# tcantenot/bmfr

Measured on AMD Instinct MI355X. Metric: ms/frame @1080p & 4K, 1/2/4/8 GPU; PSNR vs 4096spp reference, lower is better.
Workload: dtype f32+f16 tmp_data

## Files before the change

### bmfr_amd/_build.py

```python
from __future__ import annotations

import concurrent.futures as cf
import hashlib
import os
import subprocess

HERE = os.path.dirname(os.path.abspath(__file__))
CSRC = os.path.join(HERE, "csrc")
LIB = os.path.join(HERE, "libbmfr.so")
DIAG_LIB = os.path.join(HERE, "libbmfr_diag.so")
HIPCC = os.environ.get("HIPCC", "/opt/rocm/bin/hipcc")
SOURCES = ["bmfr_kernels.hip", "bmfr_fused.hip", "bmfr_fused_cols.hip", "bmfr_fused_cols_f32.hip", "bmfr_capi.hip",
           "bmfr_fused_plane.hip", "bmfr_fused_cols_plane.hip", "bmfr_fused_cols_f32_plane.hip",
           "bmfr_exchange.hip", "bmfr_prepare.hip", "bmfr_resolve.hip", "bmfr_firefly.hip",
           "bmfr_upsample.hip", "bmfr_display_taa.hip", "bmfr_synth.hip",
           "bmfr_generic_ns1.hip", "bmfr_generic_ns2.hip", "bmfr_generic_ns3.hip", "bmfr_generic_ns4.hip",
           "bmfr_generic_aux_ns1.hip", "bmfr_generic_aux_ns2.hip", "bmfr_generic_aux_ns3.hip",
           "bmfr_generic_aux_ns4.hip"]
FLAGS = ["--offload-arch=gfx950", "-O3", "-std=c++17", "-fPIC", "-ffp-contract=off", "-fno-slp-vectorize",
         "-Wall", "-Wno-unused-function"]
LINK_FLAGS = ["--offload-arch=gfx950", "-shared", "-fPIC"]
LINK_LIBS = ["-ldl"]


INCLUDE = os.path.join(HERE, "..", "include")
ID_MARK = b"bmfr-build-id:"


def source_files() -> list:
    files = [os.path.join(CSRC, f) for f in sorted(os.listdir(CSRC)) if f.endswith((".hip", ".h"))]
    files += [os.path.join(INCLUDE, f) for f in sorted(os.listdir(INCLUDE)) if f.endswith(".h")]
    return files


def source_hash() -> str:
    h = hashlib.sha256()
    h.update(" ".join(FLAGS).encode() + b"\0" + " ".join(LINK_FLAGS + LINK_LIBS).encode() + b"\0")
    for f in source_files():
        h.update(os.path.basename(f).encode() + b"\0")
        with open(f, "rb") as fh:
            h.update(fh.read())
        h.update(b"\0")
    return h.hexdigest()


def build_id(diag: bool = False, extra_flags=()) -> str:
    flags = (["-DBMFR_STAMPS"] if diag else []) + [f for f in extra_flags if f]
    return source_hash() + ("+" + ",".join(flags) if flags else "")


def embedded_id(lib: str) -> str | None:
    if not os.path.exists(lib):
        return None
    with open(lib, "rb") as f:
        data = f.read()
    i = data.find(ID_MARK)
    if i < 0:
        return None
    j = data.index(b"\0", i)
    return data[i + len(ID_MARK):j].decode()


class _BuildLock:

    def __enter__(self):
        import fcntl
        self.f = open(os.path.join(HERE, ".build.lock"), "w")
        fcntl.flock(self.f, fcntl.LOCK_EX)
        return self

    def __exit__(self, *exc):
        import fcntl
        fcntl.flock(self.f, fcntl.LOCK_UN)
        self.f.close()


def _on_gpu_box() -> bool:
    return bool(os.environ.get("GRAFT_REPO_ROOT"))


def build(force: bool = False, verbose: bool = False, diag: bool = False, variant: str = "",
          extra_flags=()) -> str:
    lib = DIAG_LIB if diag else (os.path.join(HERE, f"libbmfr_{variant}.so") if variant else LIB)
    if _on_gpu_box() and os.path.exists(lib) and not force:
        return lib
    with _BuildLock():
        return _build(force, verbose, diag, variant, extra_flags)


def _build(force, verbose, diag, variant, extra_flags) -> str:
    lib = DIAG_LIB if diag else (os.path.join(HERE, f"libbmfr_{variant}.so") if variant else LIB)
    want = build_id(diag, extra_flags)
    if not force and embedded_id(lib) == want:
        return lib
    objdir = os.path.join(HERE, "_obj_diag" if diag else (f"_obj_{variant}" if variant else "_obj"))
    os.makedirs(objdir, exist_ok=True)
# ... 79 lines not shown
```

### bmfr_amd/_lib.py

```python
from __future__ import annotations

import ctypes as C
import os

import torch

HERE = os.path.dirname(os.path.abspath(__file__))
_variant = os.environ.get("BMFR_LIB", "")
LIB_PATH = os.path.join(HERE, f"libbmfr_{_variant}.so" if _variant else "libbmfr.so")

MAX_FEATURES = 16
MAX_AUX_FEATURES = 4

FEATURE_ONE, NORMAL_X, NORMAL_Y, NORMAL_Z = 0, 1, 2, 3
POSITION_X, POSITION_Y, POSITION_Z = 4, 5, 6
POSITION_X2, POSITION_Y2, POSITION_Z2 = 7, 8, 9
POSITION_X3, POSITION_Y3, POSITION_Z3 = 10, 11, 12
FEATURE_AUX0, FEATURE_AUX1, FEATURE_AUX2, FEATURE_AUX3 = 13, 14, 15, 16

STATUS = {0: "ok", 1: "invalid argument", 2: "unsupported configuration",
          3: "out of device memory", 4: "HIP runtime error", 5: "no HIP device",
          6: "reprojection reached past the tile halo",
          7: "a kernel's bounded wait for another work-group gave up"}
HALO_EXCEEDED = 6
# ... 74 lines not shown

class Surface(C.Structure):
    _fields_ = [
        ("data", C.c_void_p), ("format", C.c_int), ("pitch", C.c_size_t),
        ("width", C.c_int), ("height", C.c_int), ("origin_x", C.c_int), ("origin_y", C.c_int),
        ("flip_y", C.c_int), ("bgr", C.c_int), ("alpha", C.c_float),
    ]


UPSAMPLE_HDR, UPSAMPLE_TONEMAPPED = 0, 1


class UpsampleGuides(C.Structure):
    _fields_ = [
        ("width", C.c_int), ("height", C.c_int),
        ("albedo", C.c_void_p), ("albedo_format", C.c_int),
        ("normals", C.c_void_p), ("normal_format", C.c_int),
        ("positions", C.c_void_p), ("depth", C.c_void_p),
        ("inv_view_proj", C.c_float * 16), ("pixel_offset", C.c_float * 2),
        ("plane_limit_squared", C.c_float), ("normal_limit_squared", C.c_float),
    ]


class Plane(C.Structure):
    _fields_ = [("data", C.c_void_p), ("format", C.c_int), ("pitch", C.c_size_t)]


class DisplayTaaArgs(C.Structure):
    _fields_ = [
        ("width", C.c_int), ("height", C.c_int),
        ("current", Plane), ("history", Plane), ("result", Plane),
        ("prev_pixel", C.c_void_p),
        ("motion", C.c_void_p), ("motion_format", C.c_int),
        ("motion_scale", C.c_float * 2), ("motion_at_pixel_centre", C.c_int), ("pixel_offset", C.c_float * 2),
        ("blend_alpha", C.c_float), ("reset", C.c_int),
    ]


class FireflyParams(C.Structure):
    _fields_ = [("threshold", C.c_float), ("radius", C.c_int), ("floor", C.c_float), ("replace_nonfinite", C.c_int)]


class StateView(C.Structure):
    _fields_ = [(n, C.c_void_p) for n in
                ("noisy_accumulated", "spp", "filtered_accumulated", "tone_mapped",
                 "prev_frame_pixel", "accept", "result")]


class FrameProfile(C.Structure):
    _fields_ = [("frame_number", C.c_int), ("fused_block_ms", C.c_float), ("taa_ms", C.c_float),
                ("total_ms", C.c_float)]


_P, _I, _F16, _F2 = C.c_void_p, C.c_int, C.POINTER(C.c_float), C.POINTER(C.c_float)
SIGNATURES = {
    "bmfr_config_default": (None, [C.POINTER(Config), _I, _I]),
    "bmfr_config_sizes": (_I, [C.POINTER(Config), C.POINTER(Sizes)]),
    "bmfr_status_string": (C.c_char_p, [_I]),
    "bmfr_last_hip_error": (_I, []),
    "bmfr_build_id": (C.c_char_p, []),
    "bmfr_create": (_I, [C.POINTER(Config), _I, C.POINTER(_P)]),
    "bmfr_destroy": (_I, [_P]),
    "bmfr_get_sizes": (_I, [_P, C.POINTER(Sizes)]),
    "bmfr_accumulate_noisy_data": (_I, [_P, _P, _P, _P, _P, _P, _P, _P, _P, _P, _P, _P, _P,
                                        _F16, _F2, _I]),
    "bmfr_fitter": (_I, [_P, _P, _P, _P, _P, _I]),
    "bmfr_weighted_sum": (_I, [_P, _P, _P, _P, _P, _P, _P, _P, _I]),
    "bmfr_accumulate_filtered_data": (_I, [_P, _P, _P, _P, _P, _P, _P, _P, _P, _P, _I]),
    "bmfr_taa": (_I, [_P, _P, _P, _P, _P, _P, _I]),
    "bmfr_process_frame": (_I, [_P, _P, C.POINTER(FrameInputs), _F16, _F2, _I]),
    "bmfr_process_frame_interior": (_I, [_P, _P, C.POINTER(FrameInputs), _F16, _F2, _I]),
    "bmfr_gbuffer_default": (None, [C.POINTER(GBuffer)]),
    "bmfr_prepare_frame": (_I, [_P, _P, C.POINTER(GBuffer), C.POINTER(Prepared), _F2]),
    "bmfr_surface_default": (None, [C.POINTER(Surface)]),
    "bmfr_resolve_output": (_I, [_P, _P, _I, _P, C.POINTER(Surface)]),
    "bmfr_upsample_guides_default": (None, [C.POINTER(UpsampleGuides), C.POINTER(Config)]),
    "bmfr_upsample_output": (_I, [_P, _P, _I, _P, _P, C.POINTER(UpsampleGuides), C.POINTER(Surface), _P]),
    "bmfr_display_taa_default": (None, [C.POINTER(DisplayTaaArgs), C.POINTER(Config)]),
    "bmfr_display_taa": (_I, [_P, _P, C.POINTER(DisplayTaaArgs), C.POINTER(Surface)]),
    "bmfr_firefly_default": (None, [C.POINTER(FireflyParams)]),
    "bmfr_suppress_fireflies": (_I, [_P, _P, _P, _P, C.POINTER(FireflyParams), _P]),
    "bmfr_halo_copy": (_I, [_P, _P, C.POINTER(C.c_int), _I, _P, _I, C.POINTER(C.c_size_t)]),
    "bmfr_halo_need": (_I, [C.POINTER(Config), _I, C.POINTER(C.c_int), C.POINTER(C.c_int)]),
    "bmfr_process_sequence": (_I, [_P, _P, _I, C.POINTER(FrameInputs), _F16, _F2, _I, C.POINTER(_P)]),
    "bmfr_process_frame_border": (_I, [_P, _P, C.POINTER(FrameInputs), _F16, _F2, _I]),
    "bmfr_process_frame_aux": (_I, [_P, _P, C.POINTER(FrameInputs), C.POINTER(AuxInputs), _F16, _F2, _I]),
    "bmfr_process_frame_interior_aux": (_I, [_P, _P, C.POINTER(FrameInputs), C.POINTER(AuxInputs), _F16, _F2, _I]),
    "bmfr_process_frame_border_aux": (_I, [_P, _P, C.POINTER(FrameInputs), C.POINTER(AuxInputs), _F16, _F2, _I]),
    "bmfr_process_sequence_aux": (_I, [_P, _P, _I, C.POINTER(FrameInputs), C.POINTER(AuxInputs), _F16, _F2, _I,
                                       C.POINTER(_P)]),
    "bmfr_output": (_P, [_P]),
    "bmfr_halo_status": (_I, [_P, C.POINTER(C.c_uint)]),
    "bmfr_frame_status": (_I, [_P]),
    "bmfr_state": (_I, [_P, _I, C.POINTER(StateView)]),
    "bmfr_set_profiling": (_I, [_P, _I, _I]),
    "bmfr_set_profiling_stride": (_I, [_P, _I]),
    "bmfr_get_profile": (_I, [_P, C.POINTER(FrameProfile), _I, C.POINTER(_I)]),
    "bmfr_halo_plan": (_I, [C.POINTER(Config), C.POINTER(_I), _I, _I, _I, C.POINTER(_I), C.POINTER(_I),
                            C.POINTER(_I), C.POINTER(_I), _I, C.POINTER(_I)]),
    "bmfr_comm_unique_id": (_I, [C.c_char_p]),
    "bmfr_comm_create": (_I, [C.c_char_p, _I, _I, _I, C.POINTER(_P)]),
    "bmfr_comm_create_all": (_I, [_I, C.POINTER(_I), C.POINTER(_P)]),
    "bmfr_comm_destroy": (_I, [_P]),
    "bmfr_exchange_create": (_I, [_P, C.POINTER(Config), C.POINTER(_I), _I, _I, _P, C.POINTER(_P)]),
    "bmfr_exchange_run": (_I, [_P, _P, _I]),
    "bmfr_exchange_run_all": (_I, [C.POINTER(_P), _I, C.POINTER(_P), _I]),
    "bmfr_exchange_bytes": (_I, [_P, _I, C.POINTER(C.c_size_t), C.POINTER(C.c_size_t)]),
    "bmfr_exchange_destroy": (_I, [_P]),
    "bmfr_synth_camera": (None, [_I, _I, _I, _F16, _F2]),
    "bmfr_debug_stamps": (_I, [_P, _P, C.c_size_t]),
    "bmfr_debug_sync": (_I, [_P, _I, _I]),
    "bmfr_debug_frame_launches": (_I, [_P, _I]),
    "bmfr_debug_suppress_fireflies": (_I, [_P, _P, _P, _I, _I, _I, C.POINTER(FireflyParams), _P]),
    "bmfr_synth_frame_host": (_I, [_I, _I, _I, C.c_uint32, _P, _P, _P, _P, _P]),
    "bmfr_synth_frame_device": (_I, [_I, _I, _I, C.c_uint32, _P, _P, _P, _P, _P, _P]),
    "bmfr_synth_region_device": (_I, [_I, _I, _I, _I, _I, _I, _I, C.c_uint32, _P, _P, _P, _P, _P, _P]),
}

_lib = None


class StaleLibraryError(ImportError):
    """The library on disk was not built from the sources in this tree."""


def check_build_id(lib: C.CDLL, path: str) -> str:
    from . import _build
    if not hasattr(lib, "bmfr_build_id"):
        raise StaleLibraryError(f"{path} predates bmfr_build_id(): rebuild it (__graft_entry__.build())")
    lib.bmfr_build_id.restype = C.c_char_p
    got = lib.bmfr_build_id().decode()
    want = _build.source_hash()
    if got.split("+")[0] != want and os.environ.get("BMFR_ALLOW_FOREIGN_BUILD") != "1":
        raise StaleLibraryError(f"{path} was built from other sources (build id {got[:16]}..., tree "
                                f"{want[:16]}...): rebuild it (__graft_entry__.build())")
    if "BMFR_PROBE" in got and os.environ.get("BMFR_ALLOW_PROBE") != "1":
        raise StaleLibraryError(f"{path} is a probe build ({got.split('+', 1)[1]}): its results are not "
                                f"guaranteed; set BMFR_ALLOW_PROBE=1 to time it anyway")
    return got


def build_id() -> str:
    return load().bmfr_build_id().decode()


def load() -> C.CDLL:
    global _lib
    if _lib is None:
        if not os.path.exists(LIB_PATH):
            raise ImportError(f"{LIB_PATH} missing: run `python -c 'import __graft_entry__ as g; g.build()'`")
        lib = C.CDLL(LIB_PATH)
        check_build_id(lib, LIB_PATH)
        for name, (res, args) in SIGNATURES.items():
            if _variant and not hasattr(lib, name):
                continue
            fn = getattr(lib, name)
            fn.restype = res
            fn.argtypes = args
        _lib = lib
    return _lib


def check(status: int, what: str) -> None:
    if status != 0:
        raise BmfrError(status, what)

# ... 5 lines not shown
```

### bmfr_amd/csrc/bmfr_capi.hip

```cpp
#include <algorithm>
#include <cmath>
#include <cstdio>
#include <cstdlib>
#include <cstring>
#include <initializer_list>

#include "../../include/bmfr.h"
#include "../../include/bmfr_debug.h"
#include "bmfr_firefly.h"
#include "bmfr_launch.h"
#include "bmfr_prepare.h"
#include "bmfr_resolve.h"
#include "bmfr_upsample.h"
#include "bmfr_display_taa.h"

using bmfr::Params;

struct bmfr_ctx {
    bmfr_config cfg;
    bmfr_sizes sizes;
    Params P;
    int device;
    float* noisy_acc[2] = {nullptr, nullptr};
    uint8_t* spp[2] = {nullptr, nullptr};
// ... 60 lines not shown
bmfr_status validate(const bmfr_config* c) {
    if (!c) return BMFR_ERROR_INVALID_ARGUMENT;
    for (int d = 0; d < 2; ++d) {
        const int n = d ? c->image_height : c->image_width;
        const int E = BMFR_BLOCK_EDGE_LENGTH;
        const int workset = E * ((n + E - 1) / E);
        if (n < E || workset + 30 > 2 * n) return BMFR_ERROR_INVALID_ARGUMENT;
    }
    if ((unsigned long long)c->image_width * c->image_height * 12ull > 0xffffffffull)
        return BMFR_ERROR_INVALID_ARGUMENT;
    if (c->features_not_scaled < 0 || c->features_scaled < 0 ||
        c->features_not_scaled + c->features_scaled > BMFR_MAX_FEATURES ||
        c->features_not_scaled + c->features_scaled < 1)
        return BMFR_ERROR_INVALID_ARGUMENT;
    for (int i = 0; i < c->features_not_scaled + c->features_scaled; ++i)
        if (c->feature_buffers[i] < 0 || c->feature_buffers[i] >= BMFR_FEATURE_COUNT_)
            return BMFR_ERROR_INVALID_ARGUMENT;
    if (c->tile_x || c->tile_y || c->tile_width || c->tile_height || c->tile_halo) {
        if (c->tile_x < 0 || c->tile_y < 0 || c->tile_width <= 0 || c->tile_height <= 0 ||
            c->tile_x + c->tile_width > c->image_width || c->tile_y + c->tile_height > c->image_height ||
            c->tile_halo < kMinTileHalo)
            return BMFR_ERROR_INVALID_ARGUMENT;
    }
    return BMFR_OK;
}

bool is_tiled(const bmfr_config* c) { return c->tile_width > 0; }
size_t done_bytes(const bmfr_ctx* c) { return (size_t)c->P.blocks_x * c->P.blocks_y * sizeof(unsigned); }
bool stage_api_ok(const bmfr_config* c) { return !is_tiled(c) && !c->input_half; }
bool names_aux(const bmfr_ctx* c) { return bmfr::aux_mask(c->P) != 0; }
bool aux_planes_ok(const bmfr_ctx* c, const bmfr_aux_inputs* aux) {
    const int mask = bmfr::aux_mask(c->P);
    for (int k = 0; k < BMFR_MAX_AUX_FEATURES; ++k)
        if ((mask & (1 << k)) && (!aux || !aux->aux[k])) return false;
    return true;
}

Params make_params(const bmfr_config* c, const bmfr_sizes* s) {
    Params P{};
    P.width = c->image_width;
    P.height = c->image_height;
    P.workset_w = s->workset_width;
    P.workset_h = s->workset_height;
    P.margins_w = s->workset_with_margins_width;
    P.margins_h = s->workset_with_margins_height;
    P.blocks_x = P.margins_w / BMFR_BLOCK_EDGE_LENGTH;
    P.blocks_y = P.margins_h / BMFR_BLOCK_EDGE_LENGTH;
    P.buffers = s->buffer_count;
    P.not_scaled = c->features_not_scaled;
    P.scaled = c->features_scaled;
    for (int i = 0; i < bmfr::kMaxFeatures; ++i) P.codes[i] = c->feature_buffers[i];
    P.noise2 = c->noise_amount * (double)2.f;
    P.blend_alpha = c->blend_alpha;
    P.second_blend_alpha = c->second_blend_alpha;
    P.taa_blend_alpha = c->taa_blend_alpha;
    P.position_limit_sq = as_kernel_literal(c->position_limit_squared);
    P.normal_limit_sq = as_kernel_literal(c->normal_limit_squared);
    P.half_tmp = c->use_half_precision_in_tmp_data ? 1 : 0;
    P.input_half = c->input_half ? 1 : 0;
    P.library_powr = c->library_powr ? 1 : 0;
    P.fast_fit = c->fast_fit ? 1 : 0;
    P.ox = s->region_x;
    P.oy = s->region_y;
    P.stride = s->region_width;
    P.rows = s->region_height;
    P.bx0 = P.by0 = 0;
    P.nbx = P.blocks_x;
    P.nby = P.blocks_y;
    P.tx0 = P.ty0 = 0;
    P.tx1 = P.width;
    P.ty1 = P.height;
    P.check_reach = c->tile_width > 0 ? 1 : 0;
    P.vx0 = P.ox;
    P.vy0 = P.oy;
    P.vx1 = P.ox + P.stride;
    P.vy1 = P.oy + P.rows;
    P.wx0 = P.vx0, P.wy0 = P.vy0, P.wx1 = P.vx1, P.wy1 = P.vy1;
    P.max_polls = bmfr::kDefaultMaxPolls;
    P.debug_delay = 0;
    P.frame_launches = 0;
    return P;
}

Params frame_params_cfg(const bmfr_config& g, Params P, int frame) {
    const int E = BMFR_BLOCK_EDGE_LENGTH;
    const int ox = bmfr::kBlockOffsetTable[frame & 15][0], oy = bmfr::kBlockOffsetTable[frame & 15][1];
    auto range = [&](int lo, int hi, int off, int nblocks, int& b0, int& nb) {
        b0 = -1;
        nb = 0;
        for (int b = 0; b < nblocks; ++b) {
            const int p0 = E * b - E / 2 + off, p1 = p0 + E;
            if (p0 < hi && p1 > lo) {
                if (b0 < 0) b0 = b;
                nb = b - b0 + 1;
            }
        }
    };
    range(std::max(0, g.tile_x - 1), std::min(g.image_width, g.tile_x + g.tile_width + 1), ox, P.blocks_x, P.bx0,
          P.nbx);
    range(std::max(0, g.tile_y - 1), std::min(g.image_height, g.tile_y + g.tile_height + 1), oy, P.blocks_y,
          P.by0, P.nby);
    P.tx0 = g.tile_x;
    P.ty0 = g.tile_y;
    P.tx1 = g.tile_x + g.tile_width;
    P.ty1 = g.tile_y + g.tile_height;
    const int reach = g.tile_halo - 33;
    auto need = [&](int b0, int nb, int off, int size, int r0, int r1, int& v0, int& v1) {
        int lo = size, hi = -1;
        for (int p = E * b0 - E / 2 + off; p < E * (b0 + nb) - E / 2 + off; ++p) {
            const int m = p < 0 ? -p - 1 : (p >= size ? 2 * size - p - 1 : p);
            lo = std::min(lo, m);
            hi = std::max(hi, m);
        }
        v0 = std::max(lo - reach, r0);
        v1 = std::min(hi + 1 + reach, r1);
    };
    need(P.bx0, P.nbx, ox, g.image_width, P.ox, P.ox + P.stride, P.vx0, P.vx1);
    need(P.by0, P.nby, oy, g.image_height, P.oy, P.oy + P.rows, P.vy0, P.vy1);
    P.wx0 = std::max(P.tx0 - reach, P.ox), P.wx1 = std::min(P.tx1 + reach, P.ox + P.stride);
    P.wy0 = std::max(P.ty0 - reach, P.oy), P.wy1 = std::min(P.ty1 + reach, P.oy + P.rows);
    return P;
}

Params frame_params(const bmfr_ctx* c, int frame) {
    return is_tiled(&c->cfg) ? frame_params_cfg(c->cfg, c->P, frame) : c->P;
}

hipStream_t as_stream(void* s) { return reinterpret_cast<hipStream_t>(s); }

bmfr::Camera make_camera(const float m[16], const float off[2]) {
    bmfr::Camera cam;
    for (int i = 0; i < 16; ++i) cam.m[i] = m[i];
    cam.jx = off[0];
    cam.jy = off[1];
    return cam;
}

}

extern "C" {

void bmfr_config_default(bmfr_config* c, int w, int h) {
    std::memset(c, 0, sizeof *c);
    c->image_width = w;
    c->image_height = h;
    const int f[] = {BMFR_FEATURE_ONE,        BMFR_FEATURE_NORMAL_X,   BMFR_FEATURE_NORMAL_Y,
                     BMFR_FEATURE_NORMAL_Z,   BMFR_FEATURE_POSITION_X, BMFR_FEATURE_POSITION_Y,
                     BMFR_FEATURE_POSITION_Z, BMFR_FEATURE_POSITION_X2, BMFR_FEATURE_POSITION_Y2,
                     BMFR_FEATURE_POSITION_Z2};
    c->features_not_scaled = 4;
    c->features_scaled = 6;
    for (int i = 0; i < 10; ++i) c->feature_buffers[i] = f[i];
    c->noise_amount = 1e-2;
    c->blend_alpha = 0.2f;
    c->second_blend_alpha = 0.1f;
    c->taa_blend_alpha = 0.2f;
    c->position_limit_squared = 0.01;
    c->normal_limit_squared = 0.1;
    c->use_half_precision_in_tmp_data = 1;
}

bmfr_status bmfr_config_sizes(const bmfr_config* c, bmfr_sizes* s) {
    const bmfr_status v = validate(c);
    if (v != BMFR_OK) return v;
    if (!s) return BMFR_ERROR_INVALID_ARGUMENT;
    const int E = BMFR_BLOCK_EDGE_LENGTH;
    s->buffer_count = c->features_not_scaled + c->features_scaled + 3;
    s->r_edge = s->buffer_count - 2;
    s->workset_width = E * ((c->image_width + E - 1) / E);
    s->workset_height = E * ((c->image_height + E - 1) / E);
    s->workset_with_margins_width = s->workset_width + E;
    s->workset_with_margins_height = s->workset_height + E;
    s->blocks = (s->workset_with_margins_width / E) * (s->workset_with_margins_height / E);
    const size_t elem = c->use_half_precision_in_tmp_data ? 2 : 4;
    s->tmp_data_bytes = (size_t)s->workset_with_margins_width * s->workset_with_margins_height *
                        s->buffer_count * elem;
    s->weights_bytes = (size_t)s->blocks * (s->buffer_count - 3) * 3 * sizeof(float);
    s->mins_maxs_bytes = (size_t)s->blocks * c->features_scaled * 2 * sizeof(float);
    s->image_bytes = (size_t)c->image_width * c->image_height * 3 * sizeof(float);
    if (is_tiled(c)) {
        s->region_x = std::max(0, c->tile_x - c->tile_halo);
        s->region_y = std::max(0, c->tile_y - c->tile_halo);
        s->region_width = std::min(c->image_width, c->tile_x + c->tile_width + c->tile_halo) - s->region_x;
        s->region_height = std::min(c->image_height, c->tile_y + c->tile_height + c->tile_halo) - s->region_y;
    } else {
        s->region_x = s->region_y = 0;
        s->region_width = c->image_width;
        s->region_height = c->image_height;
    }
    s->region_bytes = (size_t)s->region_width * s->region_height * 3 * sizeof(float);
    s->frame_launches = s->blocks >= bmfr::kTwoLaunchBlocks ? 2 : 1;
    return BMFR_OK;
}

const char* bmfr_status_string(bmfr_status s) {
    switch (s) {
        case BMFR_OK: return "ok";
        case BMFR_ERROR_INVALID_ARGUMENT: return "invalid argument";
        case BMFR_ERROR_UNSUPPORTED: return "unsupported configuration";
        case BMFR_ERROR_OUT_OF_MEMORY: return "out of device memory";
        case BMFR_ERROR_HIP: return "HIP runtime error";
        case BMFR_ERROR_NO_DEVICE: return "no HIP device";
        case BMFR_ERROR_HALO_EXCEEDED: return "reprojection reached past the tile halo";
        case BMFR_ERROR_SYNC_TIMEOUT: return "a kernel's bounded wait for another work-group gave up";
    }
    return "unknown status";
}

// ... 918 lines not shown
    if (!std::isfinite(p->threshold) || !(p->threshold > 0.0f) || (p->radius != 1 && p->radius != 2) ||
        !std::isfinite(p->floor) || p->floor < 0.0f)
        return BMFR_ERROR_INVALID_ARGUMENT;
    bmfr::FireflyArgs a{};
    a.noisy = noisy;
    a.out = out;
    a.stats = stats;
    a.threshold = p->threshold;
    a.floor = p->floor;
    a.replace_nonfinite = p->replace_nonfinite != 0;
    a.rw = width;
    a.rh = height;
    return hip_status(bmfr::launch_firefly(a, half, p->radius, as_stream(stream)));
}

}

bmfr_status bmfr_suppress_fireflies(bmfr_ctx* c, void* stream, const void* noisy, void* out,
                                    const bmfr_firefly_params* p, uint32_t* stats) {
    if (!c) return BMFR_ERROR_INVALID_ARGUMENT;
    DeviceGuard guard(c->device);
    return suppress_fireflies(stream, noisy, out, c->sizes.region_width, c->sizes.region_height,
                              c->cfg.input_half != 0, p, stats);
}

bmfr_status bmfr_debug_suppress_fireflies(void* stream, const void* noisy, void* out, int width, int height,
                                          int half, const bmfr_firefly_params* p, uint32_t* stats) {
    if (width <= 0 || height <= 0 || (unsigned long long)width * height * 12ull > 0xffffffffull)
        return BMFR_ERROR_INVALID_ARGUMENT;
    return suppress_fireflies(stream, noisy, out, width, height, half != 0, p, stats);
}

bmfr_status bmfr_halo_copy(bmfr_ctx* c, void* stream, const int* rects, int n, void* buffer, int unpack,
                           size_t* bytes) {
    if (!c || n < 0 || (n > 0 && !rects)) return BMFR_ERROR_INVALID_ARGUMENT;
    if (!is_tiled(&c->cfg)) return BMFR_ERROR_UNSUPPORTED;
    DeviceGuard guard(c->device);
    const int i = c->cur;
    struct {
        uint8_t* base;
        int bpp;
    } planes[4] = {{reinterpret_cast<uint8_t*>(c->noisy_acc[i]), 12}, {c->spp[i], 1},
                   {reinterpret_cast<uint8_t*>(c->acc[i]), 12}, {reinterpret_cast<uint8_t*>(c->result[i]), 12}};
    const bmfr_sizes& s = c->sizes;
    bmfr::HaloArgs a{};
    long long off = 0;
    for (int r = 0; r < n; ++r) {
        const int* q = rects + 5 * r;
        const int x = q[0], y = q[1], w = q[2], h = q[3], mask = q[4];
        if (w <= 0 || h <= 0 || x < s.region_x || y < s.region_y || x + w > s.region_x + s.region_width ||
            y + h > s.region_y + s.region_height || mask <= 0 || mask > BMFR_HALO_ALL)
            return BMFR_ERROR_INVALID_ARGUMENT;
        for (int k = 0; k < 4; ++k) {
            if (!(mask & (1 << k))) continue;
            if (a.nseg == bmfr::kMaxHaloSegs) return BMFR_ERROR_INVALID_ARGUMENT;
            const auto& p = planes[k];
            bmfr::HaloSeg& g = a.seg[a.nseg++];
            const size_t first = ((size_t)(y - s.region_y) * s.region_width + (x - s.region_x)) * p.bpp;
            g.plane = reinterpret_cast<unsigned long long>(p.base + first);
            g.buf_off = off;
            g.row_bytes = w * p.bpp;
            g.rows = h;
            g.pitch = s.region_width * p.bpp;
            off += ((long long)g.row_bytes * h + 15) & ~15LL;
        }
    }
    if (bytes) *bytes = (size_t)off;
    if (!buffer) return BMFR_OK;
    return hip_status(bmfr::launch_halo_copy(a, as_stream(stream), buffer, unpack));
}

bmfr_status bmfr_halo_need(const bmfr_config* cfg, int frame_number, int state_rect[4], int result_rect[4]) {
    if (!cfg || frame_number < 0 || !state_rect || !result_rect) return BMFR_ERROR_INVALID_ARGUMENT;
    bmfr_sizes sz;
    const bmfr_status st = bmfr_config_sizes(cfg, &sz);
    if (st != BMFR_OK) return st;
    if (!is_tiled(cfg)) return BMFR_ERROR_UNSUPPORTED;
    const Params P = frame_params_cfg(*cfg, make_params(cfg, &sz), frame_number);
    const int v[4] = {P.vx0, P.vy0, P.vx1 - P.vx0, P.vy1 - P.vy0}, w[4] = {P.wx0, P.wy0, P.wx1 - P.wx0, P.wy1 - P.wy0};
    for (int k = 0; k < 4; ++k) state_rect[k] = v[k], result_rect[k] = w[k];
    return BMFR_OK;
}

bmfr_status bmfr_set_profiling_stride(bmfr_ctx* c, int stride) {
    if (!c || stride <= 0 || c->pending_frame >= 0) return BMFR_ERROR_INVALID_ARGUMENT;
    c->prof_stride = stride;
    return BMFR_OK;
}

bmfr_status bmfr_set_profiling(bmfr_ctx* c, int enable, int capacity) {
    if (!c || (enable && capacity <= 0) || c->pending_frame >= 0) return BMFR_ERROR_INVALID_ARGUMENT;
    DeviceGuard guard(c->device);
    if (c->prof_events) {
        (void)hipDeviceSynchronize();
        for (int i = 0; i < 3 * c->prof_capacity; ++i) (void)hipEventDestroy(c->prof_events[i]);
        delete[] c->prof_events;
        delete[] c->prof_frames;
        c->prof_events = nullptr;
        c->prof_frames = nullptr;
    }
    c->prof_capacity = 0;
    c->prof_count = 0;
    if (!enable) return BMFR_OK;
    c->prof_events = new hipEvent_t[3 * capacity]();
    c->prof_frames = new int[capacity]();
    for (int i = 0; i < 3 * capacity; ++i) {
        const bmfr_status st = hip_status(hipEventCreate(&c->prof_events[i]));
        if (st != BMFR_OK) return st;
    }
    c->prof_capacity = capacity;
    return BMFR_OK;
}

bmfr_status bmfr_get_profile(bmfr_ctx* c, bmfr_frame_profile* out, int max_frames, int* count) {
    if (!c || !count || (max_frames > 0 && !out)) return BMFR_ERROR_INVALID_ARGUMENT;
    DeviceGuard guard(c->device);
    const long have = c->prof_count < c->prof_capacity ? c->prof_count : c->prof_capacity;
    const long first = c->prof_count - have;
    int n = 0;
    for (long k = first; k < c->prof_count && n < max_frames; ++k, ++n) {
        const int slot = (int)(k % c->prof_capacity);
        hipEvent_t* ev = c->prof_events + 3 * slot;
        bmfr_status st = hip_status(hipEventSynchronize(ev[2]));
        if (st != BMFR_OK) return st;
        float a = 0, b = 0, t = 0;
        if ((st = hip_status(hipEventElapsedTime(&a, ev[0], ev[1]))) != BMFR_OK) return st;
        if ((st = hip_status(hipEventElapsedTime(&b, ev[1], ev[2]))) != BMFR_OK) return st;
        if ((st = hip_status(hipEventElapsedTime(&t, ev[0], ev[2]))) != BMFR_OK) return st;
        out[n].frame_number = c->prof_frames[slot];
        out[n].fused_block_ms = a;
        out[n].taa_ms = b;
        out[n].total_ms = t;
    }
    *count = n;
    return BMFR_OK;
}

bmfr_status bmfr_halo_status(bmfr_ctx* c, unsigned* overshoot) {
    if (!c) return BMFR_ERROR_INVALID_ARGUMENT;
    if (overshoot) *overshoot = 0;
    DeviceGuard guard(c->device);
    const bmfr_status st = wait_frames(c);
    if (st != BMFR_OK) return st;
    if (c->reach_host && overshoot) *overshoot = c->reach_host[0];
    return reported(c);
}

bmfr_status bmfr_frame_status(bmfr_ctx* c) {
    if (!c) return BMFR_ERROR_INVALID_ARGUMENT;
    return bmfr_halo_status(c, nullptr);
}

bmfr_status bmfr_debug_sync(bmfr_ctx* c, int max_polls, int k1_delay) {
    if (!c || k1_delay < 0 || c->pending_frame >= 0) return BMFR_ERROR_INVALID_ARGUMENT;
    c->P.max_polls = max_polls < 0 ? bmfr::kDefaultMaxPolls : max_polls;
    c->P.debug_delay = k1_delay;
    return BMFR_OK;
}

bmfr_status bmfr_debug_frame_launches(bmfr_ctx* c, int launches) {
    if (!c || launches < 0 || launches > 2 || c->pending_frame >= 0) return BMFR_ERROR_INVALID_ARGUMENT;
    c->P.frame_launches = launches;
    return BMFR_OK;
}

bmfr_status bmfr_debug_stamps(const bmfr_ctx* c, unsigned long long* host, size_t count) {
// ... 28 lines not shown
```

### bmfr_amd/csrc/bmfr_fused.hip

```cpp
#include <utility>

#include "bmfr_launch.h"
#include "bmfr_taa_tile.h"
#include "bmfr_wave.h"

namespace bmfr {

constexpr int kThreads = 256;
constexpr int kS64Stride = 72;

template <int B, int N>
struct FloatRows {
    float v[B][N];
    __device__ __forceinline__ float get(int f, int j) const { return v[f][j]; }
    __device__ __forceinline__ void set(int f, int j, float x) { v[f][j] = x; }
    __device__ __forceinline__ void fence(int f) {
#pragma unroll
        for (int i = 0; i < N; ++i) asm volatile("" : "+v"(v[f][i]));
    }
};

template <int B>
struct K1Lds {
    static constexpr int KMAX = (B - 1) > 2 * (B - 7) ? (B - 1) : 2 * (B - 7);
// ... 143 lines not shown
        const float ucl = L.bc;
        const float vlen = sqrtf(sumsq + ucl * ucl);
        const float ucl2 = ucl - vlen;
        const float ulen2 = sumsq + ucl2 * ucl2;
        const float recip = 1.f / ulen2;
        if (t < col) {
#pragma unroll
            for (int ch = 0; ch < 3; ++ch) L.R[(col * RE + t) * 3 + ch] = A.get(col, 0);
        }
        if (t == col) {
#pragma unroll
            for (int ch = 0; ch < 3; ++ch) L.R[(col * RE + col) * 3 + ch] = vlen;
        }
        float u[kSubs];
#pragma unroll
        for (int s = 0; s < kSubs; ++s) u[s] = A.get(col, s);
        if (t == cl) u[0] = ucl2;

        constexpr int K = B - 1 - cl;
        float dot[K];
#pragma unroll
        for (int k = 0; k < K; ++k) {
            const int fb = cl + 1 + k;
            float sum = 0.f;
#pragma unroll
            for (int s = 0; s < kSubs; ++s)
                if (s > 0 || t >= cl) sum = sum + A.get(fb, s) * u[s];
            dot[k] = sum;
        }
#pragma unroll
        for (int fb = cl + 1; fb < B; ++fb) A.fence(fb);
        block_reduce<K>(dot, L, t);
#pragma unroll
        for (int k = 0; k < K; ++k) {
            const int fb = cl + 1 + k;
            const float c2 = 2.f * dot[k];
            if constexpr (FAST) {
                const float sc = c2 * recip;
#pragma unroll
                for (int s = 0; s < kSubs; ++s)
                    if (s > 0 || t >= cl) A.set(fb, s, __builtin_fmaf(-u[s], sc, A.get(fb, s)));
            } else {
#pragma unroll
                for (int s = 0; s < kSubs; ++s)
                    if (s > 0 || t >= cl) A.set(fb, s, A.get(fb, s) - div_by_recip(u[s] * c2, ulen2, recip));
            }
        }
    }
}

template <int B, bool FAST, class M, int... C>
__device__ __forceinline__ void qr_columns(M& A, K1Lds<B>& L, int t, const float* __restrict__ noise,
                                           double noise2, std::integer_sequence<int, C...>) {
    (qr_column<C, B, FAST>(A, L, t, noise, noise2), ...);
}

template <int B>
__device__ __forceinline__ void back_substitute(K1Lds<B>& L, int t) {
    constexpr int RE = B - 2;
    if (t >= 64) return;
    const int ch = t % 3, x = t / 3;
    float* R = L.R;
    for (int i = RE - 2; i >= 0; --i) {
        const float div = R[(i * RE + i) * 3 + ch];
        __builtin_amdgcn_wave_barrier();
        if (x < RE && x >= i) R[(x * RE + i) * 3 + ch] = R[(x * RE + i) * 3 + ch] / div;
        __builtin_amdgcn_fence(__ATOMIC_RELEASE, "wavefront");
        __builtin_amdgcn_wave_barrier();
        if (x == 0) {
            float rhs = R[((RE - 1) * RE + i) * 3 + ch];
            for (int j = i + 1; j < RE - 1; ++j) rhs = rhs - R[(j * RE + i) * 3 + ch];
            R[((RE - 1) * RE + i) * 3 + ch] = rhs;
        }
        __builtin_amdgcn_fence(__ATOMIC_RELEASE, "wavefront");
        __builtin_amdgcn_wave_barrier();
        const float xi = R[((RE - 1) * RE + i) * 3 + ch];
        if (x <= i && x < RE) R[(i * RE + x) * 3 + ch] = R[(i * RE + x) * 3 + ch] * xi;
        __builtin_amdgcn_fence(__ATOMIC_RELEASE, "wavefront");
        __builtin_amdgcn_wave_barrier();
    }
    if (x < B - 3) L.weights[x * 3 + ch] = R[((RE - 1) * RE + x) * 3 + ch];
}

template <int NS, int FS, class IN, bool COH = false, bool FAST = false, bool PLANE = false>
__device__ __forceinline__ void k1_rows_body(const Params& P, const K1Args& A, K1Lds<NS + FS + 3>& L, int g) {
    constexpr int B = NS + FS + 3;
    const int t = threadIdx.x;
    const int frame = A.frame;
    const NoisyInputs& in = A.in;
#ifdef BMFR_STAMPS
#define BMFR_STAMP(k) \
    if (t == 0 && A.stamps) A.stamps[(size_t)g * 8 + (k)] = __builtin_amdgcn_s_memtime()
#else
#define BMFR_STAMP(k) (void)0
#endif
    BMFR_STAMP(0);
    int bx, by;
    k1_block(P, g, bx, by);
    if constexpr (COH) {
        if (t == 0) {
            L.flag = (by - P.by0) * P.nbx + (bx - P.bx0);
            L.delay = P.debug_delay;
        }
    }

    FloatRows<B, kSubs> M;
    int over = 0;
    uint32_t state = 0;
    uint32_t state_hi = 0;
    NoisyCur<IN, PLANE> cur[kSubs];
#pragma unroll
    for (int s = 0; s < kSubs; ++s)
        cur[s] = noisy_load_current<IN, true, PLANE>(P, in, bx * kEdge + (t & (kEdge - 1)), by * kEdge + (t >> 5) + 8 * s,
                                                     frame, A.prev_pixel_in);
#pragma unroll
    for (int s = 0; s < kSubs; ++s) {
        const NoisyItem it = noisy_item_spec<true, IN, PLANE>(P, in, A.cam, cur[s], frame, A.acc_prev);
        L.keep[(s * 3 + 0) * kThreads + t] = it.prev_f.x;
        L.keep[(s * 3 + 1) * kThreads + t] = it.prev_f.y;
        L.keep[(s * 3 + 2) * kThreads + t] = it.prev_f.z;
        over = max(over, it.over);
#pragma unroll
        for (int f = 0; f < B; ++f) {
            float v;
            if (f < B - 3) v = feature_value(f, it.n, it.p);
            else v = f == B - 3 ? it.color.x : (f == B - 2 ? it.color.y : it.color.z);
            if (__builtin_isnan(v)) v = 0.0f;
            M.set(f, s, v);
        }
        const uint32_t bits = (uint32_t)it.owner | ((uint32_t)it.accept << 1) | ((uint32_t)it.prev_f_divided << 5) |
                              ((uint32_t)it.spp << 8);
        if (s < 2) state |= bits << (16 * s);
        else state_hi |= bits << (16 * (s - 2));
        st3_drop(drop_plane(A.noisy_out), it.lin, it.owner, it.color);
        st1_drop(drop_plane(A.spp_out), it.lin, it.owner, it.spp);
        st2_drop<COH ? kSc1 : 0>(drop_plane(A.prev_pixel_out), it.lin, it.owner, make_float2(it.pfx, it.pfy));
    }
    report_reach(P, A.reach, over);

    BMFR_STAMP(1);
    if constexpr (FS > 0) {
        float mm[2 * FS];
#pragma unroll
        for (int f = 0; f < FS; ++f) {
            float hi = -INFINITY, lo = INFINITY;
#pragma unroll
            for (int s = 0; s < kSubs; ++s) {
                hi = fmaxf(M.get(NS + f, s), hi);
                lo = fminf(M.get(NS + f, s), lo);
            }
            mm[f] = hi;
            mm[FS + f] = lo;
        }
        block_reduce<2 * FS, 1, FS>(mm, L, t);
#pragma unroll
        for (int f = 0; f < FS; ++f) {
            const float bmax = mm[f], bmin = mm[FS + f];
            const float d = bmax - bmin;
            const bool divide = fabsf(d) > 1.0f;
            const float rcp = 1.f / d;
            if (t == 0) {
                L.mm[3 * f] = bmin;
                L.mm[3 * f + 1] = bmax;
                L.mm[3 * f + 2] = rcp;
            }
#pragma unroll
            for (int s = 0; s < kSubs; ++s) {
                const float v = M.get(NS + f, s) - bmin;
                M.set(NS + f, s, divide ? div_by_recip(v, d, rcp) : v);
            }
        }
    }

    BMFR_STAMP(2);
    qr_columns<B, FAST>(M, L, t, A.noise, P.noise2, std::make_integer_sequence<int, B - 3>{});
    if (t < B - 3) {
#pragma unroll
        for (int ch = 0; ch < 3; ++ch) L.R[((B - 3) * (B - 2) + t) * 3 + ch] = M.get(B - 3 + ch, 0);
    }
    __syncthreads();
    BMFR_STAMP(3);
    back_substitute<B>(L, t);
    __syncthreads();
    BMFR_STAMP(4);

    int t3 = t;
    asm volatile("" : "+v"(t3));
    const int2 off = kBlockOffsets[frame & 15];
    f3 n[kSubs], pos[kSubs];
    uint32_t lin[kSubs];
    uint32_t bits[kSubs];
#pragma unroll
    for (int s = 0; s < kSubs; ++s) {
        bits[s] = (s < 2 ? state >> (16 * s) : state_hi >> (16 * (s - 2))) & 0xffffu;
        const int px = bx * kEdge + (t3 & (kEdge - 1)) - kEdge / 2 + off.x;
        const int py = by * kEdge + (t3 >> 5) + 8 * s - kEdge / 2 + off.y;
        lin[s] = pix(P, (bits[s] & 1u) ? px : P.ox, (bits[s] & 1u) ? py : P.oy);
        n[s] = ld3in<IN>(in.n_cur, lin[s]);
        pos[s] = ld3in<IN>(in.p_cur, lin[s]);
    }
#pragma unroll
    for (int s = 0; s < kSubs; ++s) {
        if (bits[s] & 1u) {
            f3 c{0.f, 0.f, 0.f};
#pragma unroll
            for (int f = 0; f < B - 3; ++f) {
                float v = feature_value(f, n[s], pos[s]);
                if (f >= NS) {
                    const float bmin = L.mm[3 * (f - NS)], bmax = L.mm[3 * (f - NS) + 1];
                    const float d = bmax - bmin;
                    v = v - bmin;
                    if (fabsf(d) > 1.0f) v = div_by_recip(v, d, L.mm[3 * (f - NS) + 2]);
                }
                c.x = c.x + L.weights[3 * f] * v;
                c.y = c.y + L.weights[3 * f + 1] * v;
                c.z = c.z + L.weights[3 * f + 2] * v;
            }
            c.x = c.x < 0.f ? 0.f : c.x;
            c.y = c.y < 0.f ? 0.f : c.y;
            c.z = c.z < 0.f ? 0.f : c.z;
            const float alpha = (bits[s] & 32u) ? fmaxf(rcp_nr((float)(bits[s] >> 8)), P.second_blend_alpha) : 1.f;
            const float beta = 1.f - alpha;
            const f3 prev{L.keep[(s * 3) * kThreads + t3], L.keep[(s * 3 + 1) * kThreads + t3],
                          L.keep[(s * 3 + 2) * kThreads + t3]};
            const f3 acc{alpha * c.x + beta * prev.x, alpha * c.y + beta * prev.y, alpha * c.z + beta * prev.z};
            if constexpr (COH) st3_coh(coh_plane(A.acc_out), lin[s], acc);
            else st3(A.acc_out, lin[s], acc);
        }
    }
#ifdef BMFR_STAMPS
    __syncthreads();
#endif
    BMFR_STAMP(5);
#undef BMFR_STAMP
    if constexpr (COH) {
        const int delay = L.delay;
        if (delay > 0 && g % kDelayStride == kDelayPhase)
            for (int k = 0; k < delay; ++k) __builtin_amdgcn_s_sleep(127);
        __builtin_amdgcn_s_waitcnt(0x0f70);
        __syncthreads();
        if (t == 0) __hip_atomic_store(&A.done[L.flag], A.epoch, __ATOMIC_RELAXED, __HIP_MEMORY_SCOPE_AGENT);
    }
}

constexpr int kRowsMinWaves = 4;
template <int NS, int FS, class IN, bool FAST = false, bool PLANE = false>
__global__ __launch_bounds__(kThreads, FS == 6 ? kRowsMinWaves : 3) void k_fused(Params P, K1Args A) {
    __shared__ K1Lds<NS + FS + 3> L;
    k1_rows_body<NS, FS, IN, false, FAST, PLANE>(P, A, L, xcd_swizzle(blockIdx.x, gridDim.x));
}

static_assert(kThreads == kTileThreads, "the TAA tiles run on this kernel's work-groups");
template <int NS, int FS, class IN, bool FAST = false, bool PLANE = false>
__global__ __launch_bounds__(kThreads, FS == 6 ? kRowsMinWaves : 3) void k_fused_rows_taa(Params P, K1Args A, TaaArgs T, int nk1, int nk1p) {
    __shared__ union {
        K1Lds<NS + FS + 3> k1;
        FrameTaaLds k2;
    } U;
    const int b = blockIdx.x;
    if (b < nk1) k1_rows_body<NS, FS, IN, true, FAST, PLANE>(P, A, U.k1, xcd_swizzle(b, nk1));
    else if (b >= nk1p) frame_taa_part<IN, true>(P, T, b, nk1p, U.k2);
}

#ifndef BMFR_ROWS_PLANE
#define BMFR_ROWS_PLANE 0
#endif
constexpr bool kRowsPlane = BMFR_ROWS_PLANE;
hipError_t launch_fused_rows_frame_one_plane(const Params& P, hipStream_t st, const FusedArgs& A);
hipError_t launch_fused_k1_plane(const Params& P, hipStream_t st, const FusedArgs& A);

#if !BMFR_ROWS_PLANE
bool fused_supported(const Params& P) {
    if (P.not_scaled != 4 || (P.scaled != 6 && P.scaled != 9)) return false;
    for (int f = 0; f < P.buffers - 3; ++f)
        if (P.codes[f] != f) return false;
    return true;
}
#endif

namespace {

template <template <int, class, bool> class L, class... Args>
static void dispatch_rows(const Params& Q, Args&&... args) {
    if (Q.scaled == 6) {
        if (Q.input_half) Q.fast_fit ? L<6, _Float16, true>::go(args...) : L<6, _Float16, false>::go(args...);
        else Q.fast_fit ? L<6, float, true>::go(args...) : L<6, float, false>::go(args...);
    } else {
        if (Q.input_half) Q.fast_fit ? L<9, _Float16, true>::go(args...) : L<9, _Float16, false>::go(args...);
        else Q.fast_fit ? L<9, float, true>::go(args...) : L<9, float, false>::go(args...);
    }
}

template <int FS, class IN, bool FAST>
struct LaunchK1 {
    static void go(const Params& P, hipStream_t st, const FusedArgs& A) {
        hipLaunchKernelGGL((k_fused<4, FS, IN, FAST, kRowsPlane>), dim3(k1_blocks(P)), dim3(kThreads), 0, st, P, k1_args(A));
    }
};

template <int FS, class IN, bool FAST>
struct LaunchRowsFrame {
    static void go(const Params& P, hipStream_t st, const FusedArgs& A) {
        const int nk1 = P.ring < 0 || P.nbx <= 0 || P.nby <= 0 ? 0 : k1_blocks(P), nk1p = (nk1 + 7) & ~7;
        hipLaunchKernelGGL((k_fused_rows_taa<4, FS, IN, FAST, kRowsPlane>), dim3(nk1p + frame_taa_tiles(P)),
                           dim3(kThreads), 0, st, P, k1_args(A), taa_args(A), nk1, nk1p);
    }
};

}

#if BMFR_ROWS_PLANE
hipError_t launch_fused_rows_frame_one_plane(const Params& P, hipStream_t st, const FusedArgs& A) {
    dispatch_rows<LaunchRowsFrame>(P, P, st, A);
    return hipGetLastError();
}

hipError_t launch_fused_k1_plane(const Params& P, hipStream_t st, const FusedArgs& A) {
    dispatch_rows<LaunchK1>(P, P, st, A);
    return hipGetLastError();
}
#else
hipError_t launch_fused_rows_frame_one(const Params& P, hipStream_t st, const FusedArgs& A) {
    if (A.prev_pixel_in) return launch_fused_rows_frame_one_plane(P, st, A);
    dispatch_rows<LaunchRowsFrame>(P, P, st, A);
    return hipGetLastError();
}

hipError_t launch_fused_k1(const Params& P, hipStream_t st, const FusedArgs& A) {
    if (A.prev_pixel_in) return launch_fused_k1_plane(P, st, A);
    dispatch_rows<LaunchK1>(P, P, st, A);
    return hipGetLastError();
}
#endif

}
```

### bmfr_amd/csrc/bmfr_fused_cols.hip

```cpp
#include <type_traits>
#include <utility>

#include "bmfr_launch.h"
#include "bmfr_taa_tile.h"
#include "bmfr_wave.h"

namespace bmfr {
namespace cols {

constexpr int kNW = 4;
constexpr int kK1Threads = 64 * kNW;
static_assert(kK1Threads == kTileThreads, "the frame kernels' TAA tiles run on K1's work-groups");
constexpr int kItems = 16 / kNW;
constexpr int kSlots = 16;
constexpr int kUStride = 20;
constexpr int kPre = 2;

constexpr int kUBufs = 3;
constexpr int kKeep = 16 * 3 * 64;
template <bool F32>
constexpr int m_slots() { return F32 ? kSlots - 4 : kSlots; }
constexpr bool keep_in_m(int B, bool F32 = false) {
    return (B - 1) * 64 * (F32 ? 4 * m_slots<true>() : 2 * kSlots) >= (kUBufs * 64 * kUStride + kKeep) * 4;
}
// ... 546 lines not shown
                        for (int i = 0; i < 8; ++i)
                            a[k][i] = __builtin_convertvector(
                                (f2v{fma_h<0>(a[k][i], fs, fo), fma_h<1>(a[k][i], fs, fo)}), h2);
                    } else {
#pragma unroll
                        for (int i = 0; i < 8; ++i) a[k][i] = __builtin_elementwise_fma(a[k][i], f2v{fs, fs}, f2v{fo, fo});
                    }
                } else {
#pragma unroll
                    for (int j = 0; j < kSlots; ++j) {
                        const float v = hget(a[k], j) - bmin;
                        hset(a[k], j, divide ? div_by_recip(v, d, rcp) : v);
                    }
                }
            }
        });
        if (W == 0 && l < 3) L.fo().R[l] = 32.f;

        steps(a, L, W, l, noise, pre, noise2, std::make_integer_sequence<int, NF>{});

        sfor<NSL>([&](auto K) {
            constexpr int k = decltype(K)::value;
            const int c = 1 + W + kNW * k;
            if (owns(W, c) && c >= NF) {
                if (l < NF) L.fo().R[((B - 3) * (B - 2) + l) * 3 + (c - NF)] = hget(a[k], 0);
            }
        });
    }
};

template <int K>
__device__ __forceinline__ float row_shl(float v) {
    if constexpr (K == 0) return v;
    else return __int_as_float(__builtin_amdgcn_update_dpp(0, __float_as_int(v), 0x100 + K, 0xf, 0xf, true));
}
template <int N>
__device__ __forceinline__ float row_bcast(float v) {
    return __int_as_float(__builtin_amdgcn_update_dpp(0, __float_as_int(v), 0x150 + N, 0xf, 0xf, false));
}
template <int B, bool FAST, class LDS>
__device__ __forceinline__ void back_substitute_regs(LDS& L, int t) {
    constexpr int RE = B - 2;
    static_assert(RE <= 16, "one DPP row per channel");
    if (t >= 64) return;
    const int ch = t >> 4, x = t & 15;
    const bool live = ch < 3 && x < RE;
    float col[RE - 1];
#pragma unroll
    for (int y = 0; y < RE - 1; ++y) col[y] = live ? L.fo().R[(x * RE + y) * 3 + ch] : 0.f;
    sfor<RE - 1>([&](auto I) {
        constexpr int i = RE - 2 - decltype(I)::value;
        const float div = row_bcast<i>(col[i]);
        if constexpr (FAST) {
            const float r = __builtin_amdgcn_rcpf(div);
            if (live && x >= i) col[i] = col[i] * r;
        } else {
            if (live && x >= i) col[i] = col[i] / div;
        }
        const float v = col[i];
        constexpr int src = i == RE - 2 ? RE - 1 : RE - 2;
        float acc = v;
        if constexpr (i < RE - 2) {
            acc = row_shl<RE - 2 - i>(v) - v;
#pragma unroll
            for (int j = i + 2; j <= RE - 2; ++j) acc = dpp_shr1(acc) - v;
        }
        if constexpr (i < RE - 2) {
            const float at_rhs = dpp_shr1(acc);
            if (x == RE - 1) col[i] = at_rhs;
        }
        const float xi = row_shl<src - i>(acc);
        if (x == i) {
#pragma unroll
            for (int y = 0; y <= i; ++y) col[y] = col[y] * xi;
        }
    });
    if (ch < 3 && x == RE - 1) {
#pragma unroll
        for (int y = 0; y < B - 3; ++y) L.fo().weights[y * 3 + ch] = col[y];
    }
}


template <int NS, int FS, class IN, bool COH = false, bool FAST = false, bool F32 = false, bool PLANE = false>
__device__ __forceinline__ void k1_cols_body(const Params& P, const K1Args& A, Lds<NS + FS + 3, F32>& L, int g) {
    constexpr int B = NS + FS + 3;
    constexpr bool FASTR = FAST && !F32;
    using P2 = Pair<F32>;
    using Fit = WaveFit<NS, FS, FAST, F32>;
    constexpr int NT = kK1Threads, NI = kItems;
    const int t = threadIdx.x;
    const int w = __builtin_amdgcn_readfirstlane(t >> 6);
    const int l = t & 63;
    const int frame = A.frame;
#ifdef BMFR_STAMPS
#define BMFR_STAMP(k) \
    if (t == 0 && A.stamps) A.stamps[(size_t)g * 8 + (k)] = __builtin_amdgcn_s_memtime()
#else
#define BMFR_STAMP(k) (void)0
#endif
    BMFR_STAMP(0);
#ifdef BMFR_STAMPS
    if (t == 0 && A.stamps) A.stamps[(size_t)g * 8 + 6] = __builtin_amdgcn_s_memrealtime();
#endif
    int bx, by;
    k1_block(P, g, bx, by);
    if constexpr (COH)
        if (t == 0) L.flag = (by - P.by0) * P.nbx + (bx - P.bx0);
    constexpr bool kInterleave = FASTR;
    auto item_slot = [&](int i) {
        return kInterleave ? kNW * i + w : NI * w + i;
    };
    const int lx = l & (kEdge - 1);
    auto item_row = [&](int lane, int i) { return (lane >> 5) + 2 * item_slot(i); };

    P2 pk[B];
    f2v own[Fit::NSL][2];
    uint32_t spps = 0;
    uint32_t ibits = 0;
    int over = 0;
    float kp[NI][3];
    constexpr bool kKeepNP = FAST && !F32 && B < 16;
    KeptNP<IN> keep_np[NI];
    NoisyCur<IN, PLANE> cur = noisy_load_current<IN, true, PLANE>(P, A.in, bx * kEdge + lx, by * kEdge + item_row(l, 0), frame,
                                                           A.prev_pixel_in);
#pragma unroll
    for (int i = 0; i < NI; ++i) {
        const NoisyTaps<IN> tp = noisy_taps_issue<true, IN, PLANE>(P, A.in, A.cam, cur, frame, A.acc_prev);
        NoisyCur<IN, PLANE> nxt;
        if (i < NI - 1)
            nxt = noisy_load_current<IN, true, PLANE>(P, A.in, bx * kEdge + lx, by * kEdge + item_row(l, i + 1), frame,
                                                      A.prev_pixel_in);
        __builtin_amdgcn_sched_barrier(0);
        const NoisyItem it = noisy_taps_finish<true, IN, PLANE>(P, cur, tp, frame);
        if constexpr (kKeepNP) keep_np[i].set(cur.nrm, cur.wp);
        {
#pragma unroll
            for (int f = 1; f < B; ++f) {
                float v;
                if (f < B - 3) v = feature_value(f, it.n, it.p);
                else v = f == B - 3 ? it.color.x : (f == B - 2 ? it.color.y : it.color.z);
                if constexpr (F32) v = __builtin_isnan(v) ? 0.0f : v;
                else v = __builtin_isnan(v) ? 0.0f : __builtin_amdgcn_fmed3f(v, -65504.f, 65504.f);
                if constexpr (kInterleave) {
                    const int j = item_slot(i);
                    L.M[f - 1][l * kSlots + 2 * ((j >> 1) ^ ((l >> 2) & 7)) + (j & 1)] = (_Float16)v;
                } else {
                    if constexpr (F32) pk[f][i & 1] = v;
                    else pk[f][i & 1] = (_Float16)v;
                }
            }
            spps |= (uint32_t)it.spp << (8 * i);
            ibits |= ((uint32_t)it.owner << i) | ((uint32_t)it.prev_f_divided << (4 + i));
            over = max(over, it.over);
            if constexpr (keep_in_m(B, F32)) {
                kp[i][0] = it.prev_f.x;
                kp[i][1] = it.prev_f.y;
                kp[i][2] = it.prev_f.z;
            } else {
                L.keep_s[(i * 3 + 0) * NT + t] = it.prev_f.x;
                L.keep_s[(i * 3 + 1) * NT + t] = it.prev_f.y;
                L.keep_s[(i * 3 + 2) * NT + t] = it.prev_f.z;
            }
            st3_drop(drop_plane(A.noisy_out), it.lin, it.owner, it.color);
            st1_drop(drop_plane(A.spp_out), it.lin, it.owner, it.spp);
            st2_drop<COH ? kSc1 : 0>(drop_plane(A.prev_pixel_out), it.lin, it.owner, make_float2(it.pfx, it.pfy));
            if (!kInterleave && (i & 1)) {
                if constexpr (F32) {
                    static_assert(!kInterleave, "f32 tmp_data: wave w computes row quad w");
#pragma unroll
                    for (int f = 1; f < B; ++f) {
                        const int ow = Fit::owner(f);
                        if (w == ow) own[Fit::slot(f)][i >> 1] = pk[f];
                        else
                            *reinterpret_cast<f2v*>(&L.M[f - 1][l * m_slots<true>() + 4 * (w - (w > ow)) + (i - 1)]) =
                                pk[f];
                    }
                } else {
                    const int pair = (item_slot(i) / 2) ^ ((l >> 2) & 7);
#pragma unroll
                    for (int f = 1; f < B; ++f)
                        *reinterpret_cast<uint32_t*>(&L.M[f - 1][l * kSlots + 2 * pair]) =
                            __builtin_bit_cast(uint32_t, pk[f]);
                }
            }
        }
        if (i < NI - 1) cur = nxt;
    }
    report_reach(P, A.reach, over);
    float pre[kPre][kSlots];
    Fit::prefetch_noise(w, l, A.noise, pre);
    k1_barrier();
    BMFR_STAMP(1);
    BMFR_STAMP(2);

    if (t == 0) L.delay = P.debug_delay;
    Fit::run(L, w, l, A.noise, pre, P.noise2, P.max_polls, kp, own);
    int l3 = l;
    asm volatile("" : "+v"(l3));
    const int2 off = kBlockOffsets[frame & 15];
    uint32_t lin[NI];
    In3<IN> nrm_r[NI], wp_r[NI];
#pragma unroll
    for (int i = 0; i < NI; ++i) {
        const int px = bx * kEdge + (l3 & (kEdge - 1)) - kEdge / 2 + off.x;
        const int py = by * kEdge + item_row(l3, i) - kEdge / 2 + off.y;
        lin[i] = pix(P, (ibits & (1u << i)) ? px : P.ox, (ibits & (1u << i)) ? py : P.oy);
        if constexpr (kKeepNP) {
            keep_np[i].get(nrm_r[i], wp_r[i]);
        } else {
            nrm_r[i] = ld3raw<IN>(A.in.n_cur, lin[i]);
            wp_r[i] = ld3raw<IN>(A.in.p_cur, lin[i]);
        }
    }
    k1_barrier();
    BMFR_STAMP(3);
    back_substitute_regs<B, FAST>(L, t);
    k1_barrier();
    if constexpr (!COH)
        if (t == 0 && L.timeout) report_sync_timeout(A.sync_err, kSyncPivot, frame);
    BMFR_STAMP(4);
    f3 nrm[NI], wp[NI];
#pragma unroll
    for (int i = 0; i < NI; ++i) {
        nrm[i] = widen(nrm_r[i]);
        wp[i] = widen(wp_r[i]);
    }

    constexpr int NPR = NI / 2;
    f2v cp[NPR][3];
#pragma unroll
    for (int h = 0; h < NPR; ++h)
        for (int ch = 0; ch < 3; ++ch) cp[h][ch] = f2v{0.f, 0.f};
    constexpr bool kPairs = B >= 16;
    constexpr int NH = kPairs ? NPR : 1;
#pragma unroll
    for (int hh = 0; hh < NH; ++hh) {
#pragma unroll
        for (int f = 0; f < B - 3; ++f) {
            const f2v wv[3] = {f2v{L.fo().weights[3 * f], L.fo().weights[3 * f]},
                               f2v{L.fo().weights[3 * f + 1], L.fo().weights[3 * f + 1]},
                               f2v{L.fo().weights[3 * f + 2], L.fo().weights[3 * f + 2]}};
            float bmin = 0.f, d = 0.f, rcp = 0.f;
            if (f >= NS) {
                bmin = L.fo().mm[3 * (f - NS)];
                d = L.fo().mm[3 * (f - NS) + 1] - bmin;
                rcp = L.fo().mm[3 * (f - NS) + 2];
            }
#pragma unroll
            for (int h = kPairs ? hh : 0; h < (kPairs ? hh + 1 : NPR); ++h) {
                f2v v = {feature_value(f, nrm[2 * h], wp[2 * h]), feature_value(f, nrm[2 * h + 1], wp[2 * h + 1])};
                if (f >= NS && FAST) {
                    const bool divide = fabsf(d) > 1.0f;
                    const float fs = divide ? rcp : 1.f, fo = divide ? -bmin * rcp : -bmin;
                    v = __builtin_elementwise_fma(v, f2v{fs, fs}, f2v{fo, fo});
                } else if (f >= NS) {
                    v = v - f2v{bmin, bmin};
                    if (fabsf(d) > 1.0f) {
                        const f2v q0 = v * f2v{rcp, rcp};
                        const f2v r = __builtin_elementwise_fma(-q0, f2v{d, d}, v);
                        v = __builtin_elementwise_fma(r, f2v{rcp, rcp}, q0);
                    }
                }
#pragma unroll
                for (int ch = 0; ch < 3; ++ch) cp[h][ch] = cp[h][ch] + wv[ch] * v;
            }
            __builtin_amdgcn_sched_barrier(0);
        }
    }
#pragma unroll
    for (int i = 0; i < NI; ++i) {
        if (ibits & (1u << i)) {
            f3 ci{cp[i >> 1][0][i & 1], cp[i >> 1][1][i & 1], cp[i >> 1][2][i & 1]};
            ci.x = ci.x < 0.f ? 0.f : ci.x;
            ci.y = ci.y < 0.f ? 0.f : ci.y;
            ci.z = ci.z < 0.f ? 0.f : ci.z;
            const float sp = (float)((spps >> (8 * i)) & 255u);
            const float alpha =
                (ibits & (1u << (4 + i))) ? fmaxf(COH ? 1.f / sp : rcp_nr(sp), P.second_blend_alpha) : 1.f;
            const float beta = 1.f - alpha;
            const int t3 = l3 + 64 * w;
            const float* kb = L.keep();
            const f3 prev{kb[(i * 3) * NT + t3], kb[(i * 3 + 1) * NT + t3], kb[(i * 3 + 2) * NT + t3]};
            const f3 acc{alpha * ci.x + beta * prev.x, alpha * ci.y + beta * prev.y, alpha * ci.z + beta * prev.z};
            if constexpr (COH) st3_coh(coh_plane(A.acc_out), lin[i], acc);
            else st3(A.acc_out, lin[i], acc);
        }
    }
#ifdef BMFR_STAMPS
    __syncthreads();
#endif
    BMFR_STAMP(5);
#ifdef BMFR_STAMPS
    if (t == 0 && A.stamps) A.stamps[(size_t)g * 8 + 7] = __builtin_amdgcn_s_memrealtime();
#endif
#undef BMFR_STAMP
    if constexpr (COH) {
        const int delay = L.delay;
        if (delay > 0 && g % kDelayStride == kDelayPhase)
            for (int k = 0; k < delay; ++k) __builtin_amdgcn_s_sleep(127);
        __builtin_amdgcn_s_waitcnt(0x0f70);
        lds_barrier();
        if (t == 0)
            __hip_atomic_store(&A.done[L.flag], A.epoch | (L.timeout ? kDoneTimeout : 0u), __ATOMIC_RELAXED,
                               __HIP_MEMORY_SCOPE_AGENT);
    }
}

template <int FS, bool F32>
constexpr int min_waves() {
    return F32 && FS == 9 ? 3 : 4;
}

template <int NS, int FS, class IN, bool FAST = false, bool F32 = false, bool PLANE = false>
__global__ __launch_bounds__(kK1Threads, (min_waves<FS, F32>())) void k_fused_cols(Params P, K1Args A) {
    __shared__ Lds<NS + FS + 3, F32> L;
    k1_cols_body<NS, FS, IN, false, FAST, F32, PLANE>(P, A, L, xcd_swizzle(blockIdx.x, gridDim.x));
}

template <int NS, int FS, class IN, bool SAME = false, bool FAST = false, bool F32 = false, bool PLANE = false>
__global__ __launch_bounds__(kK1Threads, (min_waves<FS, F32>())) void k_fused_cols_taa(Params P, K1Args A, Params P2,
                                                                                    TaaArgs T, int nk1, int nk1p) {
    __shared__ union {
        Lds<NS + FS + 3, F32> k1;
        FrameTaaLds k2;
    } U;
    const int b = blockIdx.x;
    if (b < nk1) k1_cols_body<NS, FS, IN, SAME, FAST, F32, PLANE>(P, A, U.k1, xcd_swizzle(b, nk1));
    else if (b >= nk1p) frame_taa_part<IN, SAME>(P2, T, b, nk1p, U.k2);
}

}

template <bool F32, bool PLANE>
hipError_t launch_cols_k1(const Params& P, hipStream_t st, const FusedArgs& A);
template <bool F32, bool PLANE>
hipError_t launch_cols_frame_one(const Params& P, hipStream_t st, const FusedArgs& A);
template <bool F32>
hipError_t launch_cols_k1_taa(const Params& P, hipStream_t st, const FusedArgs* A, const Params& P2,
                              const FusedArgs* A2);

#ifndef BMFR_COLS_F32
#define BMFR_COLS_F32 0
#endif
#ifndef BMFR_COLS_PLANE
#define BMFR_COLS_PLANE 0
#endif
constexpr bool kColsF32 = BMFR_COLS_F32;
constexpr bool kColsPlane = BMFR_COLS_PLANE;

namespace {


template <template <int, class, bool> class L, class... Args>
bool dispatch_cols(const Params& Q, Args&&... args) {
    if constexpr (!kColsF32) {
        if (Q.scaled == 6) {
            if (Q.input_half) Q.fast_fit ? L<6, _Float16, true>::go(args...) : L<6, _Float16, false>::go(args...);
            else Q.fast_fit ? L<6, float, true>::go(args...) : L<6, float, false>::go(args...);
        } else {
            if (Q.input_half) Q.fast_fit ? L<9, _Float16, true>::go(args...) : L<9, _Float16, false>::go(args...);
            else Q.fast_fit ? L<9, float, true>::go(args...) : L<9, float, false>::go(args...);
        }
    } else {
        if (!Q.fast_fit) return false;
        if (Q.scaled == 6) Q.input_half ? L<6, _Float16, true>::go(args...) : L<6, float, true>::go(args...);
        else Q.input_half ? L<9, _Float16, true>::go(args...) : L<9, float, true>::go(args...);
    }
    return true;
}

template <int FS, class IN, bool FAST>
struct LaunchCols {
    static void go(const Params& P, hipStream_t st, const FusedArgs& A) {
        hipLaunchKernelGGL((cols::k_fused_cols<4, FS, IN, FAST, kColsF32, kColsPlane>), dim3(k1_blocks(P)),
                           dim3(cols::kK1Threads), 0, st, P, k1_args(A));
    }
};

template <int FS, class IN, bool FAST>
struct LaunchFrameOne {
    static void go(const Params& P, hipStream_t st, const FusedArgs& A) {
        const int nk1 = P.ring < 0 || P.nbx <= 0 || P.nby <= 0 ? 0 : k1_blocks(P), nk1p = (nk1 + 7) & ~7;
        const int nk2 = frame_taa_tiles(P);
        hipLaunchKernelGGL((cols::k_fused_cols_taa<4, FS, IN, true, FAST, kColsF32, kColsPlane>), dim3(nk1p + nk2),
                           dim3(cols::kK1Threads), 0, st, P, k1_args(A), P, taa_args(A), nk1, nk1p);
    }
};

#if !BMFR_COLS_PLANE
template <int FS, class IN, bool FAST>
struct LaunchColsTaa {
    static void go(const Params& P, hipStream_t st, const FusedArgs* A, const Params& P2, const FusedArgs* A2) {
        const int nk1 = A ? k1_blocks(P) : 0, nk1p = (nk1 + 7) & ~7;
        const int nk2 = A2 ? frame_taa_tiles(P2) : 0;
        if (nk1 + nk2 == 0) return;
        const TaaArgs T = A2 ? taa_args(*A2) : TaaArgs{};
        hipLaunchKernelGGL((cols::k_fused_cols_taa<4, FS, IN, false, FAST, kColsF32>), dim3(nk2 ? nk1p + nk2 : nk1),
                           dim3(cols::kK1Threads), 0, st, A ? P : P2, k1_args(A ? *A : *A2), A2 ? P2 : P, T, nk1,
                           nk1p);
    }
};
#endif

}

template <>
hipError_t launch_cols_k1<kColsF32, kColsPlane>(const Params& P, hipStream_t st, const FusedArgs& A) {
    if (!dispatch_cols<LaunchCols>(P, P, st, A)) return hipErrorInvalidValue;
    return hipGetLastError();
}
template <>
hipError_t launch_cols_frame_one<kColsF32, kColsPlane>(const Params& P, hipStream_t st, const FusedArgs& A) {
    if (!dispatch_cols<LaunchFrameOne>(P, P, st, A)) return hipErrorInvalidValue;
    return hipGetLastError();
}
#if !BMFR_COLS_PLANE
template <>
hipError_t launch_cols_k1_taa<kColsF32>(const Params& P, hipStream_t st, const FusedArgs* A, const Params& P2,
                                        const FusedArgs* A2) {
    if (!dispatch_cols<LaunchColsTaa>(A ? P : P2, P, st, A, P2, A2)) return hipErrorInvalidValue;
    return hipGetLastError();
}
#endif

template <>
hipError_t launch_cols_k1<!kColsF32, kColsPlane>(const Params& P, hipStream_t st, const FusedArgs& A);
template <>
hipError_t launch_cols_k1<kColsF32, !kColsPlane>(const Params& P, hipStream_t st, const FusedArgs& A);
template <>
hipError_t launch_cols_k1<!kColsF32, !kColsPlane>(const Params& P, hipStream_t st, const FusedArgs& A);
template <>
hipError_t launch_cols_frame_one<!kColsF32, kColsPlane>(const Params& P, hipStream_t st, const FusedArgs& A);
template <>
hipError_t launch_cols_frame_one<kColsF32, !kColsPlane>(const Params& P, hipStream_t st, const FusedArgs& A);
template <>
hipError_t launch_cols_frame_one<!kColsF32, !kColsPlane>(const Params& P, hipStream_t st, const FusedArgs& A);

#if !BMFR_COLS_F32 && !BMFR_COLS_PLANE
bool fused_cols_supported(const Params& P) { return (P.half_tmp || P.fast_fit) && fused_supported(P); }

bool seq_fused_supported(const Params& P) { return fused_cols_supported(P) && P.ring == 0; }
bool frame_fused_supported(const Params& P) { return fused_supported(P); }

hipError_t launch_fused_frame_one(const Params& P, hipStream_t st, const FusedArgs& A) {
    if (!fused_cols_supported(P)) return launch_fused_rows_frame_one(P, st, A);
    if (A.prev_pixel_in)
        return P.half_tmp ? launch_cols_frame_one<false, true>(P, st, A) : launch_cols_frame_one<true, true>(P, st, A);
    return P.half_tmp ? launch_cols_frame_one<false, false>(P, st, A) : launch_cols_frame_one<true, false>(P, st, A);
}

hipError_t launch_fused_k1_taa(const Params& P, hipStream_t st, const FusedArgs* A, const Params& P2,
                               const FusedArgs* A2) {
    return (A ? P : P2).half_tmp ? launch_cols_k1_taa<false>(P, st, A, P2, A2)
                                 : launch_cols_k1_taa<true>(P, st, A, P2, A2);
}

hipError_t launch_fused_k1_cols(const Params& P, hipStream_t st, const FusedArgs& A) {
    if (A.prev_pixel_in) return P.half_tmp ? launch_cols_k1<false, true>(P, st, A) : launch_cols_k1<true, true>(P, st, A);
    return P.half_tmp ? launch_cols_k1<false, false>(P, st, A) : launch_cols_k1<true, false>(P, st, A);
}
#endif

}
```

### bmfr_amd/csrc/bmfr_kernels.h

```cpp
#pragma once

#include "bmfr_device.h"
#include "bmfr_powr.h"

namespace bmfr {

enum class RedOp { Sum, Max, Min };

template <RedOp OP>
__device__ __forceinline__ float red(float a, float b) {
    if constexpr (OP == RedOp::Sum) return a + b;
    else if constexpr (OP == RedOp::Max) return fmaxf(a, b);
    else return fminf(a, b);
}

template <RedOp OP>
__device__ __forceinline__ float bcast_lane(float v, int lane) {
    return __int_as_float(__builtin_amdgcn_readlane(__float_as_int(v), lane));
}

template <RedOp OP, int K>
__device__ __forceinline__ void block_reduce(const float (&v)[K], int n, float* __restrict__ part,
                                             float* __restrict__ res, int t) {
#pragma unroll
    for (int k = 0; k < K; ++k)
        if (k < n) part[k * kLocal + t] = v[k];
    __syncthreads();
    const int w = t >> 6, l = t & 63;
#pragma unroll
    for (int i = 0; i < (K + 3) / 4; ++i) {
        const int k = w + 4 * i;
        if (k < n) {
            const float* p = part + k * kLocal;
            float s;
            if constexpr (OP == RedOp::Sum) s = p[l] + ((p[l + 64] + p[l + 128]) + p[l + 192]);
            else s = red<OP>(red<OP>(red<OP>(p[l], p[l + 64]), p[l + 128]), p[l + 192]);
            float e;
            if constexpr (OP == RedOp::Sum) {
                float acc = __shfl(s, (l + 8) & 63);
#pragma unroll
                for (int j = 2; j < 8; ++j) acc = acc + __shfl(s, (l + 8 * j) & 63);
                e = s + acc;
            } else {
                e = s;
#pragma unroll
                for (int j = 1; j < 8; ++j) e = red<OP>(e, __shfl(s, (l + 8 * j) & 63));
            }
            float r = bcast_lane<OP>(e, 0);
#pragma unroll
            for (int j = 1; j < 8; ++j) r = red<OP>(r, bcast_lane<OP>(e, j));
            if (l == 0) res[k] = r;
        }
    }
    __syncthreads();
}

struct NoisyItem {
    f3 n, p;
    f3 color;
    float pfx, pfy;
    uint32_t lin;
    uint8_t accept;
    uint8_t spp;
    bool owner;
    f3 prev_f;
    bool prev_f_divided;
    int over;
};

struct NoisyInputs {
    const float* __restrict__ n_cur;
    const float* __restrict__ n_prev;
    const float* __restrict__ p_cur;
    const float* __restrict__ p_prev;
    const float* noisy_cur;
    const float* __restrict__ noisy_prev;
    const uint8_t* __restrict__ spp_prev;
};

struct Camera {
    float m[16];
    float jx, jy;
};

struct AuxPlanes {
    const float* p[kMaxAux];
};
struct AuxVals {
    float v[kMaxAux];
};
__device__ __forceinline__ float aux_value(int code, const AuxVals& x) {
    const int k = code - kFeatAux0;
    return k == 0 ? x.v[0] : (k == 1 ? x.v[1] : (k == 2 ? x.v[2] : x.v[3]));
}

__device__ __forceinline__ int xcd_swizzle(int g, int G) {
    constexpr int kXcds = 8;
    const int xcd = g % kXcds, k = g / kXcds;
    const int per = G / kXcds, rem = G % kXcds;
    return xcd < rem ? xcd * (per + 1) + k : rem * (per + 1) + (xcd - rem) * per + k;
}

__device__ __forceinline__ void k1_block(const Params& P, int g, int& bx, int& by) {
    if (P.ring == 0) {
        bx = P.bx0 + g % P.nbx;
        by = P.by0 + g / P.nbx;
        return;
    }
    const int W = P.nbx;
    const int top = (P.ry0 - P.by0) * W;
    if (g < top) {
        bx = P.bx0 + g % W;
        by = P.by0 + g / W;
        return;
    }
    g -= top;
    const int lw = P.rx0 - P.bx0, rw = P.bx0 + W - P.rx1, per_row = lw + rw, mid = (P.ry1 - P.ry0) * per_row;
    if (g < mid) {
        const int k = g % per_row;
        by = P.ry0 + g / per_row;
        bx = k < lw ? P.bx0 + k : P.rx1 + (k - lw);
        return;
    }
    g -= mid;
    bx = P.bx0 + g % W;
    by = P.ry1 + g / W;
}

__device__ __forceinline__ uint32_t pix(const Params& P, int x, int y) {
    return __umul24((uint32_t)(y - P.oy), (uint32_t)P.stride) + (uint32_t)(x - P.ox);
}
__device__ __forceinline__ int clamp_rx(const Params& P, int x) { return min(max(x, P.ox), P.ox + P.stride - 1); }
__device__ __forceinline__ int clamp_ry(const Params& P, int y) { return min(max(y, P.oy), P.oy + P.rows - 1); }

__device__ __forceinline__ NoisyItem noisy_item(const Params& P, const NoisyInputs& in,
                                                const Camera& cam, int gx, int gy, int frame,
                                                const float2* __restrict__ pf_plane = nullptr) {
    NoisyItem o;
    const int2 off = kBlockOffsets[frame & 15];
    const int ux = gx - kEdge / 2 + off.x, uy = gy - kEdge / 2 + off.y;
    const int px = mirror(ux, P.width), py = mirror(uy, P.height);
    o.owner = ux >= 0 && ux < P.width && uy >= 0 && uy < P.height;
    o.lin = (uint32_t)(py * P.width + px);

    const f3 wp = ld3(in.p_cur, o.lin);
    const f3 nrm = ld3(in.n_cur, o.lin);
    const f3 cur = ld3(in.noisy_cur, o.lin);
    o.n = nrm;
    o.p = wp;

    float pfx = (float)px, pfy = (float)py;
    uint8_t accept = 0;
    float alpha = 1.f;
    f3 prev{0.f, 0.f, 0.f};
    float sample_spp = 0.f;
    if (frame > 0) {
        if (pf_plane) {
            const float2 pf = ld_px(pf_plane, o.lin);
            pfx = pf.x;
            pfy = pf.y;
        } else {
            const float* M = cam.m;
            float u = dot4(M[0], M[4], M[8], M[12], wp.x, wp.y, wp.z, 1.f);
            float v = dot4(M[1], M[5], M[9], M[13], wp.x, wp.y, wp.z, 1.f);
            const float w = dot4(M[3], M[7], M[11], M[15], wp.x, wp.y, wp.z, 1.f);
            const float rw = 1.f / w;
            u = div_shared(u, w, rw);
            v = div_shared(v, w, rw);
            u = u + 1.f;
            v = v + 1.f;
            u = u / 2.f;
            v = v / 2.f;
            pfx = u * (float)P.width - cam.jx;
            pfy = v * (float)P.height - (1 - cam.jy);
        }
        const float flx = floorf(pfx), fly = floorf(pfy);
        const int ix = pf_plane ? (int)fminf(fmaxf(flx, -2.f), (float)P.width + 1.f) : (int)flx;
        const int iy = pf_plane ? (int)fminf(fmaxf(fly, -2.f), (float)P.height + 1.f) : (int)fly;
        const float fx = pfx - flx, fy = pfy - fly;
        const float omx = 1.f - fx, omy = 1.f - fy;
        const float wts[4] = {omx * omy, fx * omy, omx * fy, fx * fy};
        float total = 0.f;
#pragma unroll
        for (int i = 0; i < 4; ++i) {
            const int sx = ix + (i & 1), sy = iy + (i >> 1);
            if (sx >= 0 && sy >= 0 && sx < P.width && sy < P.height) {
                const uint32_t s = (uint32_t)(sy * P.width + sx);
                const f3 pp = ld3(in.p_prev, s);
                const f3 d{pp.x - wp.x, pp.y - wp.y, pp.z - wp.z};
                if (dot3(d, d) < P.position_limit_sq) {
                    const f3 pn = ld3(in.n_prev, s);
                    const f3 dn{pn.x - nrm.x, pn.y - nrm.y, pn.z - nrm.z};
                    if (dot3(dn, dn) < P.normal_limit_sq) {
                        accept |= (uint8_t)(1 << i);
                        sample_spp = sample_spp + wts[i] * (float)ld_px(in.spp_prev, s);
                        const f3 pc = ld3(in.noisy_prev, s);
                        prev.x = prev.x + wts[i] * pc.x;
                        prev.y = prev.y + wts[i] * pc.y;
                        prev.z = prev.z + wts[i] * pc.z;
                        total = total + wts[i];
                    }
                }
            }
        }
        if (total > 0.f) {
            const float rt = 1.f / total;
            prev.x = div_shared(prev.x, total, rt);
            prev.y = div_shared(prev.y, total, rt);
            prev.z = div_shared(prev.z, total, rt);
            sample_spp = div_shared(sample_spp, total, rt);
            alpha = 1.f / (sample_spp + 1.f);
            alpha = fmaxf(alpha, P.blend_alpha);
        }
    }
    uint8_t new_spp = 1;
    if (alpha < 1.f) new_spp = sample_spp > 254.f ? 255 : (uint8_t)((int)rintf(sample_spp) + 1);
    const float beta = 1.f - alpha;
    o.color = f3{alpha * cur.x + beta * prev.x, alpha * cur.y + beta * prev.y,
                 alpha * cur.z + beta * prev.z};
    o.pfx = pfx;
    o.pfy = pfy;
    o.accept = accept;
    o.spp = new_spp;
    return o;
}

template <bool PLANE>
struct NoisyCurPf {};
template <>
struct NoisyCurPf<true> {
    float2 pf;
};
template <class IN = float, bool PLANE = false>
struct NoisyCur : NoisyCurPf<PLANE> {
    In3<IN> wp, nrm, cur;
    int px, py;
    bool owner;
};
__device__ __forceinline__ void item_pixel(const Params& P, int gx, int gy, int frame, int& px, int& py, bool& owner) {
    const int2 off = kBlockOffsets[frame & 15];
    const int ux = gx - kEdge / 2 + off.x, uy = gy - kEdge / 2 + off.y;
    px = mirror(ux, P.width);
    py = mirror(uy, P.height);
    owner = ux >= 0 && ux < P.width && uy >= 0 && uy < P.height;
}

template <class IN = float, bool COLOUR = true, bool PLANE = false>
__device__ __forceinline__ NoisyCur<IN, PLANE> noisy_load_current(const Params& P, const NoisyInputs& in, int gx,
                                                                  int gy, int frame,
                                                                  const float2* __restrict__ pf_plane = nullptr) {
    NoisyCur<IN, PLANE> c;
    item_pixel(P, gx, gy, frame, c.px, c.py, c.owner);
    const uint32_t lin = pix(P, c.px, c.py);
    c.wp = ld3raw<IN>(in.p_cur, lin);
    c.nrm = ld3raw<IN>(in.n_cur, lin);
    if constexpr (COLOUR) c.cur = ld3raw<IN>(in.noisy_cur, lin);
    if constexpr (PLANE) c.pf = ld_px(pf_plane, lin);
    return c;
}

template <class IN>
constexpr bool kPairTaps = sizeof(IN) == 2;

template <class IN = float>
struct NoisyTaps {
    In3<IN> pp[4], pn[4];
    h3pair pq[2], nq[2];
    uint32_t fix;
    bool any_fix;
    f3 pc[4], pa[4];
    uint32_t spu[4];
    float wts[4];
    uint32_t inb;
    float pfx, pfy, flx, fly;
    int over;
};


__device__ __forceinline__ void bilinear_weights(float pfx, float pfy, float (&wts)[4]) {
    const float fx = pfx - floorf(pfx), fy = pfy - floorf(pfy);
    const float omx = 1.f - fx, omy = 1.f - fy;
    wts[0] = omx * omy;
    wts[1] = fx * omy;
    wts[2] = omx * fy;
    wts[3] = fx * fy;
}

struct Reproj {
    float pfx, pfy;
    int ix, iy;
    float wts[4];
    uint32_t inb;
    int over;
};
__device__ __forceinline__ void project_prev(const Params& P, const Camera& cam, const f3& wp, float& pfx, float& pfy) {
    const float* M = cam.m;
    float u = dot4(M[0], M[4], M[8], M[12], wp.x, wp.y, wp.z, 1.f);
    float v = dot4(M[1], M[5], M[9], M[13], wp.x, wp.y, wp.z, 1.f);
    const float w = dot4(M[3], M[7], M[11], M[15], wp.x, wp.y, wp.z, 1.f);
    const float rw = 1.f / w;
    u = div_shared(u, w, rw);
    v = div_shared(v, w, rw);
    u = u + 1.f;
    v = v + 1.f;
    u = u / 2.f;
    v = v / 2.f;
    pfx = u * (float)P.width - cam.jx;
    pfy = v * (float)P.height - (1 - cam.jy);
}
__device__ __forceinline__ Reproj reproject_taps(const Params& P, float pfx, float pfy, int px, int py) {
    Reproj r;
    r.pfx = pfx;
    r.pfy = pfy;
    const float flx = floorf(pfx), fly = floorf(pfy);
    const int ix = (int)fminf(fmaxf(flx, -2.f), (float)P.width + 1.f);
    const int iy = (int)fminf(fmaxf(fly, -2.f), (float)P.height + 1.f);
    r.ix = ix;
    r.iy = iy;
    bilinear_weights(pfx, pfy, r.wts);
    r.over = 0;
    if (P.check_reach) {
        const int x0 = max(ix, 0), x1 = min(ix + 1, P.width - 1);
        const int y0 = max(iy, 0), y1 = min(iy + 1, P.height - 1);
        const bool tpx = px >= P.tx0 && px < P.tx1 && py >= P.ty0 && py < P.ty1;
        const int vx0 = tpx ? P.wx0 : P.vx0, vx1 = tpx ? P.wx1 : P.vx1;
        const int vy0 = tpx ? P.wy0 : P.vy0, vy1 = tpx ? P.wy1 : P.vy1;
        if (x0 <= x1 && y0 <= y1)
            r.over = max(max(max(vx0 - x0, x1 - (vx1 - 1)), max(vy0 - y0, y1 - (vy1 - 1))), 0);
    }
    r.inb = 0;
#pragma unroll
    for (int i = 0; i < 4; ++i) {
        const int sx = ix + (i & 1), sy = iy + (i >> 1);
        r.inb |= (uint32_t)(sx >= 0 && sy >= 0 && sx < P.width && sy < P.height) << i;
    }
    return r;
}
__device__ __forceinline__ Reproj reproject(const Params& P, const Camera& cam, const f3& wp, int px, int py) {
    float pfx, pfy;
    project_prev(P, cam, wp, pfx, pfy);
    return reproject_taps(P, pfx, pfy, px, py);
}

template <bool FILT = false, class IN = float, bool PLANE = false>
__device__ __forceinline__ NoisyTaps<IN> noisy_taps_issue(const Params& P, const NoisyInputs& in, const Camera& cam,
                                                         const NoisyCur<IN, PLANE>& c, int frame,
                                                         const float* __restrict__ acc_prev = nullptr) {
    NoisyTaps<IN> tp;
    tp.pfx = (float)c.px;
    tp.pfy = (float)c.py;
    tp.over = 0;
    tp.inb = 0;
    if (frame > 0) {
        Reproj r;
        if constexpr (PLANE) r = reproject_taps(P, c.pf.x, c.pf.y, c.px, c.py);
        else r = reproject(P, cam, widen(c.wp), c.px, c.py);
        tp.pfx = r.pfx;
        tp.pfy = r.pfy;
        tp.over = r.over;
        tp.inb = r.inb;
        uint32_t sidx[4];
#pragma unroll
        for (int i = 0; i < 4; ++i) {
            tp.wts[i] = r.wts[i];
            sidx[i] = pix(P, clamp_rx(P, r.ix + (i & 1)), clamp_ry(P, r.iy + (i >> 1)));
        }
        if constexpr (kPairTaps<IN>) {
            const int n = P.stride * P.rows;
            const int xc = min(max(r.ix, P.ox - 1), P.ox + P.stride - 1) - P.ox;
            uint32_t spair[2];
            tp.fix = 0;
#pragma unroll
            for (int row = 0; row < 2; ++row) {
                const int sr = (int)__umul24((uint32_t)(clamp_ry(P, r.iy + row) - P.oy), (uint32_t)P.stride) + xc;
                spair[row] = (uint32_t)min(max(sr, 0), n - 2);
                tp.fix |= ((uint32_t)(sr < 0) << (2 * row)) | ((uint32_t)(sr > n - 2) << (2 * row + 1));
            }
            tp.any_fix = __builtin_amdgcn_ballot_w64(tp.fix != 0) != 0;
#pragma unroll
            for (int row = 0; row < 2; ++row) tp.pq[row] = ld3pair_h(in.p_prev, spair[row]);
#pragma unroll
            for (int row = 0; row < 2; ++row) tp.nq[row] = ld3pair_h(in.n_prev, spair[row]);
        } else {
#pragma unroll
            for (int i = 0; i < 4; ++i) tp.pp[i] = ld3raw<IN>(in.p_prev, sidx[i]);
#pragma unroll
            for (int i = 0; i < 4; ++i) tp.pn[i] = ld3raw<IN>(in.n_prev, sidx[i]);
        }
#pragma unroll
        for (int i = 0; i < 4; ++i) tp.pc[i] = ld3(in.noisy_prev, sidx[i]);
#pragma unroll
        for (int i = 0; i < 4; ++i) tp.spu[i] = ld_px(in.spp_prev, sidx[i]);
        if (FILT) {
#pragma unroll
            for (int i = 0; i < 4; ++i) tp.pa[i] = ld3(acc_prev, sidx[i]);
        }
    }
    return tp;
}

template <class IN = float>
__device__ __forceinline__ uint32_t taps_accept(const Params& P, const f3& wp, const f3& nrm, const In3<IN> (&pp)[4],
                                                const In3<IN> (&pn)[4], uint32_t inb) {
    uint32_t accept = 0;
#pragma unroll
    for (int i = 0; i < 4; ++i) {
        const f3 q = widen(pp[i]), m = widen(pn[i]);
        const f3 d{q.x - wp.x, q.y - wp.y, q.z - wp.z};
        const f3 dn{m.x - nrm.x, m.y - nrm.y, m.z - nrm.z};
        if ((inb & (1u << i)) && dot3(d, d) < P.position_limit_sq && dot3(dn, dn) < P.normal_limit_sq)
            accept |= 1u << i;
    }
    return accept;
}

template <bool FILT = false>
__device__ __forceinline__ NoisyItem taps_blend(const Params& P, const f3& cur, uint32_t accept, const float (&wts)[4],
                                                const f3 (&pc)[4], const uint32_t (&spu)[4], const f3 (&pa)[4],
                                                float pfx, float pfy, int over, uint32_t lin, bool owner, int frame) {
    NoisyItem o;
    o.owner = owner;
    o.lin = lin;
    float alpha = 1.f;
    f3 prev{0.f, 0.f, 0.f};
    float sample_spp = 0.f;
    o.prev_f = f3{0.f, 0.f, 0.f};
    o.prev_f_divided = false;
    o.over = over;
    if (frame > 0) {
        float total = 0.f;
#pragma unroll
        for (int i = 0; i < 4; ++i) {
            if (accept & (1u << i)) {
                sample_spp = sample_spp + wts[i] * (float)spu[i];
                prev.x = prev.x + wts[i] * pc[i].x;
                prev.y = prev.y + wts[i] * pc[i].y;
                prev.z = prev.z + wts[i] * pc[i].z;
                total = total + wts[i];
                if (FILT) {
                    o.prev_f.x = o.prev_f.x + wts[i] * pa[i].x;
                    o.prev_f.y = o.prev_f.y + wts[i] * pa[i].y;
                    o.prev_f.z = o.prev_f.z + wts[i] * pa[i].z;
                }
            }
        }
        if (total > 0.f) {
            const float rt = 1.f / total;
            prev.x = div_shared(prev.x, total, rt);
            prev.y = div_shared(prev.y, total, rt);
            prev.z = div_shared(prev.z, total, rt);
            sample_spp = div_shared(sample_spp, total, rt);
            alpha = rcp_nr(sample_spp + 1.f);
            alpha = fmaxf(alpha, P.blend_alpha);
            if (FILT) {
                o.prev_f_divided = true;
                o.prev_f.x = div_shared(o.prev_f.x, total, rt);
                o.prev_f.y = div_shared(o.prev_f.y, total, rt);
                o.prev_f.z = div_shared(o.prev_f.z, total, rt);
            }
        }
    }
    uint8_t new_spp = 1;
    if (alpha < 1.f) new_spp = sample_spp > 254.f ? 255 : (uint8_t)((int)rintf(sample_spp) + 1);
    const float beta = 1.f - alpha;
    o.color = f3{alpha * cur.x + beta * prev.x, alpha * cur.y + beta * prev.y, alpha * cur.z + beta * prev.z};
    o.pfx = pfx;
    o.pfy = pfy;
    o.accept = (uint8_t)accept;
    o.spp = new_spp;
    return o;
}

__device__ __forceinline__ void split_pairs(const h3pair (&q)[2], uint32_t fix, bool any_fix, In3<_Float16> (&t)[4]) {
#pragma unroll
    for (int r = 0; r < 2; ++r) {
        t[2 * r].v.xy = q[r].a;
        t[2 * r].v.z = (uint16_t)(q[r].b & 0xffffu);
        t[2 * r + 1].v.xy = __builtin_amdgcn_alignbit(q[r].c, q[r].b, 16);
        t[2 * r + 1].v.z = (uint16_t)(q[r].c >> 16);
    }
    if (any_fix) {
#pragma unroll
        for (int r = 0; r < 2; ++r) {
            if (fix & (1u << (2 * r))) t[2 * r + 1] = t[2 * r];
            if (fix & (2u << (2 * r))) t[2 * r] = t[2 * r + 1];
        }
    }
}

template <bool FILT = false, class IN = float, bool PLANE = false>
__device__ __forceinline__ NoisyItem noisy_taps_finish(const Params& P, const NoisyCur<IN, PLANE>& c,
                                                      const NoisyTaps<IN>& tp, int frame) {
    const f3 wp = widen(c.wp), nrm = widen(c.nrm), cur = widen(c.cur);
    uint32_t accept = 0u;
    if constexpr (kPairTaps<IN>) {
        if (frame > 0) {
            In3<IN> pp[4], pn[4];
            split_pairs(tp.pq, tp.fix, tp.any_fix, pp);
            split_pairs(tp.nq, tp.fix, tp.any_fix, pn);
            accept = taps_accept<IN>(P, wp, nrm, pp, pn, tp.inb);
        }
    } else {
        accept = frame > 0 ? taps_accept<IN>(P, wp, nrm, tp.pp, tp.pn, tp.inb) : 0u;
    }
    NoisyItem o = taps_blend<FILT>(P, cur, accept, tp.wts, tp.pc, tp.spu, tp.pa, tp.pfx, tp.pfy, tp.over,
                                   pix(P, c.px, c.py), c.owner, frame);
    o.n = nrm;
    o.p = wp;
    return o;
}

template <bool FILT = false, class IN = float, bool PLANE = false>
__device__ __forceinline__ NoisyItem noisy_item_spec(const Params& P, const NoisyInputs& in, const Camera& cam,
                                                     const NoisyCur<IN, PLANE>& c, int frame,
                                                     const float* __restrict__ acc_prev = nullptr) {
    return noisy_taps_finish<FILT, IN, PLANE>(P, c, noisy_taps_issue<FILT, IN, PLANE>(P, in, cam, c, frame, acc_prev), frame);
}

__device__ __forceinline__ void report_reach(const Params& P, unsigned* reach, int over) {
    if (P.check_reach && __builtin_amdgcn_ballot_w64(over > 0) != 0 && over > 0)
        atomicMax(reach, (unsigned)over);
}

template <bool AUX = false>
__device__ __forceinline__ float design_value(const Params& P, int f, const NoisyItem& it,
                                              const AuxVals* x = nullptr) {
    const int B = P.buffers;
    float v;
    if (f < B - 3) {
        if constexpr (AUX) v = P.codes[f] >= kFeatAux0 ? aux_value(P.codes[f], *x) : feature_value(P.codes[f], it.n, it.p);
        else v = feature_value(P.codes[f], it.n, it.p);
    } else v = f == B - 3 ? it.color.x : (f == B - 2 ? it.color.y : it.color.z);
    if (__builtin_isnan(v)) v = 0.0f;
    if (P.half_tmp) v = fmaxf(fminf(v, 65504.f), -65504.f);
    return v;
}

template <int B>
struct FitLds {
    float part[(B - 1) * kLocal];
    float res[B];
    float bc[2];
    float R[(B - 2) * (B - 2) * 3];
    float weights[(B - 3) * 3];
    float minmax[2 * (B - 3)];
};

template <int NS, int FS, bool HALF, bool FULL, bool FAST_DIV>
__device__ __forceinline__ void fit_block(float (&a)[NS + FS + 3][kSubs], FitLds<NS + FS + 3>& L,
                                          int t, int frame, double noise2) {
    constexpr int B = NS + FS + 3;
    constexpr int RE = B - 2;

    if constexpr (FS > 0) {
        float mx[FS], mn[FS];
#pragma unroll
        for (int f = 0; f < FS; ++f) {
            float hi = -INFINITY, lo = INFINITY;
#pragma unroll
            for (int s = 0; s < kSubs; ++s) {
                hi = fmaxf(a[NS + f][s], hi);
                lo = fminf(a[NS + f][s], lo);
            }
            mx[f] = hi;
            mn[f] = lo;
        }
        block_reduce<RedOp::Max, FS>(mx, FS, L.part, L.res, t);
        float bmax[FS];
#pragma unroll
        for (int f = 0; f < FS; ++f) bmax[f] = L.res[f];
        block_reduce<RedOp::Min, FS>(mn, FS, L.part, L.res, t);
#pragma unroll
        for (int f = 0; f < FS; ++f) {
            const float bmin = L.res[f];
            if (t == 0) {
                L.minmax[2 * f] = bmin;
                L.minmax[2 * f + 1] = bmax[f];
            }
#pragma unroll
            for (int s = 0; s < kSubs; ++s) {
                const float v = scale(a[NS + f][s], bmin, bmax[f]);
                a[NS + f][s] = HALF ? round_half(v) : v;
            }
        }
    }

    constexpr int COLS = FULL ? B : B - 3;
#pragma unroll
    for (int col = 0; col < COLS; ++col) {
        constexpr int dummy = 0;
        (void)dummy;
        const int cl = col < B - 3 ? col : B - 3;
        float sq = 0.f;
#pragma unroll
        for (int s = 0; s < kSubs; ++s) {
            const int i = t + s * kLocal;
            if (i >= cl + 1) sq = sq + a[col][s] * a[col][s];
        }
        if (t == cl) L.bc[0] = a[col][0];
        {
            float one[1] = {sq};
            block_reduce<RedOp::Sum, 1>(one, 1, L.part, L.res, t);
        }
// ... 66 lines not shown
                }
            }
        }
    }
    if constexpr (!FULL) {
        if (t < B - 3) {
#pragma unroll
            for (int ch = 0; ch < 3; ++ch) L.R[((RE - 1) * RE + t) * 3 + ch] = a[B - 3 + ch][0];
        }
    }
    __syncthreads();

    if (t < 3) {
        const int ch = t;
        float R[RE][RE];
#pragma unroll
        for (int x = 0; x < RE; ++x)
#pragma unroll
            for (int y = 0; y <= (x < RE - 1 ? x : RE - 2); ++y) R[x][y] = L.R[(x * RE + y) * 3 + ch];
#pragma unroll
        for (int i = RE - 2; i >= 0; --i) {
            const float div = R[i][i];
#pragma unroll
            for (int x = i; x < RE; ++x) R[x][i] = R[x][i] / div;
#pragma unroll
            for (int j = i + 1; j < RE - 1; ++j) R[RE - 1][i] = R[RE - 1][i] - R[j][i];
#pragma unroll
            for (int y = 0; y <= i; ++y) R[i][y] = R[i][y] * R[RE - 1][i];
        }
#pragma unroll
        for (int id = 0; id < B - 3; ++id) L.weights[id * 3 + ch] = R[RE - 1][id];
    }
    __syncthreads();
}

__device__ __forceinline__ f3 blend_filtered(const Params& P, f3 filtered, float pfx, float pfy,
                                             uint8_t acc_bits, uint8_t spp,
                                             const float* __restrict__ acc_prev, int frame) {
    f3 prev{0.f, 0.f, 0.f};
    float alpha = 1.f;
    if (frame > 0 && acc_bits > 0) {
        const float flx = floorf(pfx), fly = floorf(pfy);
        const int ix = (int)flx, iy = (int)fly;
        const float fx = pfx - flx, fy = pfy - fly;
        const float omx = 1.f - fx, omy = 1.f - fy;
        const float wts[4] = {omx * omy, fx * omy, omx * fy, fx * fy};
        float total = 0.f;
#pragma unroll
        for (int i = 0; i < 4; ++i) {
            if (acc_bits & (1 << i)) {
                total = total + wts[i];
                const f3 pc = ld3(acc_prev, pix(P, ix + (i & 1), iy + (i >> 1)));
                prev.x = prev.x + wts[i] * pc.x;
                prev.y = prev.y + wts[i] * pc.y;
                prev.z = prev.z + wts[i] * pc.z;
            }
        }
        if (total > 0.f) {
            alpha = 1.f / (float)spp;
            alpha = fmaxf(alpha, P.second_blend_alpha);
            const float rt = 1.f / total;
            prev.x = div_shared(prev.x, total, rt);
            prev.y = div_shared(prev.y, total, rt);
            prev.z = div_shared(prev.z, total, rt);
        }
    }
    const float beta = 1.f - alpha;
    return f3{alpha * filtered.x + beta * prev.x, alpha * filtered.y + beta * prev.y,
              alpha * filtered.z + beta * prev.z};
}

__device__ __forceinline__ f3 tone_map(const Params& P, f3 albedo, f3 a, const double* tE = kPowrE,
                                       const double2* tRP = kPowrRP) {
    const f3 p{albedo.x * a.x, albedo.y * a.y, albedo.z * a.z};
    if (P.library_powr) {
        const float g = 0.454545f;
        return f3{fminf(fmaxf(__ocml_powr_f32(fmaxf(0.f, p.x), g), 0.f), 1.f),
                  fminf(fmaxf(__ocml_powr_f32(fmaxf(0.f, p.y), g), 0.f), 1.f),
                  fminf(fmaxf(__ocml_powr_f32(fmaxf(0.f, p.z), g), 0.f), 1.f)};
    }
    return f3{gamma_clamped(p.x, tE, tRP), gamma_clamped(p.y, tE, tRP), gamma_clamped(p.z, tE, tRP)};
}

__device__ __forceinline__ void taa_load_taps(const Params& P, float2 pf, const float* __restrict__ prev_frame,
                                              f3 (&pc)[4]) {
    const int ix = (int)fminf(fmaxf(floorf(pf.x), -2.f), (float)P.width + 1.f);
    const int iy = (int)fminf(fmaxf(floorf(pf.y), -2.f), (float)P.height + 1.f);
#pragma unroll
    for (int i = 0; i < 4; ++i)
        pc[i] = ld3(prev_frame, pix(P, clamp_rx(P, ix + (i & 1)), clamp_ry(P, iy + (i >> 1))));
}

__device__ __forceinline__ f3 taa_history(const Params& P, float2 pf, const f3 (&pc)[4]) {
    const int W = P.width, H = P.height;
    const float flx = floorf(pf.x), fly = floorf(pf.y);
    const int ix = (int)fminf(fmaxf(flx, -2.f), (float)W + 1.f);
    const int iy = (int)fminf(fmaxf(fly, -2.f), (float)H + 1.f);
    f3 prev{0.f, 0.f, 0.f};
    float total = 0.f;
    const float fx = pf.x - flx, fy = pf.y - fly;
    const float omx = 1.f - fx, omy = 1.f - fy;
    const float tw[4] = {omx * omy, fx * omy, omx * fy, fx * fy};
#pragma unroll
    for (int i = 0; i < 4; ++i) {
        const bool okx = (i & 1) ? (ix < W - 1) : (ix >= 0);
        const bool oky = (i >> 1) ? (iy < H - 1) : (iy >= 0);
        if (okx && oky) {
            prev.x = prev.x + tw[i] * pc[i].x;
            prev.y = prev.y + tw[i] * pc[i].y;
            prev.z = prev.z + tw[i] * pc[i].z;
            total = total + tw[i];
        }
    }
    const float rt = 1.f / total;
    prev = f3{div_shared(prev.x, total, rt), div_shared(prev.y, total, rt), div_shared(prev.z, total, rt)};
    return rgb_to_ycocg(prev);
}

__device__ __forceinline__ f3 taa_clamp_tail(const Params& P, f3 me, f3 mnb, f3 mxb, f3 mnc, f3 mxc, f3 py);
__device__ __forceinline__ bool taa_offscreen(const Params& P, float2 pf, int frame) {
    const float flx = floorf(pf.x), fly = floorf(pf.y);
    return frame == 0 || flx < -1.f || fly < -1.f || flx >= (float)P.width || fly >= (float)P.height;
}
template <bool CHECK>
__device__ __forceinline__ f3 taa_clamp(const Params& P, int x, int y, f3 me, float2 pf, const f3 (&nb)[9], f3 py,
                                        int frame) {
    const int W = P.width, H = P.height;
    const float flx = floorf(pf.x), fly = floorf(pf.y);
    if (frame == 0 || flx < -1.f || fly < -1.f || flx >= (float)W || fly >= (float)H)
        return me;
    f3 nlo[9], nhi[9];
#pragma unroll
    for (int k = 0; k < 9; ++k) {
        nlo[k] = nb[k];
        nhi[k] = nb[k];
        if (CHECK) {
            const int sx = x + k % 3 - 1, sy = y + k / 3 - 1;
            const bool in = sx >= 0 && sy >= 0 && sx < W && sy < H;
            nlo[k] = in ? nlo[k] : f3{INFINITY, INFINITY, INFINITY};
            nhi[k] = in ? nhi[k] : f3{-INFINITY, -INFINITY, -INFINITY};
        }
    }
    auto box_cross = [&](auto get, float& mnb_, float& mxb_, float& mnc_, float& mxc_) {
        const float inf = INFINITY;
        float m = vmin3s(inf, get(nlo[0]), get(nlo[1]));
        m = vmin3(m, get(nlo[2]), get(nlo[3]));
        m = vmin3(m, get(nlo[4]), get(nlo[5]));
        m = vmin3(m, get(nlo[6]), get(nlo[7]));
        mnb_ = vmin(m, get(nlo[8]));
        float M = vmax3s(-inf, get(nhi[0]), get(nhi[1]));
        M = vmax3(M, get(nhi[2]), get(nhi[3]));
        M = vmax3(M, get(nhi[4]), get(nhi[5]));
        M = vmax3(M, get(nhi[6]), get(nhi[7]));
        mxb_ = vmax(M, get(nhi[8]));
        mnc_ = vmin(vmin3(vmin3s(inf, get(nlo[1]), get(nlo[3])), get(nlo[4]), get(nlo[5])), get(nlo[7]));
        mxc_ = vmax(vmax3(vmax3s(-inf, get(nhi[1]), get(nhi[3])), get(nhi[4]), get(nhi[5])), get(nhi[7]));
    };
    f3 mnb, mxb, mnc, mxc;
    box_cross([](const f3& v) { return v.x; }, mnb.x, mxb.x, mnc.x, mxc.x);
    box_cross([](const f3& v) { return v.y; }, mnb.y, mxb.y, mnc.y, mxc.y);
    box_cross([](const f3& v) { return v.z; }, mnb.z, mxb.z, mnc.z, mxc.z);
    return taa_clamp_tail(P, me, mnb, mxb, mnc, mxc, py);
}

__device__ __forceinline__ f3 taa_clamp_tail(const Params& P, f3 me, f3 mnb, f3 mxb, f3 mnc, f3 mxc, f3 py) {
    const f3 lo{(mnb.x + mnc.x) / 2.f, (mnb.y + mnc.y) / 2.f, (mnb.z + mnc.z) / 2.f};
    const f3 hi{(mxb.x + mxc.x) / 2.f, (mxb.y + mxc.y) / 2.f, (mxb.z + mxc.z) / 2.f};
// ... 14 lines not shown
```

### bmfr_amd/csrc/bmfr_kernels.hip

```cpp
#include "bmfr_kernels.h"
#include "bmfr_generic.h"
#include "bmfr_launch.h"

namespace bmfr {

__global__ __launch_bounds__(256) void k_accumulate_noisy(Params P, NoisyInputs in, Camera cam,
                                                          int frame, int pass, float2* prev_pixel,
                                                          uint8_t* accept, float* noisy_out,
                                                          uint8_t* spp_cur, void* tmp) {
    const int gx = blockIdx.x * blockDim.x + threadIdx.x;
    const int gy = blockIdx.y * blockDim.y + threadIdx.y;
    if (gx >= P.margins_w || gy >= P.margins_h) return;
    const int2 off = kBlockOffsets[frame & 15];
    const int ux = gx - kEdge / 2 + off.x, uy = gy - kEdge / 2 + off.y;
    const bool owner = ux >= 0 && ux < P.width && uy >= 0 && uy < P.height;
    if ((int)owner != pass) return;

    const NoisyItem it = noisy_item(P, in, cam, gx, gy, frame);
    spp_cur[it.lin] = it.spp;
    const int bx = gx / kEdge, by = gy / kEdge;
    const size_t base = ((size_t)by * P.blocks_x + bx) * (size_t)P.buffers * kBlockPixels +
                        (size_t)(gy % kEdge) * kEdge + (gx % kEdge);
    for (int f = 0; f < P.buffers; ++f) {
        const float v = design_value(P, f, it);
        if (P.half_tmp) ((_Float16*)tmp)[base + (size_t)f * kBlockPixels] = (_Float16)v;
        else ((float*)tmp)[base + (size_t)f * kBlockPixels] = v;
    }
    if (it.owner) {
        st3(noisy_out, it.lin, it.color);
        prev_pixel[it.lin] = make_float2(it.pfx, it.pfy);
        accept[it.lin] = it.accept;
    }
}

__device__ __forceinline__ int block_of_pixel(const Params& P, int x, int y, int frame) {
    const int2 off = kBlockOffsets[frame & 15];
    return (x + kEdge / 2 - off.x) / kEdge + ((y + kEdge / 2 - off.y) / kEdge) * P.blocks_x;
}

__global__ __launch_bounds__(256) void k_weighted_sum(Params P, const float* __restrict__ weights,
                                                      const float* __restrict__ mins_maxs,
                                                      float* __restrict__ out,
                                                      const float* __restrict__ normals,
                                                      const float* __restrict__ positions, int frame) {
    const int x = blockIdx.x * blockDim.x + threadIdx.x;
    const int y = blockIdx.y * blockDim.y + threadIdx.y;
    if (x >= P.width || y >= P.height) return;
    const uint32_t lin = (uint32_t)(y * P.width + x);
    const int g = block_of_pixel(P, x, y, frame);
    const f3 c = weighted_color(P, weights + (size_t)g * (P.buffers - 3) * 3,
                                mins_maxs + (size_t)g * P.scaled * 2, ld3(normals, lin),
                                ld3(positions, lin));
    st3(out, lin, c);
}

__global__ __launch_bounds__(256) void k_accumulate_filtered(
    Params P, const float* __restrict__ filtered, const float2* __restrict__ prev_pixel,
    const uint8_t* __restrict__ accept, const float* __restrict__ albedo,
    float* __restrict__ tone_mapped, const uint8_t* __restrict__ spp,
    const float* __restrict__ acc_prev, float* __restrict__ acc, int frame) {
    const int x = blockIdx.x * blockDim.x + threadIdx.x;
    const int y = blockIdx.y * blockDim.y + threadIdx.y;
    if (x >= P.width || y >= P.height) return;
    const uint32_t lin = (uint32_t)(y * P.width + x);
    const float2 pp = prev_pixel[lin];
    const f3 a = blend_filtered(P, ld3(filtered, lin), pp.x, pp.y, frame > 0 ? accept[lin] : 0, spp[lin],
                                acc_prev, frame);
    st3(acc, lin, a);
    st3(tone_mapped, lin, tone_map(P, ld3(albedo, lin), a));
}

__global__ __launch_bounds__(256) void k_taa(Params P, const float2* __restrict__ prev_pixel,
                                             const float* __restrict__ new_frame,
                                             float* __restrict__ result,
                                             const float* __restrict__ prev_frame, int frame) {
    const int x = blockIdx.x * blockDim.x + threadIdx.x;
    const int y = blockIdx.y * blockDim.y + threadIdx.y;
    if (x >= P.width || y >= P.height) return;
    const uint32_t lin = (uint32_t)(y * P.width + x);
    const f3 me = ld3(new_frame, lin);
    const float2 pf = prev_pixel[lin];
    f3 pc[4], nb[9];
    taa_load_taps(P, pf, prev_frame, pc);
#pragma unroll
    for (int k = 0; k < 9; ++k)
        nb[k] = rgb_to_ycocg(ld3(new_frame, pix(P, clamp_rx(P, x + k % 3 - 1), clamp_ry(P, y + k / 3 - 1))));
    st3(result, lin, taa_resolve<true>(P, x, y, me, pf, nb, pc, frame));
}

constexpr int kTaaW = 64, kTaaH = 12;
constexpr int kTaaNT = kTileThreads;
constexpr int kTaaMinWaves = 6;
template <class IN>
__global__ __launch_bounds__(kTaaNT, kTaaMinWaves) void k_fused_taa(Params P, TaaArgs T) {
    __shared__ float4 Y[(kTaaW + 2) * (kTaaH + 2)];
    __shared__ double sE[kPowrENum];
    __shared__ double2 sRP[kPowrRPNum];
    const int G = gridDim.x * gridDim.y;
    const int gi = G - 1 - xcd_swizzle(blockIdx.y * gridDim.x + blockIdx.x, G);
    const int bxi = gi % gridDim.x, byi = gi / gridDim.x;
    forward_reach(T, blockIdx.x == 0 && blockIdx.y == 0);
    taa_tile<IN, kTaaH, false>(P, T, P.tx0 + bxi * kTaaW, P.ty0 + byi * kTaaH, Y, sE, sRP);
}

__global__ __launch_bounds__(256) void k_halo_copy(HaloArgs a, uint8_t* __restrict__ buf, int unpack) {
    const HaloSeg& s = a.seg[blockIdx.y];
    uint8_t* plane = reinterpret_cast<uint8_t*>(s.plane);
    uint8_t* packed = buf + s.buf_off;
    const long total = (long)s.row_bytes * s.rows;
    const bool words = (s.row_bytes & 3) == 0 && (s.pitch & 3) == 0 && (s.plane & 3) == 0;
    const long stride = (long)gridDim.x * blockDim.x;
    if (words) {
        const int rw = s.row_bytes >> 2;
        for (long i = blockIdx.x * (long)blockDim.x + threadIdx.x; i < total / 4; i += stride) {
            const long row = i / rw, col = i % rw;
            uint32_t* p = reinterpret_cast<uint32_t*>(plane + row * s.pitch) + col;
            uint32_t* q = reinterpret_cast<uint32_t*>(packed) + i;
            if (unpack) *p = *q;
            else *q = *p;
        }
    } else {
        for (long i = blockIdx.x * (long)blockDim.x + threadIdx.x; i < total; i += stride) {
            const long row = i / s.row_bytes, col = i % s.row_bytes;
            uint8_t* p = plane + row * s.pitch + col;
            if (unpack) *p = packed[i];
            else packed[i] = *p;
        }
    }
}

hipError_t launch_halo_copy(const HaloArgs& a, hipStream_t st, void* buf, int unpack) {
    if (a.nseg <= 0) return hipSuccess;
    hipLaunchKernelGGL(k_halo_copy, dim3(64, a.nseg), dim3(256), 0, st, a, static_cast<uint8_t*>(buf), unpack);
    return hipGetLastError();
}

__global__ __launch_bounds__(256) void k_noise_table(int first, int frames, int buffers, float* __restrict__ table) {
    const int per_frame = (buffers - 4) * kBlockPixels;
    const int i = blockIdx.x * blockDim.x + threadIdx.x;
    if (i >= frames * per_frame) return;
    const int frame = first + i / per_frame, j = i % per_frame;
    const int fb = 1 + j / kBlockPixels, r = j % kBlockPixels;
    table[i] = hash_random((uint32_t)(r + fb * kBlockPixels + frame * buffers * kBlockPixels)) - 0.5f;
}

namespace {
dim3 grid2d(int w, int h, dim3 blk) { return dim3((w + blk.x - 1) / blk.x, (h + blk.y - 1) / blk.y); }
}

hipError_t launch_accumulate_noisy(const Params& P, hipStream_t st, float2* prev_pixel, uint8_t* accept,
                                   const NoisyInputs& in, float* noisy_out, uint8_t* spp_cur, void* tmp,
                                   const Camera& cam, int frame) {
    const dim3 blk(16, 16);
    const dim3 grd = grid2d(P.margins_w, P.margins_h, blk);
    for (int pass = 0; pass < 2; ++pass) {
        hipLaunchKernelGGL(k_accumulate_noisy, grd, blk, 0, st, P, in, cam, frame, pass, prev_pixel,
                           accept, noisy_out, spp_cur, tmp);
    }
    return hipGetLastError();
}

bool fitter_supported(int ns, int fs) { return ns >= 1 && ns <= 4 && fs >= 0 && fs <= 9; }

hipError_t launch_fitter(const Params& P, hipStream_t st, float* weights, float* mins_maxs, void* tmp,
                         int frame) {
    switch (P.not_scaled) {
        case 1: return launch_fitter_ns<1>(P, st, weights, mins_maxs, tmp, frame);
        case 2: return launch_fitter_ns<2>(P, st, weights, mins_maxs, tmp, frame);
        case 3: return launch_fitter_ns<3>(P, st, weights, mins_maxs, tmp, frame);
        case 4: return launch_fitter_ns<4>(P, st, weights, mins_maxs, tmp, frame);
        default: return hipErrorInvalidValue;
    }
}

hipError_t launch_fused_generic(const Params& P, hipStream_t st, const FusedArgs& A) {
    if (aux_mask(P) != 0) {
        switch (P.not_scaled) {
            case 1: return launch_fused_block_aux_ns<1>(P, st, A);
            case 2: return launch_fused_block_aux_ns<2>(P, st, A);
            case 3: return launch_fused_block_aux_ns<3>(P, st, A);
            case 4: return launch_fused_block_aux_ns<4>(P, st, A);
            default: return hipErrorInvalidValue;
        }
    }
    switch (P.not_scaled) {
        case 1: return launch_fused_block_ns<1>(P, st, A);
        case 2: return launch_fused_block_ns<2>(P, st, A);
        case 3: return launch_fused_block_ns<3>(P, st, A);
        case 4: return launch_fused_block_ns<4>(P, st, A);
        default: return hipErrorInvalidValue;
    }
}

hipError_t launch_weighted_sum(const Params& P, hipStream_t st, const float* weights,
                               const float* mins_maxs, float* out, const float* normals,
                               const float* positions, int frame) {
    const dim3 blk(64, 4);
    hipLaunchKernelGGL(k_weighted_sum, grid2d(P.width, P.height, blk), blk, 0, st, P, weights,
                       mins_maxs, out, normals, positions, frame);
    return hipGetLastError();
}

hipError_t launch_accumulate_filtered(const Params& P, hipStream_t st, const float* filtered,
                                      const float2* prev_pixel, const uint8_t* accept,
                                      const float* albedo, float* tone, const uint8_t* spp,
                                      const float* acc_prev, float* acc, int frame) {
    const dim3 blk(64, 4);
    hipLaunchKernelGGL(k_accumulate_filtered, grid2d(P.width, P.height, blk), blk, 0, st, P, filtered,
                       prev_pixel, accept, albedo, tone, spp, acc_prev, acc, frame);
    return hipGetLastError();
}

hipError_t launch_taa(const Params& P, hipStream_t st, const float2* prev_pixel, const float* new_frame,
                      float* result, const float* prev_frame, int frame) {
    const dim3 blk(64, 4);
    hipLaunchKernelGGL(k_taa, grid2d(P.width, P.height, blk), blk, 0, st, P, prev_pixel, new_frame,
                       result, prev_frame, frame);
    return hipGetLastError();
}

hipError_t launch_noise_tables(const Params& P, hipStream_t st, int first, int frames, float* table) {
    const int n = frames * (P.buffers - 4) * kBlockPixels;
    hipLaunchKernelGGL(k_noise_table, dim3((n + 255) / 256), dim3(256), 0, st, first, frames, P.buffers, table);
    return hipGetLastError();
}

hipError_t launch_noise_table(const Params& P, hipStream_t st, const FusedArgs& A) {
    return launch_noise_tables(P, st, A.frame, 1, A.noise_table);
}

hipError_t launch_fused_k1_blocks(const Params& P, hipStream_t st, const FusedArgs& A) {
    if (P.nbx <= 0 || P.nby <= 0 || P.ring < 0) return hipSuccess;
    return fused_cols_supported(P) ? launch_fused_k1_cols(P, st, A) : launch_fused_k1(P, st, A);
}

hipError_t launch_fused_k2(const Params& P, hipStream_t st, const FusedArgs& A) {
    const dim3 grd((P.tx1 - P.tx0 + kTaaW - 1) / kTaaW, (P.ty1 - P.ty0 + kTaaH - 1) / kTaaH);
    if (P.input_half) hipLaunchKernelGGL((k_fused_taa<_Float16>), grd, dim3(kTaaNT), 0, st, P, taa_args(A));
    else hipLaunchKernelGGL((k_fused_taa<float>), grd, dim3(kTaaNT), 0, st, P, taa_args(A));
    return hipGetLastError();
}

hipError_t launch_fused_frame(const Params& P, hipStream_t st, const FusedArgs& A, hipEvent_t mid) {
    hipError_t e;
    const bool one = P.frame_launches == 1 || (P.frame_launches == 0 && k1_blocks(P) < kTwoLaunchBlocks);
    if (!mid && A.done && frame_fused_supported(P) && one) return launch_fused_frame_one(P, st, A);
    if (fused_supported(P)) {
        if ((e = launch_fused_k1_blocks(P, st, A)) != hipSuccess) return e;
        if (mid) (void)hipEventRecord(mid, st);
        return launch_fused_k2(P, st, A);
    }
    e = launch_fused_generic(P, st, A);
    if (e != hipSuccess) return e;
    if (mid) (void)hipEventRecord(mid, st);
    return launch_taa(P, st, A.prev_pixel_out, A.tone_out, A.result_out, A.result_prev, A.frame);
}

}
```

### bmfr_amd/csrc/bmfr_launch.h

```cpp
#pragma once

#include <hip/hip_runtime.h>

#include "bmfr_kernels.h"
#include "bmfr_taa_tile.h"

namespace bmfr {

struct HaloSeg {
    unsigned long long plane;
    long long buf_off;
    int row_bytes, rows, pitch;
};
constexpr int kMaxHaloSegs = 64;
struct HaloArgs {
    HaloSeg seg[kMaxHaloSegs];
    int nseg;
};
hipError_t launch_halo_copy(const HaloArgs& a, hipStream_t st, void* buf, int unpack);

struct FusedArgs {
    NoisyInputs in;
    Camera cam;
    int frame;
    const float* albedo;
    const float* acc_prev;
    const float* result_prev;
    float* noisy_out;
    uint8_t* spp_out;
    float2* prev_pixel_out;
    float* acc_out;
    float* tone_out;
    float* result_out;
    float* noise_table;
    unsigned* reach;
    unsigned* reach_host;
    unsigned long long* stamps;
    unsigned* done;
    unsigned epoch;
    unsigned* sync_err;
    const float2* prev_pixel_in;
    AuxPlanes aux;
};

struct K1Args {
    NoisyInputs in;
    Camera cam;
    int frame;
    const float* acc_prev;
    float* noisy_out;
    uint8_t* spp_out;
    float2* prev_pixel_out;
    float* acc_out;
    const float* noise;
    unsigned* reach;
    unsigned long long* stamps;
    unsigned* done;
    unsigned epoch;
    unsigned* sync_err;
    const float2* prev_pixel_in;
};
inline K1Args k1_args(const FusedArgs& A) {
    return K1Args{A.in,      A.cam,         A.frame, A.acc_prev, A.noisy_out, A.spp_out,  A.prev_pixel_out, A.acc_out,
                  A.noise_table, A.reach,   A.stamps, A.done,    A.epoch,     A.sync_err, A.prev_pixel_in};
}
inline TaaArgs taa_args(const FusedArgs& A) {
    return TaaArgs{A.acc_out, A.albedo, A.prev_pixel_out, A.result_out, A.result_prev, A.frame, A.reach,
                   A.reach_host, A.done, A.epoch, A.sync_err};
}

bool fitter_supported(int not_scaled, int scaled);
inline int k1_blocks(const Params& P) { return P.ring > 0 ? P.ring : P.nbx * P.nby; }
constexpr int kTwoLaunchBlocks = 4096;
bool fused_supported(const Params& P);
hipError_t launch_fused_k1(const Params& P, hipStream_t st, const FusedArgs& A);
bool fused_cols_supported(const Params& P);
hipError_t launch_fused_k1_cols(const Params& P, hipStream_t st, const FusedArgs& A);

hipError_t launch_accumulate_noisy(const Params& P, hipStream_t st, float2* prev_pixel, uint8_t* accept,
                                   const NoisyInputs& in, float* noisy_out, uint8_t* spp_cur, void* tmp,
                                   const Camera& cam, int frame);
hipError_t launch_fitter(const Params& P, hipStream_t st, float* weights, float* mins_maxs, void* tmp,
                         int frame);
hipError_t launch_weighted_sum(const Params& P, hipStream_t st, const float* weights,
                               const float* mins_maxs, float* out, const float* normals,
                               const float* positions, int frame);
hipError_t launch_accumulate_filtered(const Params& P, hipStream_t st, const float* filtered,
                                      const float2* prev_pixel, const uint8_t* accept,
                                      const float* albedo, float* tone, const uint8_t* spp,
                                      const float* acc_prev, float* acc, int frame);
hipError_t launch_fused_frame(const Params& P, hipStream_t st, const FusedArgs& A, hipEvent_t mid = nullptr);
hipError_t launch_fused_generic(const Params& P, hipStream_t st, const FusedArgs& A);
hipError_t launch_noise_table(const Params& P, hipStream_t st, const FusedArgs& A);
constexpr int kNoiseFrames = 64;
hipError_t launch_noise_tables(const Params& P, hipStream_t st, int first, int frames, float* table);
hipError_t launch_fused_k1_blocks(const Params& P, hipStream_t st, const FusedArgs& A);
bool seq_fused_supported(const Params& P);
bool frame_fused_supported(const Params& P);
hipError_t launch_fused_frame_one(const Params& P, hipStream_t st, const FusedArgs& A);
hipError_t launch_fused_rows_frame_one(const Params& P, hipStream_t st, const FusedArgs& A);
hipError_t launch_fused_k1_taa(const Params& P, hipStream_t st, const FusedArgs* A, const Params& P2,
                               const FusedArgs* A2);
hipError_t launch_fused_k2(const Params& P, hipStream_t st, const FusedArgs& A);
hipError_t launch_taa(const Params& P, hipStream_t st, const float2* prev_pixel, const float* new_frame,
                      float* result, const float* prev_frame, int frame);

}
```

### bmfr_amd/csrc/bmfr_taa_tile.h

```cpp
#pragma once

#include "bmfr_kernels.h"

namespace bmfr {

struct TaaArgs {
    const float* src;
    const float* albedo;
    const float2* prev_pixel;
    float* result;
    const float* prev_frame;
    int frame;
    unsigned* reach_dev;
    unsigned* reach_host;
    const unsigned* done;
    unsigned epoch;
    unsigned* sync_err;
};

constexpr int kSyncPivot = 0, kSyncTile = 1;
constexpr unsigned kDoneTimeout = 0x80000000u;
__device__ __forceinline__ void report_sync_timeout(unsigned* err, int which, int frame) {
    if (err) {
        __hip_atomic_store(err + which, (unsigned)frame + 1u, __ATOMIC_RELAXED, __HIP_MEMORY_SCOPE_SYSTEM);
        __threadfence_system();
    }
}

__device__ __forceinline__ void wait_done(const Params& P, const TaaArgs& T, const unsigned* f) {
    const int limit = 4 * P.max_polls;
    for (int k = 0;; ++k) {
        const unsigned v = __hip_atomic_load(f, __ATOMIC_RELAXED, __HIP_MEMORY_SCOPE_AGENT);
        if ((v & ~kDoneTimeout) >= T.epoch) {
            if (v & kDoneTimeout) report_sync_timeout(T.sync_err, kSyncPivot, T.frame);
            return;
        }
        if (k >= limit) {
            report_sync_timeout(T.sync_err, kSyncTile, T.frame);
            return;
        }
        __builtin_amdgcn_s_sleep(2);
    }
}

__device__ __forceinline__ bool k1_in_launch(const Params& P, int bx, int by) {
    if (P.ring <= 0) return P.ring == 0;
    return bx < P.rx0 || bx >= P.rx1 || by < P.ry0 || by >= P.ry1;
}

__device__ __forceinline__ void wait_k1_blocks(const Params& P, const TaaArgs& T, int x0, int y0, int th) {
    const int2 off = kBlockOffsets[T.frame & 15];
    const int xa = max(x0 - 1, P.ox), xb = min(min(x0 + 64, P.tx1), P.ox + P.stride - 1);
    const int ya = max(y0 - 1, P.oy), yb = min(min(y0 + th, P.ty1), P.oy + P.rows - 1);
    const int bxa = (xa + kEdge / 2 - off.x) / kEdge, bxb = (xb + kEdge / 2 - off.x) / kEdge;
    const int bya = (ya + kEdge / 2 - off.y) / kEdge, byb = (yb + kEdge / 2 - off.y) / kEdge;
    const int nx = bxb - bxa + 1, n = nx * (byb - bya + 1);
    const int t = threadIdx.x;
    if (t < n) {
        const int bx = bxa + t % nx, by = bya + t / nx;
        if (k1_in_launch(P, bx, by)) wait_done(P, T, T.done + (by - P.by0) * P.nbx + (bx - P.bx0));
    }
    __syncthreads();
}

__device__ __forceinline__ void wait_all_k1_blocks(const Params& P, const TaaArgs& T) {
    for (int i = threadIdx.x; i < P.nbx * P.nby; i += blockDim.x) {
        const int bx = P.bx0 + i % P.nbx, by = P.by0 + i / P.nbx;
        if (k1_in_launch(P, bx, by)) wait_done(P, T, T.done + i);
    }
    __syncthreads();
}

__device__ __forceinline__ void forward_reach(const TaaArgs& T, bool here = true) {
    if (T.reach_dev && here && threadIdx.x == 0) {
        const unsigned v = atomicExch(T.reach_dev, 0u);
        volatile unsigned* h = T.reach_host;
        if (v > h[0]) h[0] = v;
        __threadfence_system();
        h[1] = (unsigned)T.frame + 1u;
        __threadfence_system();
    }
}

constexpr int kTileThreads = 256;

template <int TH>
struct TileShape {
    static constexpr int RP = kTileThreads / 64;
    static_assert(TH % RP == 0 && TH >= RP, "tile height");
    static constexpr int HW = 64 + 2, HH = TH + 2, N = HW * HH;
    static constexpr int RING = N - 64 * TH;
    static constexpr int KN = TH / RP;
    static_assert(RING <= kTileThreads, "one ring pixel per thread");
    static __device__ __forceinline__ int row(int ty, int k) { return ty * KN + k; }
};

template <class IN, int KN>
struct TileLoads {
    float2 pf[KN];
    f3 v[KN + 1];
    In3<IN> al[KN + 1];
};

template <int TH>
__device__ __forceinline__ void ring_pixel(int t, int& hx, int& hy) {
    using S = TileShape<TH>;
    if (t < 2 * S::HW) {
        hx = t % S::HW;
        hy = t < S::HW ? 0 : S::HH - 1;
    } else {
        hx = t < 2 * S::HW + TH ? 0 : S::HW - 1;
        hy = 1 + (t - 2 * S::HW) % TH;
    }
}

template <class IN, int TH, bool COH>
__device__ __forceinline__ void tile_issue(const Params& P, const TaaArgs& T, int x0, int y0, int hx, int hy,
                                           TileLoads<IN, TileShape<TH>::KN>& L) {
    using S = TileShape<TH>;
    const int t = threadIdx.x, tx = t & 63, ty = t >> 6;
    const CohPlane c_pp = coh_plane(T.prev_pixel), c_src = coh_plane(T.src);
#pragma unroll
    for (int k = 0; k < S::KN; ++k) {
        const uint32_t i = pix(P, min(x0 + tx, P.tx1 - 1), min(y0 + S::row(ty, k), P.ty1 - 1));
        if constexpr (COH) L.pf[k] = ld2_coh(c_pp, i);
        else L.pf[k] = ld_px(T.prev_pixel, i);
    }
#pragma unroll
    for (int k = 0; k <= S::KN; ++k) {
        const int lx = k < S::KN ? tx + 1 : hx, ly = k < S::KN ? S::row(ty, k) + 1 : hy;
        if (k == S::KN && t >= S::RING) break;
        const uint32_t lin = pix(P, clamp_rx(P, x0 - 1 + lx), clamp_ry(P, y0 - 1 + ly));
        if constexpr (COH) L.v[k] = ld3_coh(c_src, lin);
        else L.v[k] = ld3(T.src, lin);
        L.al[k] = ld3raw<IN>(T.albedo, lin);
    }
}

template <class IN, int TH>
__device__ __forceinline__ void tile_tone(const Params& P, const TileLoads<IN, TileShape<TH>::KN>& L, int hx,
                                          int hy, float4* __restrict__ Y, const double* __restrict__ sE,
                                          const double2* __restrict__ sRP, f3 (&me)[TileShape<TH>::KN]) {
    using S = TileShape<TH>;
    const int t = threadIdx.x, tx = t & 63, ty = t >> 6;
    uint32_t rare = 0;
    auto put = [&](int k, const f3& v) {
        const int lx = k < S::KN ? tx + 1 : hx, ly = k < S::KN ? S::row(ty, k) + 1 : hy;
        if (k < S::KN) me[k] = v;
        const f3 yc = rgb_to_ycocg(v);
        Y[ly * S::HW + lx] = make_float4(yc.x, yc.y, yc.z, 0.f);
    };
    if (P.library_powr) {
#pragma unroll
        for (int k = 0; k <= S::KN; ++k) {
            if (k == S::KN && t >= S::RING) break;
            put(k, tone_map(P, widen(L.al[k]), L.v[k], sE, sRP));
        }
    } else {
#pragma unroll
        for (int k = 0; k <= S::KN; ++k) {
            if (k == S::KN && t >= S::RING) break;
            const f3 a = widen(L.al[k]);
            const float p[3] = {a.x * L.v[k].x, a.y * L.v[k].y, a.z * L.v[k].z};
            float g[3];
            uint32_t r;
            gamma_table3(p, g, r, sE, sRP);
            rare |= (r != 0 ? 1u : 0u) << k;
            put(k, f3{g[0], g[1], g[2]});
        }
    }
    if (__builtin_expect(rare != 0, 0)) {
#pragma unroll
        for (int k = 0; k <= S::KN; ++k)
            if (rare & (1u << k)) put(k, tone_map(P, widen(L.al[k]), L.v[k], sE, sRP));
    }
}

template <int KN>
__device__ __forceinline__ void tile_taps(const Params& P, const TaaArgs& T, const float2 (&pf)[KN],
                                          f3 (&taps)[KN][4]) {
#pragma unroll
    for (int k = 0; k < KN; ++k) taa_load_taps(P, pf[k], T.prev_frame, taps[k]);
}

template <int TH, bool CHECK>
__device__ __forceinline__ void resolve_strip(const Params& P, const TaaArgs& T, int x0, int y0,
                                              const float4* __restrict__ Y, const f3 (&me)[TileShape<TH>::KN],
                                              const float2 (&pf)[TileShape<TH>::KN],
                                              const f3 (&hist)[TileShape<TH>::KN]) {
    using S = TileShape<TH>;
    const int t = threadIdx.x, tx = t & 63, ty = t >> 6;
    const int r0 = S::row(ty, 0);
    struct Row {
        f3 mn, mx;
        f3 clo, chi;
    };
    auto reduce_row = [&](int r) {
        f3 lo[3], hi[3];
#pragma unroll
        for (int dx = 0; dx < 3; ++dx) {
            const float4 q = Y[(r0 + r) * S::HW + tx + dx];
            lo[dx] = hi[dx] = f3{q.x, q.y, q.z};
            if constexpr (CHECK) {
                const int sx = x0 + tx + dx - 1, sy = y0 + r0 + r - 1;
                const bool in = sx >= 0 && sy >= 0 && sx < P.width && sy < P.height;
                lo[dx] = in ? lo[dx] : f3{INFINITY, INFINITY, INFINITY};
                hi[dx] = in ? hi[dx] : f3{-INFINITY, -INFINITY, -INFINITY};
            }
        }
        Row w;
        w.mn = f3{vmin3(lo[0].x, lo[1].x, lo[2].x), vmin3(lo[0].y, lo[1].y, lo[2].y), vmin3(lo[0].z, lo[1].z, lo[2].z)};
        w.mx = f3{vmax3(hi[0].x, hi[1].x, hi[2].x), vmax3(hi[0].y, hi[1].y, hi[2].y), vmax3(hi[0].z, hi[1].z, hi[2].z)};
        w.clo = lo[1];
        w.chi = hi[1];
        return w;
    };
    auto mn4 = [](float a, float b, float c) { return vmin(vmin3s(INFINITY, a, b), c); };
    auto mx4 = [](float a, float b, float c) { return vmax(vmax3s(-INFINITY, a, b), c); };
    Row w0 = reduce_row(0), w1 = reduce_row(1);
#pragma unroll
    for (int k = 0; k < S::KN; ++k) {
        const Row w2 = reduce_row(k + 2);
        const int x = x0 + tx, y = y0 + r0 + k;
        if (x < P.tx1 && y < P.ty1) {
            f3 r = me[k];
            if (!taa_offscreen(P, pf[k], T.frame)) {
                const f3 mnb{mn4(w0.mn.x, w1.mn.x, w2.mn.x), mn4(w0.mn.y, w1.mn.y, w2.mn.y),
                             mn4(w0.mn.z, w1.mn.z, w2.mn.z)};
                const f3 mxb{mx4(w0.mx.x, w1.mx.x, w2.mx.x), mx4(w0.mx.y, w1.mx.y, w2.mx.y),
                             mx4(w0.mx.z, w1.mx.z, w2.mx.z)};
                const f3 mnc{mn4(w0.clo.x, w1.mn.x, w2.clo.x), mn4(w0.clo.y, w1.mn.y, w2.clo.y),
                             mn4(w0.clo.z, w1.mn.z, w2.clo.z)};
                const f3 mxc{mx4(w0.chi.x, w1.mx.x, w2.chi.x), mx4(w0.chi.y, w1.mx.y, w2.chi.y),
                             mx4(w0.chi.z, w1.mx.z, w2.chi.z)};
                r = taa_clamp_tail(P, me[k], mnb, mxb, mnc, mxc, hist[k]);
            }
            st3(T.result, pix(P, x, y), r);
        }
        w0 = w1;
        w1 = w2;
    }
}

template <int TH>
__device__ __forceinline__ void tile_resolve(const Params& P, const TaaArgs& T, int x0, int y0,
                                             const float4* __restrict__ Y, const f3 (&me)[TileShape<TH>::KN],
                                             const float2 (&pf)[TileShape<TH>::KN],
                                             const f3 (&hist)[TileShape<TH>::KN]) {
    const bool edge = x0 == 0 || y0 == 0 || x0 + 64 >= P.width || y0 + TH >= P.height;
    if (edge) resolve_strip<TH, true>(P, T, x0, y0, Y, me, pf, hist);
    else resolve_strip<TH, false>(P, T, x0, y0, Y, me, pf, hist);
}

template <class IN, int TH, bool COH = false>
__device__ __forceinline__ void taa_tile(const Params& P, const TaaArgs& T, int x0, int y0, float4* __restrict__ Y,
                                         double* __restrict__ sE, double2* __restrict__ sRP) {
    using S = TileShape<TH>;
    constexpr int KN = S::KN;
    const int t = threadIdx.x;
    bmfr_powr_tables_to_lds<kTileThreads>(sE, sRP, t);
    if constexpr (COH) wait_k1_blocks(P, T, x0, y0, TH);
    int hx = 0, hy = 0;
    ring_pixel<TH>(t, hx, hy);
    TileLoads<IN, KN> L;
    tile_issue<IN, TH, COH>(P, T, x0, y0, hx, hy, L);
    __syncthreads();
    f3 me[KN];
    tile_tone<IN, TH>(P, L, hx, hy, Y, sE, sRP, me);
    f3 taps[KN][4];
    tile_taps<KN>(P, T, L.pf, taps);
    __syncthreads();
    f3 hist[KN];
#pragma unroll
    for (int k = 0; k < KN; ++k) hist[k] = taa_history(P, L.pf[k], taps[k]);
    tile_resolve<TH>(P, T, x0, y0, Y, me, L.pf, hist);
}

constexpr int kFrameTaaH = 16;
struct FrameTaaLds {
    float4 Y[(64 + 2) * (kFrameTaaH + 2)];
    double sE[kPowrENum];
    double2 sRP[kPowrRPNum];
};
template <class IN, bool COH>
__device__ __forceinline__ void frame_taa_part(const Params& P2, const TaaArgs& T, int b, int nk1p, FrameTaaLds& L) {
    constexpr int TH = kFrameTaaH;
    const int gx = (P2.tx1 - P2.tx0 + 63) / 64, n2 = (int)gridDim.x - nk1p;
    const int gi = xcd_swizzle(b - nk1p, n2);
    taa_tile<IN, TH, COH>(P2, T, P2.tx0 + (gi % gx) * 64, P2.ty0 + (gi / gx) * TH, L.Y, L.sE, L.sRP);
    if constexpr (COH) {
        if (T.reach_dev && b == (int)gridDim.x - 1) {
            wait_all_k1_blocks(P2, T);
            forward_reach(T);
        }
    }
}
inline int frame_taa_tiles(const Params& P) {
    constexpr int TH = kFrameTaaH;
    return ((P.tx1 - P.tx0 + 63) / 64) * ((P.ty1 - P.ty0 + TH - 1) / TH);
}

}
```

### bmfr_amd/pipeline.py

```python
from __future__ import annotations

import ctypes as C
import dataclasses

import torch

from . import _lib
from ._lib import check, floats

NOT_SCALED_DEFAULT = (_lib.FEATURE_ONE, _lib.NORMAL_X, _lib.NORMAL_Y, _lib.NORMAL_Z)
SCALED_DEFAULT = (_lib.POSITION_X, _lib.POSITION_Y, _lib.POSITION_Z,
                  _lib.POSITION_X2, _lib.POSITION_Y2, _lib.POSITION_Z2)
SCALED_THIRD_ORDER = SCALED_DEFAULT + (_lib.POSITION_X3, _lib.POSITION_Y3, _lib.POSITION_Z3)


@dataclasses.dataclass(frozen=True)
class BmfrConfig:
    image_width: int = 1280
    image_height: int = 720
    not_scaled: tuple = NOT_SCALED_DEFAULT
    scaled: tuple = SCALED_DEFAULT
    noise_amount: float = 1e-2
    blend_alpha: float = 0.2
    second_blend_alpha: float = 0.1
    taa_blend_alpha: float = 0.2
    position_limit_squared: float = 0.01
    normal_limit_squared: float = 0.1
    use_half_precision_in_tmp_data: int = 1
    tile: tuple | None = None
    tile_halo: int = 0
    input_half: int = 0
    library_powr: int = 0
    fast_fit: int = 0

    @property
    def buffer_count(self) -> int:
        return len(self.not_scaled) + len(self.scaled) + 3

    def to_c(self) -> _lib.Config:
        lib = _lib.load()
        c = _lib.Config()
        lib.bmfr_config_default(C.byref(c), self.image_width, self.image_height)
        feats = tuple(self.not_scaled) + tuple(self.scaled)
        c.features_not_scaled = len(self.not_scaled)
        c.features_scaled = len(self.scaled)
        for i in range(_lib.MAX_FEATURES):
            c.feature_buffers[i] = feats[i] if i < len(feats) else 0
        c.noise_amount = self.noise_amount
        c.blend_alpha = self.blend_alpha
        c.second_blend_alpha = self.second_blend_alpha
        c.taa_blend_alpha = self.taa_blend_alpha
        c.position_limit_squared = self.position_limit_squared
        c.normal_limit_squared = self.normal_limit_squared
        c.use_half_precision_in_tmp_data = self.use_half_precision_in_tmp_data
        if self.tile is not None:
            c.tile_x, c.tile_y, c.tile_width, c.tile_height = self.tile
            c.tile_halo = self.tile_halo
        c.input_half = self.input_half
        c.library_powr = self.library_powr
        c.fast_fit = self.fast_fit
        return c

    def sizes(self) -> _lib.Sizes:
        s = _lib.Sizes()
        check(_lib.load().bmfr_config_sizes(C.byref(self.to_c()), C.byref(s)), "bmfr_config_sizes")
        return s


def _ptr(t) -> int | None:
    return None if t is None else t.data_ptr()


def check_prev_pixel(plane, width: int, height: int, device: int = 0) -> None:
    if plane is None:
        return
    if not isinstance(plane, torch.Tensor):
        raise TypeError(f"prev_pixel must be a torch tensor or None, not {type(plane).__name__}")
    if plane.dtype != torch.float32:
        raise TypeError(f"prev_pixel must be float32 (also with input_half), not {plane.dtype}")
    if tuple(plane.shape) not in ((height, width, 2), (height * width * 2,)):
        raise ValueError(f"prev_pixel must have shape ({height}, {width}, 2) or ({height * width * 2},), "
                         f"not {tuple(plane.shape)}")
    if not plane.is_contiguous():
        raise ValueError("prev_pixel must be contiguous")
    if plane.device.type != "cuda" or (plane.device.index or 0) != device:
        raise ValueError(f"prev_pixel must live on cuda:{device}, not {plane.device}")


def aux_named(cfg: "BmfrConfig") -> tuple:
    feats = tuple(cfg.not_scaled) + tuple(cfg.scaled)
    return tuple(k for k in range(_lib.MAX_AUX_FEATURES) if _lib.FEATURE_AUX0 + k in feats)


def check_aux(aux, named, width: int, height: int, device: int = 0) -> tuple:
    if aux is None:
        aux = ()
    if isinstance(aux, torch.Tensor) or not hasattr(aux, "__len__"):
        raise TypeError("aux must be a sequence of up to four tensors or Nones")
    if len(aux) > _lib.MAX_AUX_FEATURES:
        raise ValueError(f"aux takes at most {_lib.MAX_AUX_FEATURES} planes, not {len(aux)}")
    planes = tuple(aux) + (None,) * (_lib.MAX_AUX_FEATURES - len(aux))
    for k in named:
        if planes[k] is None:
            raise ValueError(f"the feature list names FEATURE_AUX{k} but aux[{k}] is missing")
    for k, t in enumerate(planes):
        if t is None:
            continue
        if not isinstance(t, torch.Tensor):
            raise TypeError(f"aux[{k}] must be a torch tensor or None, not {type(t).__name__}")
        if t.dtype != torch.float32:
            raise TypeError(f"aux[{k}] must be float32, not {t.dtype}")
        if t.numel() != height * width:
            raise ValueError(f"aux[{k}] must have {height * width} elements ({height} x {width}), "
                             f"not {tuple(t.shape)}")
        if not t.is_contiguous():
            raise ValueError(f"aux[{k}] must be contiguous")
        if t.device.type != "cuda" or (t.device.index or 0) != device:
            raise ValueError(f"aux[{k}] must live on cuda:{device}, not {t.device}")
    return planes


def _stream(stream) -> int | None:
    s = stream if stream is not None else torch.cuda.current_stream()
    return s.cuda_stream


class _Context:
    def __init__(self, cfg: BmfrConfig, device: int = 0):
        self.cfg = cfg
        self.lib = _lib.load()
        self.device = device
        h = C.c_void_p()
        check(self.lib.bmfr_create(C.byref(cfg.to_c()), device, C.byref(h)), "bmfr_create")
        self.handle = h
        self.sizes = cfg.sizes()

    def close(self) -> None:
        if self.handle:
            self.lib.bmfr_destroy(self.handle)
            self.handle = None

    def __del__(self):
        try:
            self.close()
        except Exception:
            pass


class StagePipeline(_Context):
# ... 566 lines not shown
```

### include/bmfr.h

```cpp
#ifndef BMFR_H
#define BMFR_H

#include <stddef.h>
#include <stdint.h>

#ifdef __cplusplus
extern "C" {
#endif

#define BMFR_VERSION_MAJOR 0
#define BMFR_VERSION_MINOR 3

#define BMFR_BLOCK_EDGE_LENGTH 32
#define BMFR_MAX_FEATURES 16
#define BMFR_MAX_AUX_FEATURES 4

typedef enum bmfr_status {
    BMFR_OK = 0,
    BMFR_ERROR_INVALID_ARGUMENT = 1,
    BMFR_ERROR_UNSUPPORTED = 2,
    BMFR_ERROR_OUT_OF_MEMORY = 3,
    BMFR_ERROR_HIP = 4,
    BMFR_ERROR_NO_DEVICE = 5,
    BMFR_ERROR_HALO_EXCEEDED = 6,
// ... 105 lines not shown
    const float prev_frame_camera_matrix[16], const float pixel_offset[2], int frame_number);

bmfr_status bmfr_process_frame_interior(bmfr_ctx *ctx, void *stream, const bmfr_frame_inputs *in,
    const float prev_frame_camera_matrix[16], const float pixel_offset[2], int frame_number);
bmfr_status bmfr_process_frame_border(bmfr_ctx *ctx, void *stream, const bmfr_frame_inputs *in,
    const float prev_frame_camera_matrix[16], const float pixel_offset[2], int frame_number);

bmfr_status bmfr_process_sequence(bmfr_ctx *ctx, void *stream, int count, const bmfr_frame_inputs *in,
    const float *prev_frame_camera_matrices, const float *pixel_offsets, int first_frame,
    float *const *outputs);

bmfr_status bmfr_process_frame_aux(bmfr_ctx *ctx, void *stream, const bmfr_frame_inputs *in,
    const bmfr_aux_inputs *aux, const float prev_frame_camera_matrix[16], const float pixel_offset[2],
    int frame_number);
bmfr_status bmfr_process_frame_interior_aux(bmfr_ctx *ctx, void *stream, const bmfr_frame_inputs *in,
    const bmfr_aux_inputs *aux, const float prev_frame_camera_matrix[16], const float pixel_offset[2],
    int frame_number);
bmfr_status bmfr_process_frame_border_aux(bmfr_ctx *ctx, void *stream, const bmfr_frame_inputs *in,
    const bmfr_aux_inputs *aux, const float prev_frame_camera_matrix[16], const float pixel_offset[2],
    int frame_number);
bmfr_status bmfr_process_sequence_aux(bmfr_ctx *ctx, void *stream, int count, const bmfr_frame_inputs *in,
    const bmfr_aux_inputs *aux, const float *prev_frame_camera_matrices, const float *pixel_offsets,
    int first_frame, float *const *outputs);

typedef enum bmfr_format {
    BMFR_FORMAT_NONE = 0,
    BMFR_FORMAT_F32X3,
    BMFR_FORMAT_F16X4,
    BMFR_FORMAT_UNORM8X4,
    BMFR_FORMAT_OCT_SNORM16X2,
    BMFR_FORMAT_F32X2,
    BMFR_FORMAT_F16X2,
    BMFR_FORMAT_UNORM8X3,
    BMFR_FORMAT_UNORM10X3A2
} bmfr_format;

typedef struct bmfr_gbuffer {
    const void *radiance;
    int radiance_format;
    const void *albedo;
    int albedo_format;
    float albedo_floor;
    const void *normals;
    int normal_format;
    const float *positions;
    const float *depth;
    float inv_view_proj[16];
    const void *motion;
    int motion_format;
    float motion_scale[2];
    int motion_at_pixel_centre;
    const void *prev_positions;
    const void *prev_normals;
    const uint16_t *prev_object_id;
    const float *object_transforms;
    int n_objects;
} bmfr_gbuffer;

typedef struct bmfr_prepared {
    void *noisy;
    void *normals;
    void *positions;
    void *albedo;
    float *prev_pixel;
    void *prev_positions_moved;
    void *prev_normals_moved;
} bmfr_prepared;

void bmfr_gbuffer_default(bmfr_gbuffer *g);
bmfr_status bmfr_prepare_frame(bmfr_ctx *ctx, void *stream, const bmfr_gbuffer *g,
    const bmfr_prepared *out, const float pixel_offset[2]);

#define BMFR_HALO_NOISY 1
#define BMFR_HALO_SPP 2
#define BMFR_HALO_FILTERED 4
#define BMFR_HALO_RESULT 8
#define BMFR_HALO_STATE (BMFR_HALO_NOISY | BMFR_HALO_SPP | BMFR_HALO_FILTERED)
#define BMFR_HALO_ALL (BMFR_HALO_STATE | BMFR_HALO_RESULT)
bmfr_status bmfr_halo_copy(bmfr_ctx *ctx, void *stream, const int *rects, int n, void *buffer, int unpack,
    size_t *bytes);

bmfr_status bmfr_halo_need(const bmfr_config *cfg, int frame_number, int state_rect[4], int result_rect[4]);

bmfr_status bmfr_halo_plan(const bmfr_config *cfg, const int *tiles, int ntiles, int rank, int frame_number,
    int *peers, int *send_counts, int *recv_counts, int *records, int max_records, int *n_peers);

typedef struct bmfr_comm bmfr_comm;
bmfr_status bmfr_comm_unique_id(unsigned char id[128]);
bmfr_status bmfr_comm_create(const unsigned char id[128], int nranks, int rank, int hip_device, bmfr_comm **out);
bmfr_status bmfr_comm_create_all(int ndev, const int *devices, bmfr_comm **out);
bmfr_status bmfr_comm_destroy(bmfr_comm *comm);

typedef struct bmfr_exchange bmfr_exchange;
bmfr_status bmfr_exchange_create(bmfr_ctx *ctx, const bmfr_config *cfg, const int *tiles, int ntiles, int rank,
    bmfr_comm *comm, bmfr_exchange **out);
bmfr_status bmfr_exchange_run(bmfr_exchange *x, void *stream, int frame_number);
bmfr_status bmfr_exchange_run_all(bmfr_exchange *const *xs, int n, void *const *streams, int frame_number);
bmfr_status bmfr_exchange_bytes(const bmfr_exchange *x, int frame_number, size_t *sent, size_t *received);
bmfr_status bmfr_exchange_destroy(bmfr_exchange *x);

bmfr_status bmfr_halo_status(bmfr_ctx *ctx, unsigned *overshoot);

bmfr_status bmfr_frame_status(bmfr_ctx *ctx);

const float *bmfr_output(const bmfr_ctx *ctx);

typedef struct bmfr_state_view {
    float *noisy_accumulated;
    uint8_t *spp;
    float *filtered_accumulated;
    float *tone_mapped;
    float *prev_frame_pixel;
    uint8_t *accept;
    float *result;
} bmfr_state_view;
bmfr_status bmfr_state(const bmfr_ctx *ctx, int previous, bmfr_state_view *out);

typedef struct bmfr_surface {
    void  *data;
    int    format;
    size_t pitch;
    int    width, height;
    int    origin_x, origin_y;
    int    flip_y;
    int    bgr;
    float  alpha;
} bmfr_surface;
typedef enum bmfr_resolve_source { BMFR_RESOLVE_OUTPUT = 0, BMFR_RESOLVE_HDR = 1 } bmfr_resolve_source;

void bmfr_surface_default(bmfr_surface *s);
bmfr_status bmfr_resolve_output(bmfr_ctx *ctx, void *stream, int source,
                                const void *albedo, const bmfr_surface *dst);

typedef struct bmfr_upsample_guides {
    int width, height;
    const void *albedo;   int albedo_format;
    const void *normals;  int normal_format;
    const float *positions;
    const float *depth;
    float inv_view_proj[16];
    float pixel_offset[2];
    float plane_limit_squared;
    float normal_limit_squared;
} bmfr_upsample_guides;
typedef enum bmfr_upsample_source { BMFR_UPSAMPLE_HDR = 0, BMFR_UPSAMPLE_TONEMAPPED = 1 } bmfr_upsample_source;

void bmfr_upsample_guides_default(bmfr_upsample_guides *g, const bmfr_config *cfg);
bmfr_status bmfr_upsample_output(bmfr_ctx *ctx, void *stream, int source,
    const void *frame_normals, const void *frame_positions,
    const bmfr_upsample_guides *g, const bmfr_surface *dst, uint32_t *stats );

typedef struct bmfr_plane { void *data; int format; size_t pitch; } bmfr_plane;

typedef struct bmfr_display_taa_args {
    int width, height;
    bmfr_plane current;
    bmfr_plane history;
    bmfr_plane result;
    const float *prev_pixel;
    const void *motion; int motion_format;
    float motion_scale[2]; int motion_at_pixel_centre; float pixel_offset[2];
    float blend_alpha;
    int reset;
} bmfr_display_taa_args;

void bmfr_display_taa_default(bmfr_display_taa_args *a, const bmfr_config *cfg);
// ... 40 lines not shown
```

Before: 0.3337.

## Add untiled kernel specializations with compile-time params and per-frame block ranges

Adds template specializations of the fused rows/cols and TAA kernels for the untiled (single-tile) case, using a ParamsView/UntiledParams type so tile origin, stride and ring fields become compile-time constants or drop out. For untiled configs, per-frame block ranges are now computed from the jittered block offset, so blocks that fall entirely outside the image are not launched. A dedicated untiled TAA kernel and a bmfr_frame_blocks query API are also added. The aim is fewer wasted blocks and cheaper address arithmetic and register use on the common single-GPU path, in exchange for more kernel instantiations and a longer build.

```diff
diff --git a/bmfr_amd/_build.py b/bmfr_amd/_build.py
--- a/bmfr_amd/_build.py
+++ b/bmfr_amd/_build.py
@@ -12,6 +12,9 @@
 HIPCC = os.environ.get("HIPCC", "/opt/rocm/bin/hipcc")
 SOURCES = ["bmfr_kernels.hip", "bmfr_fused.hip", "bmfr_fused_cols.hip", "bmfr_fused_cols_f32.hip", "bmfr_capi.hip",
            "bmfr_fused_plane.hip", "bmfr_fused_cols_plane.hip", "bmfr_fused_cols_f32_plane.hip",
+           "bmfr_fused_untiled.hip", "bmfr_fused_cols_untiled.hip", "bmfr_fused_cols_f32_untiled.hip",
+           "bmfr_fused_plane_untiled.hip", "bmfr_fused_cols_plane_untiled.hip",
+           "bmfr_fused_cols_f32_plane_untiled.hip", "bmfr_taa_untiled.hip",
            "bmfr_exchange.hip", "bmfr_prepare.hip", "bmfr_resolve.hip", "bmfr_firefly.hip",
            "bmfr_upsample.hip", "bmfr_display_taa.hip", "bmfr_synth.hip",
            "bmfr_generic_ns1.hip", "bmfr_generic_ns2.hip", "bmfr_generic_ns3.hip", "bmfr_generic_ns4.hip",
diff --git a/bmfr_amd/_lib.py b/bmfr_amd/_lib.py
--- a/bmfr_amd/_lib.py
+++ b/bmfr_amd/_lib.py
@@ -180,6 +180,7 @@
     "bmfr_suppress_fireflies": (_I, [_P, _P, _P, _P, C.POINTER(FireflyParams), _P]),
     "bmfr_halo_copy": (_I, [_P, _P, C.POINTER(C.c_int), _I, _P, _I, C.POINTER(C.c_size_t)]),
     "bmfr_halo_need": (_I, [C.POINTER(Config), _I, C.POINTER(C.c_int), C.POINTER(C.c_int)]),
+    "bmfr_frame_blocks": (_I, [C.POINTER(Config), _I, C.POINTER(C.c_int)]),
     "bmfr_process_sequence": (_I, [_P, _P, _I, C.POINTER(FrameInputs), _F16, _F2, _I, C.POINTER(_P)]),
     "bmfr_process_frame_border": (_I, [_P, _P, C.POINTER(FrameInputs), _F16, _F2, _I]),
     "bmfr_process_frame_aux": (_I, [_P, _P, C.POINTER(FrameInputs), C.POINTER(AuxInputs), _F16, _F2, _I]),
diff --git a/bmfr_amd/csrc/bmfr_capi.hip b/bmfr_amd/csrc/bmfr_capi.hip
--- a/bmfr_amd/csrc/bmfr_capi.hip
+++ b/bmfr_amd/csrc/bmfr_capi.hip
@@ -166,24 +166,32 @@
     return P;
 }
 
+void block_range(int lo, int hi, int off, int nblocks, int& b0, int& nb) {
+    const int E = BMFR_BLOCK_EDGE_LENGTH;
+    b0 = -1;
+    nb = 0;
+    for (int b = 0; b < nblocks; ++b) {
+        const int p0 = E * b - E / 2 + off, p1 = p0 + E;
+        if (p0 < hi && p1 > lo) {
+            if (b0 < 0) b0 = b;
+            nb = b - b0 + 1;
+        }
+    }
+}
+
+Params frame_params_untiled(Params P, int frame) {
+    block_range(0, P.width, bmfr::kBlockOffsetTable[frame & 15][0], P.blocks_x, P.bx0, P.nbx);
+    block_range(0, P.height, bmfr::kBlockOffsetTable[frame & 15][1], P.blocks_y, P.by0, P.nby);
+    return P;
+}
+
 Params frame_params_cfg(const bmfr_config& g, Params P, int frame) {
     const int E = BMFR_BLOCK_EDGE_LENGTH;
     const int ox = bmfr::kBlockOffsetTable[frame & 15][0], oy = bmfr::kBlockOffsetTable[frame & 15][1];
-    auto range = [&](int lo, int hi, int off, int nblocks, int& b0, int& nb) {
-        b0 = -1;
-        nb = 0;
-        for (int b = 0; b < nblocks; ++b) {
-            const int p0 = E * b - E / 2 + off, p1 = p0 + E;
-            if (p0 < hi && p1 > lo) {
-                if (b0 < 0) b0 = b;
-                nb = b - b0 + 1;
-            }
-        }
-    };
-    range(std::max(0, g.tile_x - 1), std::min(g.image_width, g.tile_x + g.tile_width + 1), ox, P.blocks_x, P.bx0,
-          P.nbx);
-    range(std::max(0, g.tile_y - 1), std::min(g.image_height, g.tile_y + g.tile_height + 1), oy, P.blocks_y,
-          P.by0, P.nby);
+    block_range(std::max(0, g.tile_x - 1), std::min(g.image_width, g.tile_x + g.tile_width + 1), ox, P.blocks_x,
+                P.bx0, P.nbx);
+    block_range(std::max(0, g.tile_y - 1), std::min(g.image_height, g.tile_y + g.tile_height + 1), oy, P.blocks_y,
+                P.by0, P.nby);
     P.tx0 = g.tile_x;
     P.ty0 = g.tile_y;
     P.tx1 = g.tile_x + g.tile_width;
@@ -207,7 +215,7 @@
 }
 
 Params frame_params(const bmfr_ctx* c, int frame) {
-    return is_tiled(&c->cfg) ? frame_params_cfg(c->cfg, c->P, frame) : c->P;
+    return is_tiled(&c->cfg) ? frame_params_cfg(c->cfg, c->P, frame) : frame_params_untiled(c->P, frame);
 }
 
 hipStream_t as_stream(void* s) { return reinterpret_cast<hipStream_t>(s); }
@@ -1292,6 +1300,17 @@
     return BMFR_OK;
 }
 
+bmfr_status bmfr_frame_blocks(const bmfr_config* cfg, int frame_number, int block_rect[4]) {
+    if (!cfg || frame_number < 0 || !block_rect) return BMFR_ERROR_INVALID_ARGUMENT;
+    bmfr_sizes sz;
+    const bmfr_status st = bmfr_config_sizes(cfg, &sz);
+    if (st != BMFR_OK) return st;
+    const Params P0 = make_params(cfg, &sz);
+    const Params P = is_tiled(cfg) ? frame_params_cfg(*cfg, P0, frame_number) : frame_params_untiled(P0, frame_number);
+    block_rect[0] = P.bx0, block_rect[1] = P.by0, block_rect[2] = P.nbx, block_rect[3] = P.nby;
+    return BMFR_OK;
+}
+
 bmfr_status bmfr_set_profiling_stride(bmfr_ctx* c, int stride) {
     if (!c || stride <= 0 || c->pending_frame >= 0) return BMFR_ERROR_INVALID_ARGUMENT;
     c->prof_stride = stride;
diff --git a/bmfr_amd/csrc/bmfr_fused.hip b/bmfr_amd/csrc/bmfr_fused.hip
--- a/bmfr_amd/csrc/bmfr_fused.hip
+++ b/bmfr_amd/csrc/bmfr_fused.hip
@@ -249,8 +249,8 @@
     if (x < B - 3) L.weights[x * 3 + ch] = R[((RE - 1) * RE + x) * 3 + ch];
 }
 
-template <int NS, int FS, class IN, bool COH = false, bool FAST = false, bool PLANE = false>
-__device__ __forceinline__ void k1_rows_body(const Params& P, const K1Args& A, K1Lds<NS + FS + 3>& L, int g) {
+template <int NS, int FS, class IN, bool COH = false, bool FAST = false, bool PLANE = false, class PT>
+__device__ __forceinline__ void k1_rows_body(const PT& P, const K1Args& A, K1Lds<NS + FS + 3>& L, int g) {
     constexpr int B = NS + FS + 3;
     const int t = threadIdx.x;
     const int frame = A.frame;
@@ -362,7 +362,7 @@
         bits[s] = (s < 2 ? state >> (16 * s) : state_hi >> (16 * (s - 2))) & 0xffffu;
         const int px = bx * kEdge + (t3 & (kEdge - 1)) - kEdge / 2 + off.x;
         const int py = by * kEdge + (t3 >> 5) + 8 * s - kEdge / 2 + off.y;
-        lin[s] = pix(P, (bits[s] & 1u) ? px : P.ox, (bits[s] & 1u) ? py : P.oy);
+        lin[s] = pix(P, (bits[s] & 1u) ? px : p_ox(P), (bits[s] & 1u) ? py : p_oy(P));
         n[s] = ld3in<IN>(in.n_cur, lin[s]);
         pos[s] = ld3in<IN>(in.p_cur, lin[s]);
     }
@@ -411,15 +411,15 @@
 }
 
 constexpr int kRowsMinWaves = 4;
-template <int NS, int FS, class IN, bool FAST = false, bool PLANE = false>
-__global__ __launch_bounds__(kThreads, FS == 6 ? kRowsMinWaves : 3) void k_fused(Params P, K1Args A) {
+template <int NS, int FS, class IN, bool FAST = false, bool PLANE = false, bool UNT = false>
+__global__ __launch_bounds__(kThreads, FS == 6 ? kRowsMinWaves : 3) void k_fused(ParamsView<UNT> P, K1Args A) {
     __shared__ K1Lds<NS + FS + 3> L;
     k1_rows_body<NS, FS, IN, false, FAST, PLANE>(P, A, L, xcd_swizzle(blockIdx.x, gridDim.x));
 }
 
 static_assert(kThreads == kTileThreads, "the TAA tiles run on this kernel's work-groups");
-template <int NS, int FS, class IN, bool FAST = false, bool PLANE = false>
-__global__ __launch_bounds__(kThreads, FS == 6 ? kRowsMinWaves : 3) void k_fused_rows_taa(Params P, K1Args A, TaaArgs T, int nk1, int nk1p) {
+template <int NS, int FS, class IN, bool FAST = false, bool PLANE = false, bool UNT = false>
+__global__ __launch_bounds__(kThreads, FS == 6 ? kRowsMinWaves : 3) void k_fused_rows_taa(ParamsView<UNT> P, K1Args A, TaaArgs T, int nk1, int nk1p) {
     __shared__ union {
         K1Lds<NS + FS + 3> k1;
         FrameTaaLds k2;
@@ -432,11 +432,28 @@
 #ifndef BMFR_ROWS_PLANE
 #define BMFR_ROWS_PLANE 0
 #endif
+#ifndef BMFR_ROWS_UNTILED
+#define BMFR_ROWS_UNTILED 0
+#endif
 constexpr bool kRowsPlane = BMFR_ROWS_PLANE;
-hipError_t launch_fused_rows_frame_one_plane(const Params& P, hipStream_t st, const FusedArgs& A);
-hipError_t launch_fused_k1_plane(const Params& P, hipStream_t st, const FusedArgs& A);
-
-#if !BMFR_ROWS_PLANE
+constexpr bool kRowsUntiled = BMFR_ROWS_UNTILED;
+template <bool PLANE, bool UNT>
+hipError_t launch_rows_frame_one(const Params& P, hipStream_t st, const FusedArgs& A);
+template <bool PLANE, bool UNT>
+hipError_t launch_rows_k1(const Params& P, hipStream_t st, const FusedArgs& A);
+#define BMFR_ROWS_UNIT(PLANE, UNT)                                                                   \
+    template <>                                                                                      \
+    hipError_t launch_rows_frame_one<PLANE, UNT>(const Params& P, hipStream_t st, const FusedArgs& A); \
+    template <>                                                                                      \
+    hipError_t launch_rows_k1<PLANE, UNT>(const Params& P, hipStream_t st, const FusedArgs& A);
+BMFR_ROWS_UNIT(false, false)
+BMFR_ROWS_UNIT(true, false)
+BMFR_ROWS_UNIT(false, true)
+BMFR_ROWS_UNIT(true, true)
+#undef BMFR_ROWS_UNIT
+inline ParamsView<kRowsUntiled> rows_view(const Params& P) { return ParamsView<kRowsUntiled>{P}; }
+
+#if !BMFR_ROWS_PLANE && !BMFR_ROWS_UNTILED
 bool fused_supported(const Params& P) {
     if (P.not_scaled != 4 || (P.scaled != 6 && P.scaled != 9)) return false;
     for (int f = 0; f < P.buffers - 3; ++f)
@@ -461,7 +478,8 @@
 template <int FS, class IN, bool FAST>
 struct LaunchK1 {
     static void go(const Params& P, hipStream_t st, const FusedArgs& A) {
-        hipLaunchKernelGGL((k_fused<4, FS, IN, FAST, kRowsPlane>), dim3(k1_blocks(P)), dim3(kThreads), 0, st, P, k1_args(A));
+        hipLaunchKernelGGL((k_fused<4, FS, IN, FAST, kRowsPlane, kRowsUntiled>), dim3(k1_blocks(P)), dim3(kThreads), 0,
+                           st, rows_view(P), k1_args(A));
     }
 };
 
@@ -469,34 +487,35 @@
 struct LaunchRowsFrame {
     static void go(const Params& P, hipStream_t st, const FusedArgs& A) {
         const int nk1 = P.ring < 0 || P.nbx <= 0 || P.nby <= 0 ? 0 : k1_blocks(P), nk1p = (nk1 + 7) & ~7;
-        hipLaunchKernelGGL((k_fused_rows_taa<4, FS, IN, FAST, kRowsPlane>), dim3(nk1p + frame_taa_tiles(P)),
-                           dim3(kThreads), 0, st, P, k1_args(A), taa_args(A), nk1, nk1p);
+        hipLaunchKernelGGL((k_fused_rows_taa<4, FS, IN, FAST, kRowsPlane, kRowsUntiled>),
+                           dim3(nk1p + frame_taa_tiles(P)), dim3(kThreads), 0, st, rows_view(P), k1_args(A), taa_args(A),
+                           nk1, nk1p);
     }
 };
 
 }
 
-#if BMFR_ROWS_PLANE
-hipError_t launch_fused_rows_frame_one_plane(const Params& P, hipStream_t st, const FusedArgs& A) {
+template <>
+hipError_t launch_rows_frame_one<kRowsPlane, kRowsUntiled>(const Params& P, hipStream_t st, const FusedArgs& A) {
     dispatch_rows<LaunchRowsFrame>(P, P, st, A);
     return hipGetLastError();
 }
-
-hipError_t launch_fused_k1_plane(const Params& P, hipStream_t st, const FusedArgs& A) {
+template <>
+hipError_t launch_rows_k1<kRowsPlane, kRowsUntiled>(const Params& P, hipStream_t st, const FusedArgs& A) {
     dispatch_rows<LaunchK1>(P, P, st, A);
     return hipGetLastError();
 }
-#else
+
+#if !BMFR_ROWS_PLANE && !BMFR_ROWS_UNTILED
 hipError_t launch_fused_rows_frame_one(const Params& P, hipStream_t st, const FusedArgs& A) {
-    if (A.prev_pixel_in) return launch_fused_rows_frame_one_plane(P, st, A);
-    dispatch_rows<LaunchRowsFrame>(P, P, st, A);
-    return hipGetLastError();
+    if (untiled(P))
+        return A.prev_pixel_in ? launch_rows_frame_one<true, true>(P, st, A) : launch_rows_frame_one<false, true>(P, st, A);
+    return A.prev_pixel_in ? launch_rows_frame_one<true, false>(P, st, A) : launch_rows_frame_one<false, false>(P, st, A);
 }
 
 hipError_t launch_fused_k1(const Params& P, hipStream_t st, const FusedArgs& A) {
-    if (A.prev_pixel_in) return launch_fused_k1_plane(P, st, A);
-    dispatch_rows<LaunchK1>(P, P, st, A);
-    return hipGetLastError();
+    if (untiled(P)) return A.prev_pixel_in ? launch_rows_k1<true, true>(P, st, A) : launch_rows_k1<false, true>(P, st, A);
+    return A.prev_pixel_in ? launch_rows_k1<true, false>(P, st, A) : launch_rows_k1<false, false>(P, st, A);
 }
 #endif
 
diff --git a/bmfr_amd/csrc/bmfr_fused_cols.hip b/bmfr_amd/csrc/bmfr_fused_cols.hip
--- a/bmfr_amd/csrc/bmfr_fused_cols.hip
+++ b/bmfr_amd/csrc/bmfr_fused_cols.hip
@@ -652,8 +652,8 @@
 }
 
 
-template <int NS, int FS, class IN, bool COH = false, bool FAST = false, bool F32 = false, bool PLANE = false>
-__device__ __forceinline__ void k1_cols_body(const Params& P, const K1Args& A, Lds<NS + FS + 3, F32>& L, int g) {
+template <int NS, int FS, class IN, bool COH = false, bool FAST = false, bool F32 = false, bool PLANE = false, class PT>
+__device__ __forceinline__ void k1_cols_body(const PT& P, const K1Args& A, Lds<NS + FS + 3, F32>& L, int g) {
     constexpr int B = NS + FS + 3;
     constexpr bool FASTR = FAST && !F32;
     using P2 = Pair<F32>;
@@ -775,7 +775,7 @@
     for (int i = 0; i < NI; ++i) {
         const int px = bx * kEdge + (l3 & (kEdge - 1)) - kEdge / 2 + off.x;
         const int py = by * kEdge + item_row(l3, i) - kEdge / 2 + off.y;
-        lin[i] = pix(P, (ibits & (1u << i)) ? px : P.ox, (ibits & (1u << i)) ? py : P.oy);
+        lin[i] = pix(P, (ibits & (1u << i)) ? px : p_ox(P), (ibits & (1u << i)) ? py : p_oy(P));
         if constexpr (kKeepNP) {
             keep_np[i].get(nrm_r[i], wp_r[i]);
         } else {
@@ -882,15 +882,17 @@
     return F32 && FS == 9 ? 3 : 4;
 }
 
-template <int NS, int FS, class IN, bool FAST = false, bool F32 = false, bool PLANE = false>
-__global__ __launch_bounds__(kK1Threads, (min_waves<FS, F32>())) void k_fused_cols(Params P, K1Args A) {
+template <int NS, int FS, class IN, bool FAST = false, bool F32 = false, bool PLANE = false, bool UNT = false>
+__global__ __launch_bounds__(kK1Threads, (min_waves<FS, F32>())) void k_fused_cols(ParamsView<UNT> P, K1Args A) {
     __shared__ Lds<NS + FS + 3, F32> L;
     k1_cols_body<NS, FS, IN, false, FAST, F32, PLANE>(P, A, L, xcd_swizzle(blockIdx.x, gridDim.x));
 }
 
-template <int NS, int FS, class IN, bool SAME = false, bool FAST = false, bool F32 = false, bool PLANE = false>
-__global__ __launch_bounds__(kK1Threads, (min_waves<FS, F32>())) void k_fused_cols_taa(Params P, K1Args A, Params P2,
-                                                                                    TaaArgs T, int nk1, int nk1p) {
+template <int NS, int FS, class IN, bool SAME = false, bool FAST = false, bool F32 = false, bool PLANE = false,
+          bool UNT = false>
+__global__ __launch_bounds__(kK1Threads, (min_waves<FS, F32>())) void k_fused_cols_taa(ParamsView<UNT> P, K1Args A,
+                                                                                    ParamsView<UNT> P2, TaaArgs T,
+                                                                                    int nk1, int nk1p) {
     __shared__ union {
         Lds<NS + FS + 3, F32> k1;
         FrameTaaLds k2;
@@ -902,13 +904,27 @@
 
 }
 
-template <bool F32, bool PLANE>
+template <bool F32, bool PLANE, bool UNT>
 hipError_t launch_cols_k1(const Params& P, hipStream_t st, const FusedArgs& A);
-template <bool F32, bool PLANE>
+template <bool F32, bool PLANE, bool UNT>
 hipError_t launch_cols_frame_one(const Params& P, hipStream_t st, const FusedArgs& A);
 template <bool F32>
 hipError_t launch_cols_k1_taa(const Params& P, hipStream_t st, const FusedArgs* A, const Params& P2,
                               const FusedArgs* A2);
+#define BMFR_COLS_UNIT(F32, PLANE, UNT)                                                                   \
+    template <>                                                                                           \
+    hipError_t launch_cols_k1<F32, PLANE, UNT>(const Params& P, hipStream_t st, const FusedArgs& A);       \
+    template <>                                                                                           \
+    hipError_t launch_cols_frame_one<F32, PLANE, UNT>(const Params& P, hipStream_t st, const FusedArgs& A);
+BMFR_COLS_UNIT(false, false, false)
+BMFR_COLS_UNIT(true, false, false)
+BMFR_COLS_UNIT(false, true, false)
+BMFR_COLS_UNIT(true, true, false)
+BMFR_COLS_UNIT(false, false, true)
+BMFR_COLS_UNIT(true, false, true)
+BMFR_COLS_UNIT(false, true, true)
+BMFR_COLS_UNIT(true, true, true)
+#undef BMFR_COLS_UNIT
 
 #ifndef BMFR_COLS_F32
 #define BMFR_COLS_F32 0
@@ -916,8 +932,13 @@
 #ifndef BMFR_COLS_PLANE
 #define BMFR_COLS_PLANE 0
 #endif
+#ifndef BMFR_COLS_UNTILED
+#define BMFR_COLS_UNTILED 0
+#endif
 constexpr bool kColsF32 = BMFR_COLS_F32;
 constexpr bool kColsPlane = BMFR_COLS_PLANE;
+constexpr bool kColsUntiled = BMFR_COLS_UNTILED;
+inline ParamsView<kColsUntiled> cols_view(const Params& P) { return ParamsView<kColsUntiled>{P}; }
 
 namespace {
 
@@ -943,8 +964,8 @@
 template <int FS, class IN, bool FAST>
 struct LaunchCols {
     static void go(const Params& P, hipStream_t st, const FusedArgs& A) {
-        hipLaunchKernelGGL((cols::k_fused_cols<4, FS, IN, FAST, kColsF32, kColsPlane>), dim3(k1_blocks(P)),
-                           dim3(cols::kK1Threads), 0, st, P, k1_args(A));
+        hipLaunchKernelGGL((cols::k_fused_cols<4, FS, IN, FAST, kColsF32, kColsPlane, kColsUntiled>),
+                           dim3(k1_blocks(P)), dim3(cols::kK1Threads), 0, st, cols_view(P), k1_args(A));
     }
 };
 
@@ -953,12 +974,13 @@
     static void go(const Params& P, hipStream_t st, const FusedArgs& A) {
         const int nk1 = P.ring < 0 || P.nbx <= 0 || P.nby <= 0 ? 0 : k1_blocks(P), nk1p = (nk1 + 7) & ~7;
         const int nk2 = frame_taa_tiles(P);
-        hipLaunchKernelGGL((cols::k_fused_cols_taa<4, FS, IN, true, FAST, kColsF32, kColsPlane>), dim3(nk1p + nk2),
-                           dim3(cols::kK1Threads), 0, st, P, k1_args(A), P, taa_args(A), nk1, nk1p);
+        hipLaunchKernelGGL((cols::k_fused_cols_taa<4, FS, IN, true, FAST, kColsF32, kColsPlane, kColsUntiled>),
+                           dim3(nk1p + nk2), dim3(cols::kK1Threads), 0, st, cols_view(P), k1_args(A), cols_view(P),
+                           taa_args(A), nk1, nk1p);
     }
 };
 
-#if !BMFR_COLS_PLANE
+#if !BMFR_COLS_PLANE && !BMFR_COLS_UNTILED
 template <int FS, class IN, bool FAST>
 struct LaunchColsTaa {
     static void go(const Params& P, hipStream_t st, const FusedArgs* A, const Params& P2, const FusedArgs* A2) {
@@ -976,16 +998,17 @@
 }
 
 template <>
-hipError_t launch_cols_k1<kColsF32, kColsPlane>(const Params& P, hipStream_t st, const FusedArgs& A) {
+hipError_t launch_cols_k1<kColsF32, kColsPlane, kColsUntiled>(const Params& P, hipStream_t st, const FusedArgs& A) {
     if (!dispatch_cols<LaunchCols>(P, P, st, A)) return hipErrorInvalidValue;
     return hipGetLastError();
 }
 template <>
-hipError_t launch_cols_frame_one<kColsF32, kColsPlane>(const Params& P, hipStream_t st, const FusedArgs& A) {
+hipError_t launch_cols_frame_one<kColsF32, kColsPlane, kColsUntiled>(const Params& P, hipStream_t st,
+                                                                     const FusedArgs& A) {
     if (!dispatch_cols<LaunchFrameOne>(P, P, st, A)) return hipErrorInvalidValue;
     return hipGetLastError();
 }
-#if !BMFR_COLS_PLANE
+#if !BMFR_COLS_PLANE && !BMFR_COLS_UNTILED
 template <>
 hipError_t launch_cols_k1_taa<kColsF32>(const Params& P, hipStream_t st, const FusedArgs* A, const Params& P2,
                                         const FusedArgs* A2) {
@@ -994,30 +1017,38 @@
 }
 #endif
 
-template <>
-hipError_t launch_cols_k1<!kColsF32, kColsPlane>(const Params& P, hipStream_t st, const FusedArgs& A);
-template <>
-hipError_t launch_cols_k1<kColsF32, !kColsPlane>(const Params& P, hipStream_t st, const FusedArgs& A);
-template <>
-hipError_t launch_cols_k1<!kColsF32, !kColsPlane>(const Params& P, hipStream_t st, const FusedArgs& A);
-template <>
-hipError_t launch_cols_frame_one<!kColsF32, kColsPlane>(const Params& P, hipStream_t st, const FusedArgs& A);
-template <>
-hipError_t launch_cols_frame_one<kColsF32, !kColsPlane>(const Params& P, hipStream_t st, const FusedArgs& A);
-template <>
-hipError_t launch_cols_frame_one<!kColsF32, !kColsPlane>(const Params& P, hipStream_t st, const FusedArgs& A);
-
-#if !BMFR_COLS_F32 && !BMFR_COLS_PLANE
+#if !BMFR_COLS_F32 && !BMFR_COLS_PLANE && !BMFR_COLS_UNTILED
 bool fused_cols_supported(const Params& P) { return (P.half_tmp || P.fast_fit) && fused_supported(P); }
 
 bool seq_fused_supported(const Params& P) { return fused_cols_supported(P) && P.ring == 0; }
 bool frame_fused_supported(const Params& P) { return fused_supported(P); }
 
+template <template <bool, bool, bool> class L>
+hipError_t pick_cols_unit(const Params& P, hipStream_t st, const FusedArgs& A) {
+    const bool f32 = !P.half_tmp, plane = A.prev_pixel_in != nullptr;
+    if (untiled(P)) {
+        if (plane) return f32 ? L<true, true, true>::go(P, st, A) : L<false, true, true>::go(P, st, A);
+        return f32 ? L<true, false, true>::go(P, st, A) : L<false, false, true>::go(P, st, A);
+    }
+    if (plane) return f32 ? L<true, true, false>::go(P, st, A) : L<false, true, false>::go(P, st, A);
+    return f32 ? L<true, false, false>::go(P, st, A) : L<false, false, false>::go(P, st, A);
+}
+template <bool F32, bool PLANE, bool UNT>
+struct UnitFrameOne {
+    static hipError_t go(const Params& P, hipStream_t st, const FusedArgs& A) {
+        return launch_cols_frame_one<F32, PLANE, UNT>(P, st, A);
+    }
+};
+template <bool F32, bool PLANE, bool UNT>
+struct UnitK1 {
+    static hipError_t go(const Params& P, hipStream_t st, const FusedArgs& A) {
+        return launch_cols_k1<F32, PLANE, UNT>(P, st, A);
+    }
+};
+
 hipError_t launch_fused_frame_one(const Params& P, hipStream_t st, const FusedArgs& A) {
     if (!fused_cols_supported(P)) return launch_fused_rows_frame_one(P, st, A);
-    if (A.prev_pixel_in)
-        return P.half_tmp ? launch_cols_frame_one<false, true>(P, st, A) : launch_cols_frame_one<true, true>(P, st, A);
-    return P.half_tmp ? launch_cols_frame_one<false, false>(P, st, A) : launch_cols_frame_one<true, false>(P, st, A);
+    return pick_cols_unit<UnitFrameOne>(P, st, A);
 }
 
 hipError_t launch_fused_k1_taa(const Params& P, hipStream_t st, const FusedArgs* A, const Params& P2,
@@ -1027,9 +1058,8 @@
 }
 
 hipError_t launch_fused_k1_cols(const Params& P, hipStream_t st, const FusedArgs& A) {
-    if (A.prev_pixel_in) return P.half_tmp ? launch_cols_k1<false, true>(P, st, A) : launch_cols_k1<true, true>(P, st, A);
-    return P.half_tmp ? launch_cols_k1<false, false>(P, st, A) : launch_cols_k1<true, false>(P, st, A);
-}
-#endif
-
-}
+    return pick_cols_unit<UnitK1>(P, st, A);
+}
+#endif
+
+}
diff --git a/bmfr_amd/csrc/bmfr_fused_cols_f32_plane_untiled.hip b/bmfr_amd/csrc/bmfr_fused_cols_f32_plane_untiled.hip
--- /dev/null
+++ b/bmfr_amd/csrc/bmfr_fused_cols_f32_plane_untiled.hip
@@ -0,0 +1,4 @@
+#define BMFR_COLS_F32 1
+#define BMFR_COLS_PLANE 1
+#define BMFR_COLS_UNTILED 1
+#include "bmfr_fused_cols.hip"
diff --git a/bmfr_amd/csrc/bmfr_fused_cols_f32_untiled.hip b/bmfr_amd/csrc/bmfr_fused_cols_f32_untiled.hip
--- /dev/null
+++ b/bmfr_amd/csrc/bmfr_fused_cols_f32_untiled.hip
@@ -0,0 +1,3 @@
+#define BMFR_COLS_F32 1
+#define BMFR_COLS_UNTILED 1
+#include "bmfr_fused_cols.hip"
diff --git a/bmfr_amd/csrc/bmfr_fused_cols_plane_untiled.hip b/bmfr_amd/csrc/bmfr_fused_cols_plane_untiled.hip
--- /dev/null
+++ b/bmfr_amd/csrc/bmfr_fused_cols_plane_untiled.hip
@@ -0,0 +1,3 @@
+#define BMFR_COLS_PLANE 1
+#define BMFR_COLS_UNTILED 1
+#include "bmfr_fused_cols.hip"
diff --git a/bmfr_amd/csrc/bmfr_fused_cols_untiled.hip b/bmfr_amd/csrc/bmfr_fused_cols_untiled.hip
--- /dev/null
+++ b/bmfr_amd/csrc/bmfr_fused_cols_untiled.hip
@@ -0,0 +1,2 @@
+#define BMFR_COLS_UNTILED 1
+#include "bmfr_fused_cols.hip"
diff --git a/bmfr_amd/csrc/bmfr_fused_plane_untiled.hip b/bmfr_amd/csrc/bmfr_fused_plane_untiled.hip
--- /dev/null
+++ b/bmfr_amd/csrc/bmfr_fused_plane_untiled.hip
@@ -0,0 +1,3 @@
+#define BMFR_ROWS_PLANE 1
+#define BMFR_ROWS_UNTILED 1
+#include "bmfr_fused.hip"
diff --git a/bmfr_amd/csrc/bmfr_fused_untiled.hip b/bmfr_amd/csrc/bmfr_fused_untiled.hip
--- /dev/null
+++ b/bmfr_amd/csrc/bmfr_fused_untiled.hip
@@ -0,0 +1,2 @@
+#define BMFR_ROWS_UNTILED 1
+#include "bmfr_fused.hip"
diff --git a/bmfr_amd/csrc/bmfr_kernels.h b/bmfr_amd/csrc/bmfr_kernels.h
--- a/bmfr_amd/csrc/bmfr_kernels.h
+++ b/bmfr_amd/csrc/bmfr_kernels.h
@@ -1,4 +1,6 @@
 #pragma once
+
+#include <type_traits>
 
 #include "bmfr_device.h"
 #include "bmfr_powr.h"
@@ -101,8 +103,29 @@
     return xcd < rem ? xcd * (per + 1) + k : rem * (per + 1) + (xcd - rem) * per + k;
 }
 
-__device__ __forceinline__ void k1_block(const Params& P, int g, int& bx, int& by) {
-    if (P.ring == 0) {
+struct UntiledParams : Params {};
+template <bool UNT>
+using ParamsView = std::conditional_t<UNT, UntiledParams, Params>;
+template <class PT>
+constexpr bool kUntiled = std::is_same_v<PT, UntiledParams>;
+#define BMFR_VIEW(name, field, untiled_value)                                         \
+    __device__ __forceinline__ int name(const Params& P) { return P.field; }          \
+    __device__ __forceinline__ int name(const UntiledParams& P) { return untiled_value; }
+BMFR_VIEW(p_ox, ox, 0)
+BMFR_VIEW(p_oy, oy, 0)
+BMFR_VIEW(p_stride, stride, P.width)
+BMFR_VIEW(p_rows, rows, P.height)
+BMFR_VIEW(p_check_reach, check_reach, 0)
+BMFR_VIEW(p_ring, ring, 0)
+BMFR_VIEW(p_tx0, tx0, 0)
+BMFR_VIEW(p_ty0, ty0, 0)
+BMFR_VIEW(p_tx1, tx1, P.width)
+BMFR_VIEW(p_ty1, ty1, P.height)
+#undef BMFR_VIEW
+
+template <class PT>
+__device__ __forceinline__ void k1_block(const PT& P, int g, int& bx, int& by) {
+    if (p_ring(P) == 0) {
         bx = P.bx0 + g % P.nbx;
         by = P.by0 + g / P.nbx;
         return;
@@ -127,11 +150,18 @@
     by = P.ry1 + g / W;
 }
 
-__device__ __forceinline__ uint32_t pix(const Params& P, int x, int y) {
-    return __umul24((uint32_t)(y - P.oy), (uint32_t)P.stride) + (uint32_t)(x - P.ox);
-}
-__device__ __forceinline__ int clamp_rx(const Params& P, int x) { return min(max(x, P.ox), P.ox + P.stride - 1); }
-__device__ __forceinline__ int clamp_ry(const Params& P, int y) { return min(max(y, P.oy), P.oy + P.rows - 1); }
+template <class PT>
+__device__ __forceinline__ uint32_t pix(const PT& P, int x, int y) {
+    return __umul24((uint32_t)(y - p_oy(P)), (uint32_t)p_stride(P)) + (uint32_t)(x - p_ox(P));
+}
+template <class PT>
+__device__ __forceinline__ int clamp_rx(const PT& P, int x) {
+    return min(max(x, p_ox(P)), p_ox(P) + p_stride(P) - 1);
+}
+template <class PT>
+__device__ __forceinline__ int clamp_ry(const PT& P, int y) {
+    return min(max(y, p_oy(P)), p_oy(P) + p_rows(P) - 1);
+}
 
 __device__ __forceinline__ NoisyItem noisy_item(const Params& P, const NoisyInputs& in,
                                                 const Camera& cam, int gx, int gy, int frame,
@@ -245,8 +275,8 @@
     owner = ux >= 0 && ux < P.width && uy >= 0 && uy < P.height;
 }
 
-template <class IN = float, bool COLOUR = true, bool PLANE = false>
-__device__ __forceinline__ NoisyCur<IN, PLANE> noisy_load_current(const Params& P, const NoisyInputs& in, int gx,
+template <class IN = float, bool COLOUR = true, bool PLANE = false, class PT>
+__device__ __forceinline__ NoisyCur<IN, PLANE> noisy_load_current(const PT& P, const NoisyInputs& in, int gx,
                                                                   int gy, int frame,
                                                                   const float2* __restrict__ pf_plane = nullptr) {
     NoisyCur<IN, PLANE> c;
@@ -308,7 +338,8 @@
     pfx = u * (float)P.width - cam.jx;
     pfy = v * (float)P.height - (1 - cam.jy);
 }
-__device__ __forceinline__ Reproj reproject_taps(const Params& P, float pfx, float pfy, int px, int py) {
+template <class PT>
+__device__ __forceinline__ Reproj reproject_taps(const PT& P, float pfx, float pfy, int px, int py) {
     Reproj r;
     r.pfx = pfx;
     r.pfy = pfy;
@@ -319,10 +350,10 @@
     r.iy = iy;
     bilinear_weights(pfx, pfy, r.wts);
     r.over = 0;
-    if (P.check_reach) {
+    if (p_check_reach(P)) {
         const int x0 = max(ix, 0), x1 = min(ix + 1, P.width - 1);
         const int y0 = max(iy, 0), y1 = min(iy + 1, P.height - 1);
-        const bool tpx = px >= P.tx0 && px < P.tx1 && py >= P.ty0 && py < P.ty1;
+        const bool tpx = px >= p_tx0(P) && px < p_tx1(P) && py >= p_ty0(P) && py < p_ty1(P);
         const int vx0 = tpx ? P.wx0 : P.vx0, vx1 = tpx ? P.wx1 : P.vx1;
         const int vy0 = tpx ? P.wy0 : P.vy0, vy1 = tpx ? P.wy1 : P.vy1;
         if (x0 <= x1 && y0 <= y1)
@@ -336,14 +367,15 @@
     }
     return r;
 }
-__device__ __forceinline__ Reproj reproject(const Params& P, const Camera& cam, const f3& wp, int px, int py) {
+template <class PT>
+__device__ __forceinline__ Reproj reproject(const PT& P, const Camera& cam, const f3& wp, int px, int py) {
     float pfx, pfy;
     project_prev(P, cam, wp, pfx, pfy);
     return reproject_taps(P, pfx, pfy, px, py);
 }
 
-template <bool FILT = false, class IN = float, bool PLANE = false>
-__device__ __forceinline__ NoisyTaps<IN> noisy_taps_issue(const Params& P, const NoisyInputs& in, const Camera& cam,
+template <bool FILT = false, class IN = float, bool PLANE = false, class PT>
+__device__ __forceinline__ NoisyTaps<IN> noisy_taps_issue(const PT& P, const NoisyInputs& in, const Camera& cam,
                                                          const NoisyCur<IN, PLANE>& c, int frame,
                                                          const float* __restrict__ acc_prev = nullptr) {
     NoisyTaps<IN> tp;
@@ -366,13 +398,13 @@
             sidx[i] = pix(P, clamp_rx(P, r.ix + (i & 1)), clamp_ry(P, r.iy + (i >> 1)));
         }
         if constexpr (kPairTaps<IN>) {
-            const int n = P.stride * P.rows;
-            const int xc = min(max(r.ix, P.ox - 1), P.ox + P.stride - 1) - P.ox;
+            const int n = p_stride(P) * p_rows(P);
+            const int xc = min(max(r.ix, p_ox(P) - 1), p_ox(P) + p_stride(P) - 1) - p_ox(P);
             uint32_t spair[2];
             tp.fix = 0;
 #pragma unroll
             for (int row = 0; row < 2; ++row) {
-                const int sr = (int)__umul24((uint32_t)(clamp_ry(P, r.iy + row) - P.oy), (uint32_t)P.stride) + xc;
+                const int sr = (int)__umul24((uint32_t)(clamp_ry(P, r.iy + row) - p_oy(P)), (uint32_t)p_stride(P)) + xc;
                 spair[row] = (uint32_t)min(max(sr, 0), n - 2);
                 tp.fix |= ((uint32_t)(sr < 0) << (2 * row)) | ((uint32_t)(sr > n - 2) << (2 * row + 1));
             }
@@ -488,8 +520,8 @@
     }
 }
 
-template <bool FILT = false, class IN = float, bool PLANE = false>
-__device__ __forceinline__ NoisyItem noisy_taps_finish(const Params& P, const NoisyCur<IN, PLANE>& c,
+template <bool FILT = false, class IN = float, bool PLANE = false, class PT>
+__device__ __forceinline__ NoisyItem noisy_taps_finish(const PT& P, const NoisyCur<IN, PLANE>& c,
                                                       const NoisyTaps<IN>& tp, int frame) {
     const f3 wp = widen(c.wp), nrm = widen(c.nrm), cur = widen(c.cur);
     uint32_t accept = 0u;
@@ -510,15 +542,16 @@
     return o;
 }
 
-template <bool FILT = false, class IN = float, bool PLANE = false>
-__device__ __forceinline__ NoisyItem noisy_item_spec(const Params& P, const NoisyInputs& in, const Camera& cam,
+template <bool FILT = false, class IN = float, bool PLANE = false, class PT>
+__device__ __forceinline__ NoisyItem noisy_item_spec(const PT& P, const NoisyInputs& in, const Camera& cam,
                                                      const NoisyCur<IN, PLANE>& c, int frame,
                                                      const float* __restrict__ acc_prev = nullptr) {
     return noisy_taps_finish<FILT, IN, PLANE>(P, c, noisy_taps_issue<FILT, IN, PLANE>(P, in, cam, c, frame, acc_prev), frame);
 }
 
-__device__ __forceinline__ void report_reach(const Params& P, unsigned* reach, int over) {
-    if (P.check_reach && __builtin_amdgcn_ballot_w64(over > 0) != 0 && over > 0)
+template <class PT>
+__device__ __forceinline__ void report_reach(const PT& P, unsigned* reach, int over) {
+    if (p_check_reach(P) && __builtin_amdgcn_ballot_w64(over > 0) != 0 && over > 0)
         atomicMax(reach, (unsigned)over);
 }
 
@@ -751,7 +784,8 @@
     return f3{gamma_clamped(p.x, tE, tRP), gamma_clamped(p.y, tE, tRP), gamma_clamped(p.z, tE, tRP)};
 }
 
-__device__ __forceinline__ void taa_load_taps(const Params& P, float2 pf, const float* __restrict__ prev_frame,
+template <class PT>
+__device__ __forceinline__ void taa_load_taps(const PT& P, float2 pf, const float* __restrict__ prev_frame,
                                               f3 (&pc)[4]) {
     const int ix = (int)fminf(fmaxf(floorf(pf.x), -2.f), (float)P.width + 1.f);
     const int iy = (int)fminf(fmaxf(floorf(pf.y), -2.f), (float)P.height + 1.f);
diff --git a/bmfr_amd/csrc/bmfr_kernels.hip b/bmfr_amd/csrc/bmfr_kernels.hip
--- a/bmfr_amd/csrc/bmfr_kernels.hip
+++ b/bmfr_amd/csrc/bmfr_kernels.hip
@@ -88,9 +88,6 @@
     st3(result, lin, taa_resolve<true>(P, x, y, me, pf, nb, pc, frame));
 }
 
-constexpr int kTaaW = 64, kTaaH = 12;
-constexpr int kTaaNT = kTileThreads;
-constexpr int kTaaMinWaves = 6;
 template <class IN>
 __global__ __launch_bounds__(kTaaNT, kTaaMinWaves) void k_fused_taa(Params P, TaaArgs T) {
     __shared__ float4 Y[(kTaaW + 2) * (kTaaH + 2)];
@@ -235,6 +232,7 @@
 }
 
 hipError_t launch_fused_k2(const Params& P, hipStream_t st, const FusedArgs& A) {
+    if (untiled(P)) return launch_fused_k2_untiled(P, st, A);
     const dim3 grd((P.tx1 - P.tx0 + kTaaW - 1) / kTaaW, (P.ty1 - P.ty0 + kTaaH - 1) / kTaaH);
     if (P.input_half) hipLaunchKernelGGL((k_fused_taa<_Float16>), grd, dim3(kTaaNT), 0, st, P, taa_args(A));
     else hipLaunchKernelGGL((k_fused_taa<float>), grd, dim3(kTaaNT), 0, st, P, taa_args(A));
@@ -243,7 +241,7 @@
 
 hipError_t launch_fused_frame(const Params& P, hipStream_t st, const FusedArgs& A, hipEvent_t mid) {
     hipError_t e;
-    const bool one = P.frame_launches == 1 || (P.frame_launches == 0 && k1_blocks(P) < kTwoLaunchBlocks);
+    const bool one = P.frame_launches == 1 || (P.frame_launches == 0 && form_blocks(P) < kTwoLaunchBlocks);
     if (!mid && A.done && frame_fused_supported(P) && one) return launch_fused_frame_one(P, st, A);
     if (fused_supported(P)) {
         if ((e = launch_fused_k1_blocks(P, st, A)) != hipSuccess) return e;
diff --git a/bmfr_amd/csrc/bmfr_launch.h b/bmfr_amd/csrc/bmfr_launch.h
--- a/bmfr_amd/csrc/bmfr_launch.h
+++ b/bmfr_amd/csrc/bmfr_launch.h
@@ -71,6 +71,11 @@
 
 bool fitter_supported(int not_scaled, int scaled);
 inline int k1_blocks(const Params& P) { return P.ring > 0 ? P.ring : P.nbx * P.nby; }
+inline bool untiled(const Params& P) {
+    return !P.check_reach && P.ring == 0 && P.ox == 0 && P.oy == 0 && P.stride == P.width && P.rows == P.height &&
+           P.tx0 == 0 && P.ty0 == 0 && P.tx1 == P.width && P.ty1 == P.height;
+}
+inline int form_blocks(const Params& P) { return P.check_reach ? k1_blocks(P) : P.blocks_x * P.blocks_y; }
 constexpr int kTwoLaunchBlocks = 4096;
 bool fused_supported(const Params& P);
 hipError_t launch_fused_k1(const Params& P, hipStream_t st, const FusedArgs& A);
@@ -102,6 +107,7 @@
 hipError_t launch_fused_k1_taa(const Params& P, hipStream_t st, const FusedArgs* A, const Params& P2,
                                const FusedArgs* A2);
 hipError_t launch_fused_k2(const Params& P, hipStream_t st, const FusedArgs& A);
+hipError_t launch_fused_k2_untiled(const Params& P, hipStream_t st, const FusedArgs& A);
 hipError_t launch_taa(const Params& P, hipStream_t st, const float2* prev_pixel, const float* new_frame,
                       float* result, const float* prev_frame, int frame);
 
diff --git a/bmfr_amd/csrc/bmfr_taa_tile.h b/bmfr_amd/csrc/bmfr_taa_tile.h
--- a/bmfr_amd/csrc/bmfr_taa_tile.h
+++ b/bmfr_amd/csrc/bmfr_taa_tile.h
@@ -43,15 +43,17 @@
     }
 }
 
-__device__ __forceinline__ bool k1_in_launch(const Params& P, int bx, int by) {
-    if (P.ring <= 0) return P.ring == 0;
+template <class PT>
+__device__ __forceinline__ bool k1_in_launch(const PT& P, int bx, int by) {
+    if (p_ring(P) <= 0) return p_ring(P) == 0;
     return bx < P.rx0 || bx >= P.rx1 || by < P.ry0 || by >= P.ry1;
 }
 
-__device__ __forceinline__ void wait_k1_blocks(const Params& P, const TaaArgs& T, int x0, int y0, int th) {
+template <class PT>
+__device__ __forceinline__ void wait_k1_blocks(const PT& P, const TaaArgs& T, int x0, int y0, int th) {
     const int2 off = kBlockOffsets[T.frame & 15];
-    const int xa = max(x0 - 1, P.ox), xb = min(min(x0 + 64, P.tx1), P.ox + P.stride - 1);
-    const int ya = max(y0 - 1, P.oy), yb = min(min(y0 + th, P.ty1), P.oy + P.rows - 1);
+    const int xa = max(x0 - 1, p_ox(P)), xb = min(min(x0 + 64, p_tx1(P)), p_ox(P) + p_stride(P) - 1);
+    const int ya = max(y0 - 1, p_oy(P)), yb = min(min(y0 + th, p_ty1(P)), p_oy(P) + p_rows(P) - 1);
     const int bxa = (xa + kEdge / 2 - off.x) / kEdge, bxb = (xb + kEdge / 2 - off.x) / kEdge;
     const int bya = (ya + kEdge / 2 - off.y) / kEdge, byb = (yb + kEdge / 2 - off.y) / kEdge;
     const int nx = bxb - bxa + 1, n = nx * (byb - bya + 1);
@@ -114,15 +116,15 @@
     }
 }
 
-template <class IN, int TH, bool COH>
-__device__ __forceinline__ void tile_issue(const Params& P, const TaaArgs& T, int x0, int y0, int hx, int hy,
+template <class IN, int TH, bool COH, class PT>
+__device__ __forceinline__ void tile_issue(const PT& P, const TaaArgs& T, int x0, int y0, int hx, int hy,
                                            TileLoads<IN, TileShape<TH>::KN>& L) {
     using S = TileShape<TH>;
     const int t = threadIdx.x, tx = t & 63, ty = t >> 6;
     const CohPlane c_pp = coh_plane(T.prev_pixel), c_src = coh_plane(T.src);
 #pragma unroll
     for (int k = 0; k < S::KN; ++k) {
-        const uint32_t i = pix(P, min(x0 + tx, P.tx1 - 1), min(y0 + S::row(ty, k), P.ty1 - 1));
+        const uint32_t i = pix(P, min(x0 + tx, p_tx1(P) - 1), min(y0 + S::row(ty, k), p_ty1(P) - 1));
         if constexpr (COH) L.pf[k] = ld2_coh(c_pp, i);
         else L.pf[k] = ld_px(T.prev_pixel, i);
     }
@@ -176,15 +178,15 @@
     }
 }
 
-template <int KN>
-__device__ __forceinline__ void tile_taps(const Params& P, const TaaArgs& T, const float2 (&pf)[KN],
+template <int KN, class PT>
+__device__ __forceinline__ void tile_taps(const PT& P, const TaaArgs& T, const float2 (&pf)[KN],
                                           f3 (&taps)[KN][4]) {
 #pragma unroll
     for (int k = 0; k < KN; ++k) taa_load_taps(P, pf[k], T.prev_frame, taps[k]);
 }
 
-template <int TH, bool CHECK>
-__device__ __forceinline__ void resolve_strip(const Params& P, const TaaArgs& T, int x0, int y0,
+template <int TH, bool CHECK, class PT>
+__device__ __forceinline__ void resolve_strip(const PT& P, const TaaArgs& T, int x0, int y0,
                                               const float4* __restrict__ Y, const f3 (&me)[TileShape<TH>::KN],
                                               const float2 (&pf)[TileShape<TH>::KN],
                                               const f3 (&hist)[TileShape<TH>::KN]) {
@@ -222,7 +224,7 @@
     for (int k = 0; k < S::KN; ++k) {
         const Row w2 = reduce_row(k + 2);
         const int x = x0 + tx, y = y0 + r0 + k;
-        if (x < P.tx1 && y < P.ty1) {
+        if (x < p_tx1(P) && y < p_ty1(P)) {
             f3 r = me[k];
             if (!taa_offscreen(P, pf[k], T.frame)) {
                 const f3 mnb{mn4(w0.mn.x, w1.mn.x, w2.mn.x), mn4(w0.mn.y, w1.mn.y, w2.mn.y),
@@ -242,8 +244,8 @@
     }
 }
 
-template <int TH>
-__device__ __forceinline__ void tile_resolve(const Params& P, const TaaArgs& T, int x0, int y0,
+template <int TH, class PT>
+__device__ __forceinline__ void tile_resolve(const PT& P, const TaaArgs& T, int x0, int y0,
                                              const float4* __restrict__ Y, const f3 (&me)[TileShape<TH>::KN],
                                              const float2 (&pf)[TileShape<TH>::KN],
                                              const f3 (&hist)[TileShape<TH>::KN]) {
@@ -252,8 +254,8 @@
     else resolve_strip<TH, false>(P, T, x0, y0, Y, me, pf, hist);
 }
 
-template <class IN, int TH, bool COH = false>
-__device__ __forceinline__ void taa_tile(const Params& P, const TaaArgs& T, int x0, int y0, float4* __restrict__ Y,
+template <class IN, int TH, bool COH = false, class PT>
+__device__ __forceinline__ void taa_tile(const PT& P, const TaaArgs& T, int x0, int y0, float4* __restrict__ Y,
                                          double* __restrict__ sE, double2* __restrict__ sRP) {
     using S = TileShape<TH>;
     constexpr int KN = S::KN;
@@ -282,13 +284,13 @@
     double sE[kPowrENum];
     double2 sRP[kPowrRPNum];
 };
-template <class IN, bool COH>
-__device__ __forceinline__ void frame_taa_part(const Params& P2, const TaaArgs& T, int b, int nk1p, FrameTaaLds& L) {
+template <class IN, bool COH, class PT>
+__device__ __forceinline__ void frame_taa_part(const PT& P2, const TaaArgs& T, int b, int nk1p, FrameTaaLds& L) {
     constexpr int TH = kFrameTaaH;
-    const int gx = (P2.tx1 - P2.tx0 + 63) / 64, n2 = (int)gridDim.x - nk1p;
+    const int gx = (p_tx1(P2) - p_tx0(P2) + 63) / 64, n2 = (int)gridDim.x - nk1p;
     const int gi = xcd_swizzle(b - nk1p, n2);
-    taa_tile<IN, TH, COH>(P2, T, P2.tx0 + (gi % gx) * 64, P2.ty0 + (gi / gx) * TH, L.Y, L.sE, L.sRP);
-    if constexpr (COH) {
+    taa_tile<IN, TH, COH>(P2, T, p_tx0(P2) + (gi % gx) * 64, p_ty0(P2) + (gi / gx) * TH, L.Y, L.sE, L.sRP);
+    if constexpr (COH && !kUntiled<PT>) {
         if (T.reach_dev && b == (int)gridDim.x - 1) {
             wait_all_k1_blocks(P2, T);
             forward_reach(T);
@@ -300,4 +302,8 @@
     return ((P.tx1 - P.tx0 + 63) / 64) * ((P.ty1 - P.ty0 + TH - 1) / TH);
 }
 
-}
+constexpr int kTaaW = 64, kTaaH = 12;
+constexpr int kTaaNT = kTileThreads;
+constexpr int kTaaMinWaves = 6;
+
+}
diff --git a/bmfr_amd/csrc/bmfr_taa_untiled.hip b/bmfr_amd/csrc/bmfr_taa_untiled.hip
--- /dev/null
+++ b/bmfr_amd/csrc/bmfr_taa_untiled.hip
@@ -0,0 +1,25 @@
+#include "bmfr_launch.h"
+#include "bmfr_taa_tile.h"
+
+namespace bmfr {
+
+template <class IN>
+__global__ __launch_bounds__(kTaaNT, kTaaMinWaves) void k_fused_taa_untiled(UntiledParams P, TaaArgs T) {
+    __shared__ float4 Y[(kTaaW + 2) * (kTaaH + 2)];
+    __shared__ double sE[kPowrENum];
+    __shared__ double2 sRP[kPowrRPNum];
+    const int G = gridDim.x * gridDim.y;
+    const int gi = G - 1 - xcd_swizzle(blockIdx.y * gridDim.x + blockIdx.x, G);
+    const int bxi = gi % gridDim.x, byi = gi / gridDim.x;
+    taa_tile<IN, kTaaH, false>(P, T, bxi * kTaaW, byi * kTaaH, Y, sE, sRP);
+}
+
+hipError_t launch_fused_k2_untiled(const Params& P, hipStream_t st, const FusedArgs& A) {
+    const dim3 grd((P.width + kTaaW - 1) / kTaaW, (P.height + kTaaH - 1) / kTaaH);
+    const UntiledParams U{P};
+    if (P.input_half) hipLaunchKernelGGL((k_fused_taa_untiled<_Float16>), grd, dim3(kTaaNT), 0, st, U, taa_args(A));
+    else hipLaunchKernelGGL((k_fused_taa_untiled<float>), grd, dim3(kTaaNT), 0, st, U, taa_args(A));
+    return hipGetLastError();
+}
+
+}
diff --git a/bmfr_amd/pipeline.py b/bmfr_amd/pipeline.py
--- a/bmfr_amd/pipeline.py
+++ b/bmfr_amd/pipeline.py
@@ -65,6 +65,11 @@
         s = _lib.Sizes()
         check(_lib.load().bmfr_config_sizes(C.byref(self.to_c()), C.byref(s)), "bmfr_config_sizes")
         return s
+
+    def frame_blocks(self, frame: int) -> tuple:
+        r = (C.c_int * 4)()
+        check(_lib.load().bmfr_frame_blocks(C.byref(self.to_c()), frame, r), "bmfr_frame_blocks")
+        return tuple(r)
 
 
 def _ptr(t) -> int | None:
diff --git a/include/bmfr.h b/include/bmfr.h
--- a/include/bmfr.h
+++ b/include/bmfr.h
@@ -211,6 +211,8 @@
 
 bmfr_status bmfr_halo_need(const bmfr_config *cfg, int frame_number, int state_rect[4], int result_rect[4]);
 
+bmfr_status bmfr_frame_blocks(const bmfr_config *cfg, int frame_number, int block_rect[4]);
+
 bmfr_status bmfr_halo_plan(const bmfr_config *cfg, const int *tiles, int ntiles, int rank, int frame_number,
     int *peers, int *send_counts, int *recv_counts, int *records, int max_records, int *n_peers);
 
```

New measurement: 0.3340. About the same (+0.1%).
